# kanster/moped

Measured on AMD Instinct MI355X. Metric: detections/sec (frames/s) 640x480 ~3k SIFT vs N models, higher is better.
Workload: dtype f32

## Files before the change

### include/moped_hip.h

```cpp
#ifndef MOPED_HIP_H
#define MOPED_HIP_H

#include <stddef.h>
#include <stdint.h>

#ifdef __cplusplus
extern "C" {
#endif

#define MH_DESC_DIM 128
#define MH_MAX_BATCH 32
#define MH_MAX_IMAGES 8
#define MH_MAX_MODELS 8192
#define MH_OK 0
#define MH_ERR_ARG (-1)
#define MH_ERR_HIP (-2)
#define MH_ERR_CAPACITY (-3)
#define MH_ERR_NODEVICE (-4)

typedef struct mh_ctx mh_ctx;


int mh_create(int device, mh_ctx** out);
void mh_destroy(mh_ctx* ctx);
const char* mh_last_error(const mh_ctx* ctx);
int mh_set_stream(mh_ctx* ctx, void* hip_stream);
int mh_synchronize(mh_ctx* ctx);
int mh_reserve(mh_ctx* ctx, int max_queries, int max_clusters, int max_objects);
int mh_reserve_batch(mh_ctx* ctx, int queries_per_frame, int frames, int max_clusters, int max_objects);


int mh_db_upload(mh_ctx* ctx, const float* desc_host, const int32_t* model_of_host,
                 const float* xyz_host, int N, int n_models, int32_t index_base);
int mh_db_upload_blocks(mh_ctx* ctx, const float* desc_host, const int32_t* model_of_host, const float* xyz_host, int N,
                        int n_models, const int32_t* block_global_row, const int32_t* block_rows, int n_blocks,
                        int normalize);
int mh_db_size(const mh_ctx* ctx, int* N, int* n_models);
int mh_db_share(mh_ctx* dst, mh_ctx* src);

enum { MH_DB_INSERT = 0, MH_DB_REPLACE = 1, MH_DB_REMOVE = 2 };
int mh_db_model_rows(const mh_ctx* ctx, int model, int32_t* row_begin, int32_t* n_rows);
int mh_db_splice(mh_ctx* ctx, int op, int model, const float* desc, const float* xyz, int n_rows, int normalize,
                 int on_device);
int mh_db_reserve(mh_ctx* ctx, int64_t max_rows, int max_models);
int mh_db_adopt(mh_ctx* dst, mh_ctx* src);
int mh_db_generation(const mh_ctx* ctx, uint64_t* generation);
int mh_db_debug_fetch(mh_ctx* ctx, int which, void* out_host, size_t bytes);
int mh_db_debug_screen(mh_ctx* ctx, uint32_t out[8]);
int mh_db_debug_route(mh_ctx* ctx, int route);
int mh_db_edit_ms(mh_ctx* ctx, float* ms);


int mh_normalize(mh_ctx* ctx, float* desc_host, int n);

int mh_match(mh_ctx* ctx, const float* q_host, int Q, float ratio,
             int32_t* nn_idx, int32_t* nn_raw, float* d1, float* d2);
int mh_normalize_match(mh_ctx* ctx, float* q_host, int Q, float ratio, int32_t* nn_idx, int32_t* nn_raw, float* d1,
                       float* d2);

int mh_match_stats(mh_ctx* ctx, int Q, uint32_t stats[4], int reset);
int mh_match_set_mode(mh_ctx* ctx, int mode);
int mh_pose_set_split(mh_ctx* ctx, int on);
int mh_match_launches(mh_ctx* ctx, uint32_t out[3]);
float mh_screen_margin(float qq, float dmax);
int mh_screen_values(mh_ctx* ctx, const float* q_host, int Q, int n_rows, float* out_host, float* dmax, float* spread,
                     int shape );
uint16_t mh_screen_record_value(float top, float thr);
void mh_screen_record_bounds(uint16_t value_bits, uint32_t row0, float tau, float spread, int N, float dmax, float* lo,
                             float* hi);
float mh_screen_pack_value(float v, uint32_t id, int bits);
float mh_screen_pack_pert(float qq, float dmax, int bits);
void mh_screen_sample_bounds(uint16_t value_bits, float tau, float pert, float dmax, float* lo, float* hi);
void mh_screen_launch_plan(int Q, int q_expected, int N, int32_t out[8]);
int mh_screen_park_places(void);
int mh_match_incomplete(mh_ctx* ctx, uint32_t* count, int reset);
int mh_screen_sample_values(mh_ctx* ctx, const float* q_host, int Q, const int32_t* row0_host, float* out_host);
int mh_match_query_candidates(mh_ctx* ctx, int Q, uint32_t* out);

int mh_match_local_dev(mh_ctx* ctx, const float* qn_dev, const float* qnorm_dev, int Q,
                       int32_t* idx1_dev, float* d1_dev, float* d2_dev);
int mh_match_local_counted_dev(mh_ctx* ctx, const float* qn_dev, const float* qnorm_dev, int Q,
                               const int32_t* q_count_dev, int q_expected, int32_t* idx1_dev, float* d1_dev,
                               float* d2_dev);
int mh_match_merge_dev(mh_ctx* ctx, const int32_t* idx1_s_dev, const float* d1_s_dev,
                       const float* d2_s_dev, int n_shards, int Q,
                       int32_t* idx1_dev, float* d1_dev, float* d2_dev);
int mh_normalize_dev(mh_ctx* ctx, float* q_dev, float* qnorm_dev, int Q);


int mh_meanshift(mh_ctx* ctx, const float* pts_host, int n, int dim, float radius,
                 float merge, int min_pts, int max_iter, int32_t* label,
                 int32_t* order, int32_t* n_clusters);
int mh_meanshift_batch(mh_ctx* ctx, const float* pts_host, const int32_t* off, int n_problems,
                       int dim, float radius, float merge, int min_pts, int max_iter,
                       int32_t* label, int32_t* order, int32_t* n_clusters);


typedef struct {
  float u, v;
  float x, y, z;
} mh_corr;

typedef struct {
  float K[4];
  float cam[7];
} mh_cam;

typedef struct {
  int n_hypotheses;
  int max_objects_per_cluster;
  int n_pts_align;
  int min_n_pts_object;
  float error_threshold;
  int lm_iters_l2;
  int lm_iters_l4;
} mh_pose_params;

typedef struct {
  float pose[7];
  int32_t cluster;
  int32_t n_inliers;
  float err;
} mh_pose_out;

int mh_pose_ransac(mh_ctx* ctx, const mh_corr* corr_host, const int32_t* cluster_off,
                   int n_clusters, const mh_cam* cam, const mh_pose_params* prm,
                   uint64_t seed, mh_pose_out* out_host, int32_t* n_out);
int mh_pose_ransac_images(mh_ctx* ctx, const mh_corr* corr_host, const int32_t* image_of_host,
                          const int32_t* cluster_off, int n_clusters, const mh_cam* cams, int n_images,
                          const mh_pose_params* prm, uint64_t seed, mh_pose_out* out_host, int32_t* n_out);

typedef struct {
  float wx, wy, wz;
  float w;
} mh_depth;

#define MH_DEPTH_NONE 0
#define MH_DEPTH_BACKPROJECTION 1
#define MH_DEPTH_REPROJECTION 2

int mh_pose_ransac_depth(mh_ctx* ctx, const mh_corr* corr_host, const mh_depth* depth_host,
                         const int32_t* cluster_off, int n_clusters, const mh_cam* cam,
                         const mh_pose_params* prm, int kind, float alpha, uint64_t seed,
                         mh_pose_out* out_host, int32_t* n_out);

int mh_project_test(mh_ctx* ctx, const float pose[7], const mh_corr* corr_host, int n,
                    const mh_cam* cam, float thr, uint8_t* inlier_host, float* err2_host,
                    int32_t* n_inliers);


int mh_filter_images(mh_ctx* ctx, const mh_corr* corr_host, const int32_t* image_of_host, const int32_t* model_off,
                     int n_models, const int32_t* obj_model, const float* obj_pose, int n_obj, const mh_cam* cams,
                     int n_images, int min_points, float feature_distance, float min_score, float* score,
                     uint8_t* keep, int32_t* out_order, int32_t* cl_members, int32_t* cl_off, int32_t* n_kept);
int mh_filter(mh_ctx* ctx, const mh_corr* corr_host, const int32_t* model_off, int n_models,
              const int32_t* obj_model, const float* obj_pose, int n_obj, const mh_cam* cam,
              int min_points, float feature_distance, float min_score,
              float* score, uint8_t* keep, int32_t* out_order, int32_t* cl_members,
// ... 403 lines not shown
```

### moped_amd/capi.py

```python
from __future__ import annotations

import ctypes as C
import os

import numpy as np

_HERE = os.path.dirname(os.path.abspath(__file__))
LIB_PATH = os.environ.get("MH_LIB_PATH") or os.path.join(_HERE, "libmoped_hip.so")

MH_OK = 0
MH_ERR_ARG = -1
MH_ERR_CAPACITY = -3


class MhError(RuntimeError):
    pass


class mh_corr(C.Structure):
    _fields_ = [("u", C.c_float), ("v", C.c_float), ("x", C.c_float), ("y", C.c_float), ("z", C.c_float)]


class mh_cam(C.Structure):
    _fields_ = [("K", C.c_float * 4), ("cam", C.c_float * 7)]
# ... 117 lines not shown
    sp.merge_dist = float(merge_dist)
    return sp


def make_view(depth_ptr, fill_ptr=None, pose=None, K=None) -> mh_view:
    v = mh_view()
    v.depth_xyzn_dev = depth_ptr
    v.fill_distance_dev = fill_ptr
    v.pose[:] = [float(x) for x in (pose if pose is not None else POSE_IDENTITY)]
    v.K[:] = [float(x) for x in (K if K is not None else (1.0, 1.0, 0.0, 0.0))]
    return v


RAW_DEPTH_F32_M, RAW_DEPTH_U16_MM = 0, 1


class mh_raw_depth(C.Structure):
    _fields_ = [("format", C.c_int32), ("width", C.c_int32), ("height", C.c_int32), ("elem_stride", C.c_int32),
                ("row_stride", C.c_int32), ("offset", C.c_int32)]


def make_raw_depth(fmt, width, height, elem_stride=None, row_stride=None, offset=0) -> mh_raw_depth:
    es = 4 if fmt == RAW_DEPTH_F32_M else 2
    elem_stride = es if elem_stride is None else elem_stride
    row_stride = width * elem_stride if row_stride is None else row_stride
    return mh_raw_depth(int(fmt), int(width), int(height), int(elem_stride), int(row_stride), int(offset))


def make_filter_depth_params(p):
    if p is None or isinstance(p, mh_filter_depth_params):
        return p
    a, b, c = p
    return mh_filter_depth_params(float(a), float(b), float(c))


EXPORTS = [
    "mh_create", "mh_destroy", "mh_last_error", "mh_set_stream", "mh_synchronize", "mh_reserve",
    "mh_db_upload", "mh_db_size", "mh_normalize", "mh_match", "mh_normalize_match", "mh_match_local_dev", "mh_match_local_counted_dev",
    "mh_match_merge_dev", "mh_normalize_dev", "mh_meanshift", "mh_meanshift_batch", "mh_pose_ransac", "mh_pose_ransac_depth",
    "mh_frame_set_depth", "mh_project_test",
    "mh_filter", "mh_frame_default_params", "mh_frame_enqueue", "mh_frame_set_depth_image", "mh_frame_enqueue_match_local",
    "mh_frame_enqueue_rest", "mh_frame_fetch", "mh_frame_result_dev", "mh_enable_timing", "mh_timing",
    "mh_frame_set_cluster_linkage", "mh_cluster_linkage", "mh_frame_set_depth_image_host",
    "mh_depth_fill", "mh_depth_fill_status", "mh_depth_fill_host", "mh_depth_fill_batch", "mh_depth_fill_set_mode", "mh_depth_fill_get_mode", "mh_depth_fill_stats",
    "mh_frame_enqueue_rest_batch", "mh_frame_enqueue_rest_frames", "mh_frame_fetch_slot", "mh_frame_result_copy_slots_dev",
    "mh_frame_set_depth_rules", "mh_frame_fetch_matches", "mh_frame_enqueue_rest_strided", "mh_frame_result_copy_dev",
    "mh_sift_extract", "mh_sift_extract_dev", "mh_frame_enqueue_image", "mh_frame_enqueue_image_batch", "mh_frame_features_dev", "mh_frame_keypoints",
    "mh_models_create", "mh_models_destroy", "mh_models_last_error", "mh_models_add_xml",
    "mh_models_add_xml_buffer", "mh_models_count", "mh_models_rows", "mh_models_name", "mh_models_range",
    "mh_models_desc", "mh_models_xyz", "mh_models_save", "mh_models_load", "mh_db_upload_models",
    "mh_db_splice", "mh_db_reserve", "mh_db_adopt", "mh_db_generation", "mh_db_model_rows", "mh_db_splice_models",
    "mh_db_debug_fetch", "mh_depth_rules_debug_fetch", "mh_db_debug_screen", "mh_db_debug_route", "mh_db_edit_ms",
    "mh_db_upload_raw", "mh_db_share", "mh_match_stats", "mh_match_set_mode", "mh_match_launches", "mh_pose_set_split", "mh_frame_fetch_match_points", "mh_screen_margin", "mh_frame_counters", "mh_match_timing", "mh_frame_set_images", "mh_filter_images",
    "mh_pose_ransac_images",
    "mh_comm_unique_id", "mh_comm_create", "mh_comm_create_all", "mh_comm_create_host", "mh_comm_destroy", "mh_comm_info",
    "mh_frame_enqueue_sharded", "mh_frame_enqueue_sharded_batch", "mh_frame_enqueue_sharded_all",
    "mh_frame_previous_objects", "mh_frame_gather_objects", "mh_frame_enqueue_batch", "mh_frame_set_depth_image_batch",
    "mh_pose_kernel_info", "mh_db_upload_blocks", "mh_frame_fetch_matches_slot", "mh_frame_fetch_match_reps_slot",
    "mh_screen_values", "mh_screen_record_value", "mh_screen_record_bounds", "mh_reserve_batch", "mh_frame_run_host",
    "mh_frame_block_stride", "mh_frame_fetch_batch_async", "mh_frame_fetch_previous_async", "mh_frame_fetch_wait",
    "mh_frame_fetch_query", "mh_host_alloc", "mh_host_free", "mh_frame_run_host_begin", "mh_frame_wait_descriptors",
    "mh_step_match", "mh_step_match_fetch", "mh_step_cluster", "mh_step_pose", "mh_step_filter",
    "mh_set_linkage_scratch_limit",
    "mh_undistort_map", "mh_undistort", "mh_undistort_dev", "mh_frame_set_undistort",
    "mh_sift_extract_batch_dev", "mh_sift_debug_plan", "mh_sift_debug_level", "mh_sift_debug_candidates",
    "mh_sift_debug_keys", "mh_sift_debug_blur",
    "mh_screen_pack_value", "mh_screen_pack_pert", "mh_screen_sample_bounds", "mh_screen_launch_plan", "mh_match_incomplete",
    "mh_screen_sample_values", "mh_match_query_candidates", "mh_screen_park_places",
    "mh_frame_enqueue_images", "mh_frame_enqueue_images_batch", "mh_frame_set_undistort_images", "mh_frame_image_counts",
    "mh_frame_features_image_dev",
    "mh_filter_depth_set_points", "mh_filter_depth", "mh_frame_set_filter_depth",
    "mh_frame_route", "mh_filter_depth_debug_form",
    "mh_depth_filter", "mh_depth_prop", "mh_frame_run_kinect_host",
    "mh_linkage_debug_matrix", "mh_linkage_debug_agglomerate", "mh_linkage_set_mode", "mh_linkage_get_mode", "mh_linkage_stats", "mh_frame_debug_fetch_clusters_slot",
    "mh_planar_rows_dev", "mh_planar_rows_batch_dev", "mh_db_splice_image", "mh_db_splice_images",
    "mh_models_add_rows", "mh_models_write_xml",
    "mh_view_rows_dev", "mh_view_rows_batch_dev", "mh_db_append", "mh_db_splice_view", "mh_db_append_view", "mh_db_splice_views",
    "mh_depth_map_from_raw_dev", "mh_depth_map_from_raw_batch_dev", "mh_depth_map_from_raw_host",
    "mh_frame_run_kinect_raw_host",
    "mh_frame_debug_fetch_cluster_table_slot",
    "mh_object_hulls", "mh_hull_debug_form",
    "mh_frame_set_hulls", "mh_frame_fetch_hulls_slot", "mh_frame_fetch_hulls", "mh_frame_hull_block_stride",
    "mh_frame_fetch_batch_hulls_async",
]
COMM_ID_BYTES = 128
EX2_OBJECTS = 62
ALLGATHER_FN = C.CFUNCTYPE(C.c_int, C.c_void_p, C.c_void_p, C.c_void_p, C.c_size_t)

DIM = 128
HULL_LDS_POINTS = 8192
DB_INSERT, DB_REPLACE, DB_REMOVE = 0, 1, 2
_lib = None


def load():
    global _lib
    if _lib is not None:
        return _lib
    try:
        import torch
    except Exception:
        pass
    if not os.path.exists(LIB_PATH):
        raise MhError(f"{LIB_PATH} not built: run `python -c 'import __graft_entry__ as g; g.build()'`")
    L = C.CDLL(LIB_PATH)
    vp, i32, f32 = C.c_void_p, C.c_int, C.c_float
    L.mh_create.argtypes = [i32, C.POINTER(vp)]
    L.mh_destroy.argtypes = [vp]
    L.mh_destroy.restype = None
    L.mh_last_error.argtypes = [vp]
    L.mh_last_error.restype = C.c_char_p
    L.mh_set_stream.argtypes = [vp, vp]
    L.mh_synchronize.argtypes = [vp]
    L.mh_reserve.argtypes = [vp, i32, i32, i32]
    L.mh_reserve_batch.argtypes = [vp, i32, i32, i32, i32]
    if hasattr(L, "mh_lane_create"):
        L.mh_lane_create.argtypes = [i32, i32, i32, i32, C.POINTER(vp)]
        L.mh_lane_destroy.argtypes = [vp]
        L.mh_set_lane.argtypes = [vp, vp]
    L.mh_db_upload.argtypes = [vp, vp, vp, vp, i32, i32, C.c_int32]
    L.mh_db_size.argtypes = [vp, C.POINTER(i32), C.POINTER(i32)]
    L.mh_normalize.argtypes = [vp, vp, i32]
    L.mh_match.argtypes = [vp, vp, i32, f32, vp, vp, vp, vp]
    L.mh_normalize_match.argtypes = [vp, vp, i32, f32, vp, vp, vp, vp]
    L.mh_match_local_dev.argtypes = [vp, vp, vp, i32, vp, vp, vp]
    if hasattr(L, "mh_match_local_counted_dev"):
        L.mh_match_local_counted_dev.argtypes = [vp, vp, vp, i32, vp, i32, vp, vp, vp]
    L.mh_match_merge_dev.argtypes = [vp, vp, vp, vp, i32, i32, vp, vp, vp]
    L.mh_normalize_dev.argtypes = [vp, vp, vp, i32]
    L.mh_meanshift.argtypes = [vp, vp, i32, i32, f32, f32, i32, i32, vp, vp, C.POINTER(C.c_int32)]
    L.mh_meanshift_batch.argtypes = [vp, vp, vp, i32, i32, f32, f32, i32, i32, vp, vp, vp]
    L.mh_pose_ransac.argtypes = [vp, vp, vp, i32, C.POINTER(mh_cam), C.POINTER(mh_pose_params),
                                 C.c_uint64, vp, C.POINTER(C.c_int32)]
    L.mh_pose_ransac_depth.argtypes = [vp, vp, vp, vp, i32, C.POINTER(mh_cam), C.POINTER(mh_pose_params), i32, f32,
                                       C.c_uint64, vp, C.POINTER(C.c_int32)]
    L.mh_frame_set_depth.argtypes = [vp, vp, i32, f32]
    L.mh_project_test.argtypes = [vp, vp, vp, i32, C.POINTER(mh_cam), f32, vp, vp, C.POINTER(C.c_int32)]
    L.mh_filter.argtypes = [vp, vp, vp, i32, vp, vp, i32, C.POINTER(mh_cam), i32, f32, f32,
                            vp, vp, vp, vp, vp, C.POINTER(C.c_int32)]
    L.mh_frame_default_params.argtypes = [C.POINTER(mh_frame_params)]
    L.mh_frame_default_params.restype = None
    L.mh_frame_enqueue.argtypes = [vp, vp, vp, i32, C.POINTER(mh_cam), C.POINTER(mh_frame_params), C.c_uint64]
    L.mh_frame_run_host.argtypes = [vp, vp, vp, vp, i32, C.POINTER(mh_cam), i32, C.POINTER(mh_frame_params), C.c_uint64, i32,
                                    vp, i32, C.POINTER(C.c_int32), vp]
    L.mh_frame_run_host_begin.argtypes = [vp, vp, vp, vp, i32, C.POINTER(mh_cam), i32, C.POINTER(mh_frame_params), C.c_uint64, i32]
    L.mh_sift_extract.argtypes = [vp, vp, i32, i32, i32, vp, vp, vp, i32, C.POINTER(C.c_int32)]
    L.mh_sift_extract_dev.argtypes = [vp, vp, i32, i32, i32, vp, vp, vp, i32, vp]
    L.mh_sift_extract_batch_dev.argtypes = [vp, vp, i32, i32, i32, i32, vp, vp, i32, vp]
    L.mh_sift_debug_plan.argtypes = [vp, vp, vp, vp, vp]
    L.mh_sift_debug_level.argtypes = [vp, i32, i32, i32, i32, vp]
    L.mh_sift_debug_candidates.argtypes = [vp, i32, vp, vp, i32, C.POINTER(C.c_int32)]
    L.mh_sift_debug_keys.argtypes = [vp, i32, vp, i32, C.POINTER(C.c_int32)]
    L.mh_sift_debug_blur.argtypes = [vp, i32, vp, i32, i32, f32, i32, vp, vp, vp]
    L.mh_frame_enqueue_image.argtypes = [vp, vp, i32, i32, i32, i32, C.POINTER(mh_cam), C.POINTER(mh_frame_params),
                                         C.c_uint64]
    L.mh_frame_enqueue_image_batch.argtypes = [vp, vp, i32, i32, i32, i32, i32, C.POINTER(mh_cam), C.POINTER(mh_frame_params), vp]
    L.mh_frame_set_depth_image_host.argtypes = [vp, vp, vp, i32, i32, i32, f32, f32]
    L.mh_depth_fill.argtypes = [vp, vp, i32, i32, i32, i32, vp, vp, vp]
    L.mh_depth_fill_status.argtypes = [vp]
    L.mh_depth_fill_set_mode.argtypes = [vp, i32]
    L.mh_depth_fill_get_mode.argtypes = [vp, vp]
    L.mh_depth_fill_stats.argtypes = [vp, i32, vp]
    if hasattr(L, "mh_depth_fill_batch"):
        L.mh_depth_fill_batch.argtypes = [vp, C.POINTER(vp), C.POINTER(vp), i32, i32, i32, i32, i32, vp]
    L.mh_depth_fill_host.argtypes = [vp, vp, i32, i32, i32, i32, vp, vp, vp]
    L.mh_frame_set_cluster_linkage.argtypes = [vp, C.POINTER(mh_linkage_params)]
# ... 42 lines not shown
    L.mh_db_upload_raw.argtypes = [vp, vp, vp, vp, i32, i32, i32, i32]
    L.mh_frame_set_depth_image.argtypes = [vp, vp, vp, i32, i32, i32, f32, f32]
    L.mh_frame_enqueue_match_local.argtypes = [vp, vp, i32, vp]
    L.mh_frame_enqueue_rest.argtypes = [vp, vp, i32, vp, i32, C.POINTER(mh_cam),
                                        C.POINTER(mh_frame_params), C.c_uint64]
    L.mh_frame_fetch.argtypes = [vp, vp, i32, C.POINTER(C.c_int32), vp]
    L.mh_frame_result_dev.argtypes = [vp, C.POINTER(vp), C.POINTER(C.c_int64)]
    L.mh_db_share.argtypes = [vp, vp]
    L.mh_db_splice.argtypes = [vp, i32, i32, vp, vp, i32, i32, i32]
    L.mh_db_reserve.argtypes = [vp, C.c_int64, i32]
    L.mh_db_adopt.argtypes = [vp, vp]
    L.mh_db_generation.argtypes = [vp, C.POINTER(C.c_uint64)]
    L.mh_db_model_rows.argtypes = [vp, i32, C.POINTER(C.c_int32), C.POINTER(C.c_int32)]
    L.mh_db_splice_models.argtypes = [vp, i32, i32, vp, i32]
    L.mh_db_debug_fetch.argtypes = [vp, i32, vp, C.c_size_t]
    L.mh_depth_rules_debug_fetch.argtypes = [vp, i32, i32, vp, C.c_size_t]
    L.mh_depth_filter.argtypes = [vp, vp, i32, i32, vp, i32, f32, vp, vp, i32, vp]
    L.mh_depth_prop.argtypes = [vp, vp, vp, i32, i32, vp, i32, vp]
    L.mh_frame_run_kinect_host.argtypes = [vp, vp, vp, vp, i32, i32, i32, i32, C.POINTER(mh_cam), C.POINTER(mh_frame_params),
                                           i32, i32, i32, f32, f32, C.c_uint64, vp, i32, C.POINTER(C.c_int32), vp]
    if hasattr(L, "mh_depth_map_from_raw_dev"):
        rd = C.POINTER(mh_raw_depth)
        L.mh_depth_map_from_raw_dev.argtypes = [vp, vp, rd, vp, vp, i32, i32]
        L.mh_depth_map_from_raw_batch_dev.argtypes = [vp, C.POINTER(vp), rd, vp, C.POINTER(vp), i32, i32, i32]
        L.mh_depth_map_from_raw_host.argtypes = [vp, vp, rd, vp, vp, i32, i32]
        L.mh_frame_run_kinect_raw_host.argtypes = [vp, vp, vp, rd, vp, vp, i32, i32, i32, i32, C.POINTER(mh_cam),
                                                   C.POINTER(mh_frame_params), i32, i32, i32, f32, f32, C.c_uint64, vp, i32,
                                                   C.POINTER(C.c_int32), vp]
    L.mh_db_debug_screen.argtypes = [vp, vp]
    L.mh_db_debug_route.argtypes = [vp, i32]
    L.mh_db_edit_ms.argtypes = [vp, C.POINTER(f32)]
    L.mh_match_stats.argtypes = [vp, i32, vp, i32]
    L.mh_match_set_mode.argtypes = [vp, i32]
    L.mh_match_launches.argtypes = [vp, vp]
    L.mh_pose_set_split.argtypes = [vp, i32]
    L.mh_frame_counters.argtypes = [vp, vp]
    L.mh_frame_set_images.argtypes = [vp, vp, vp, i32]
    L.mh_filter_images.argtypes = [vp, vp, vp, vp, i32, vp, vp, i32, vp, i32, i32, f32, f32,
                                   vp, vp, vp, vp, vp, C.POINTER(C.c_int32)]
    L.mh_pose_ransac_images.argtypes = [vp, vp, vp, vp, i32, vp, i32, C.POINTER(mh_pose_params),
                                        C.c_uint64, vp, C.POINTER(C.c_int32)]
    L.mh_match_timing.argtypes = [vp, vp]
    L.mh_screen_margin.argtypes = [f32, f32]
    L.mh_screen_margin.restype = f32
    L.mh_enable_timing.argtypes = [vp, i32]
    L.mh_timing.argtypes = [vp, C.POINTER(mh_times)]
    L.mh_comm_unique_id.argtypes = [vp]
    L.mh_comm_create.argtypes = [vp, vp, i32, i32, C.POINTER(vp)]
    L.mh_comm_create_all.argtypes = [C.POINTER(vp), i32, C.POINTER(vp)]
    L.mh_comm_create_host.argtypes = [vp, i32, i32, ALLGATHER_FN, vp, C.POINTER(vp)]
    L.mh_comm_destroy.argtypes = [vp]
    L.mh_comm_info.argtypes = [vp, C.POINTER(i32), C.POINTER(i32), C.POINTER(i32)]
    L.mh_frame_enqueue_sharded.argtypes = [vp, vp, vp, vp, i32, C.POINTER(mh_cam), C.POINTER(mh_frame_params), C.c_uint64]
    L.mh_frame_enqueue_sharded_batch.argtypes = [vp, vp, vp, vp, i32, i32, C.POINTER(mh_cam),
                                                 C.POINTER(mh_frame_params), C.POINTER(C.c_uint64)]
    L.mh_frame_enqueue_sharded_all.argtypes = [C.POINTER(vp), C.POINTER(vp), i32, C.POINTER(vp), C.POINTER(vp), i32, i32,
                                               C.POINTER(mh_cam), C.POINTER(mh_frame_params), C.POINTER(C.c_uint64)]
    L.mh_frame_enqueue_batch.argtypes = [vp, vp, vp, i32, i32, C.POINTER(mh_cam), C.POINTER(mh_frame_params),
                                         C.POINTER(C.c_uint64)]
    L.mh_frame_set_depth_image_batch.argtypes = [vp, C.POINTER(vp), C.POINTER(vp), i32, i32, i32, i32, f32, f32]
    L.mh_frame_previous_objects.argtypes = [vp, i32, vp, i32, C.POINTER(C.c_int32)]
    L.mh_frame_gather_objects.argtypes = [vp, vp, i32, vp, i32, C.POINTER(C.c_int32)]
    L.mh_pose_kernel_info.argtypes = [vp, i32, vp]
    L.mh_frame_fetch_matches_slot.argtypes = [vp, i32, vp, vp, i32, C.POINTER(C.c_int32)]
    L.mh_frame_fetch_match_reps_slot.argtypes = [vp, i32, vp, i32, C.POINTER(C.c_int32)]
    L.mh_frame_fetch_match_points.argtypes = [vp, vp, i32, C.POINTER(C.c_int32)]
    L.mh_frame_enqueue_rest_frames.argtypes = [vp, vp, i32, vp, i32, i32, i32, i32, C.POINTER(mh_cam),
                                               C.POINTER(mh_frame_params), C.POINTER(C.c_uint64)]
    L.mh_screen_values.argtypes = [vp, vp, i32, i32, vp, C.POINTER(f32), C.POINTER(f32), i32]
    L.mh_screen_record_value.argtypes = [f32, f32]
    L.mh_screen_record_value.restype = C.c_uint16
    L.mh_screen_record_bounds.argtypes = [C.c_uint16, C.c_uint32, f32, f32, i32, f32, C.POINTER(f32), C.POINTER(f32)]
    L.mh_screen_record_bounds.restype = None
    if hasattr(L, "mh_screen_pack_value"):
        L.mh_screen_pack_value.argtypes = [f32, C.c_uint32, i32]
        L.mh_screen_pack_value.restype = f32
        L.mh_screen_pack_pert.argtypes = [f32, f32, i32]
        L.mh_screen_pack_pert.restype = f32
        L.mh_screen_sample_bounds.argtypes = [C.c_uint16, f32, f32, f32, C.POINTER(f32), C.POINTER(f32)]
        L.mh_screen_sample_bounds.restype = None
        L.mh_screen_launch_plan.argtypes = [i32, i32, i32, vp]
        L.mh_screen_launch_plan.restype = None
        L.mh_match_incomplete.argtypes = [vp, C.POINTER(C.c_uint32), i32]
    if hasattr(L, "mh_screen_sample_values"):
        L.mh_screen_sample_values.argtypes = [vp, vp, i32, vp, vp]
        L.mh_match_query_candidates.argtypes = [vp, i32, vp]
    L.mh_db_upload_blocks.argtypes = [vp, vp, vp, vp, i32, i32, vp, vp, i32, i32]
    L.mh_frame_block_stride.argtypes = [i32]
    L.mh_frame_block_stride.restype = C.c_size_t
    L.mh_frame_fetch_batch_async.argtypes = [vp, i32, i32, vp, C.c_uint32]
    L.mh_frame_fetch_previous_async.argtypes = [vp, i32, vp, C.c_uint32]
    L.mh_frame_fetch_wait.argtypes = [vp, C.POINTER(C.c_int32)]
    L.mh_host_alloc.argtypes = [vp, C.c_size_t, C.POINTER(vp)]
    L.mh_host_free.argtypes = [vp, vp]
    L.mh_frame_wait_descriptors.argtypes = [vp]
    if hasattr(L, "mh_step_match"):
        L.mh_set_linkage_scratch_limit.argtypes = [vp, C.c_size_t]
        L.mh_step_match.argtypes = [vp, vp, vp, i32, C.POINTER(mh_cam), f32, i32]
        L.mh_step_match_fetch.argtypes = [vp, vp, vp, vp, i32, C.POINTER(C.c_int32)]
        L.mh_step_cluster.argtypes = [vp, f32, f32, i32, i32, vp, vp, vp, i32, i32, C.POINTER(C.c_int32)]
        L.mh_step_pose.argtypes = [vp, i32, C.POINTER(mh_pose_params), C.c_uint64, vp, i32, C.POINTER(C.c_int32)]
        L.mh_step_filter.argtypes = [vp, i32, i32, f32, f32, i32, vp, vp, vp, vp, vp, i32, C.POINTER(C.c_int32)]
    L.mh_frame_fetch_query.argtypes = [vp]
    if hasattr(L, "mh_undistort"):
        L.mh_undistort_map.argtypes = [vp, i32, i32, vp, vp, vp, vp]
        L.mh_undistort.argtypes = [vp, vp, vp, i32, i32, vp, vp]
        L.mh_undistort_dev.argtypes = [vp, vp, vp, i32, i32, vp, vp]
        L.mh_frame_set_undistort.argtypes = [vp, vp]
    if hasattr(L, "mh_frame_enqueue_images"):
        L.mh_frame_enqueue_images.argtypes = [vp, vp, i32, i32, i32, i32, i32, vp, C.POINTER(mh_frame_params), C.c_uint64]
        L.mh_frame_enqueue_images_batch.argtypes = [vp, vp, i32, i32, i32, i32, i32, i32, vp, C.POINTER(mh_frame_params), vp]
        L.mh_frame_set_undistort_images.argtypes = [vp, vp, i32]
        L.mh_frame_image_counts.argtypes = [vp, vp, i32, C.POINTER(C.c_int32)]
        L.mh_frame_features_image_dev.argtypes = [vp, C.POINTER(vp)]
    if hasattr(L, "mh_filter_depth"):
        L.mh_filter_depth_set_points.argtypes = [vp, vp, vp, i32]
        L.mh_filter_depth.argtypes = [vp, vp, vp, i32, vp, vp, i32, C.POINTER(mh_cam), i32, f32, f32, C.POINTER(mh_cam),
                                      C.POINTER(mh_filter_depth_params), vp, vp, vp, vp, vp, C.POINTER(C.c_int32), vp, vp, vp]
        L.mh_frame_set_filter_depth.argtypes = [vp, C.POINTER(mh_filter_depth_params), C.POINTER(mh_filter_depth_params),
                                                C.POINTER(mh_cam)]
    if hasattr(L, "mh_frame_route"):
        L.mh_frame_route.argtypes = [vp, vp]
        L.mh_filter_depth_debug_form.argtypes = [vp, i32]
    if hasattr(L, "mh_planar_rows_dev"):
        L.mh_planar_rows_dev.argtypes = [vp, vp, vp, vp, i32, C.POINTER(mh_planar_spec), vp, vp, i32, vp, vp]
        L.mh_planar_rows_batch_dev.argtypes = [vp, vp, vp, vp, i32, i32, C.POINTER(mh_planar_spec), vp, vp, i32, vp, vp]
        L.mh_db_splice_image.argtypes = [vp, i32, i32, vp, i32, i32, i32, i32, C.POINTER(mh_planar_spec),
                                         C.POINTER(C.c_int32), vp, vp, vp, i32]
        L.mh_db_splice_images.argtypes = [vp, i32, vp, i32, i32, i32, i32, i32, C.POINTER(mh_planar_spec), vp, vp, vp, vp, i32]
        L.mh_models_add_rows.argtypes = [vp, C.c_char_p, vp, vp, C.c_int64]
        L.mh_models_write_xml.argtypes = [vp, i32, C.c_char_p]
    if hasattr(L, "mh_view_rows_dev"):
        pv, ps, pd = C.POINTER(mh_view), C.POINTER(mh_view_spec), C.POINTER(mh_view_dup)
        L.mh_view_rows_dev.argtypes = [vp, vp, vp, vp, i32, pv, i32, i32, ps, pd, vp, vp, i32, vp, vp, vp]
        L.mh_view_rows_batch_dev.argtypes = [vp, vp, vp, vp, i32, i32, pv, i32, i32, ps, pd, vp, vp, i32, vp, vp, vp]
        L.mh_db_append.argtypes = [vp, i32, vp, vp, i32, i32, i32]
        L.mh_db_splice_view.argtypes = [vp, i32, i32, vp, pv, i32, i32, i32, i32, ps, C.POINTER(C.c_int32), vp, vp, vp, vp, i32]
        L.mh_db_append_view.argtypes = [vp, i32, vp, pv, i32, i32, i32, i32, ps, C.POINTER(C.c_int32), vp, vp, vp, vp, i32]
        L.mh_db_splice_views.argtypes = [vp, i32, vp, pv, i32, i32, i32, i32, i32, ps, vp, vp, vp, vp, vp, i32]
    if hasattr(L, "mh_object_hulls"):
        L.mh_object_hulls.argtypes = [vp, vp, vp, i32, C.POINTER(mh_cam), i32, vp, vp, vp, vp]
        L.mh_hull_debug_form.argtypes = [vp, i32]
        L.mh_frame_set_hulls.argtypes = [vp, i32, i32]
        L.mh_frame_fetch_hulls_slot.argtypes = [vp, i32, i32, i32, vp, vp, vp, vp, C.POINTER(C.c_int32)]
        L.mh_frame_fetch_hulls.argtypes = [vp, i32, i32, vp, vp, vp, vp, C.POINTER(C.c_int32)]
        L.mh_frame_hull_block_stride.argtypes = [i32, i32]
        L.mh_frame_hull_block_stride.restype = C.c_size_t
        L.mh_frame_fetch_batch_hulls_async.argtypes = [vp, i32, i32, vp]
    _lib = L
    return L


def _calib(v):
    a = np.ascontiguousarray(v, np.float32).reshape(-1)
    if a.size != 4:
        raise ValueError("a calibration has 4 values")
    return a


def make_cam(K, cam) -> mh_cam:
    c = mh_cam()
    c.K[:] = [float(x) for x in K]
    c.cam[:] = [float(x) for x in cam]
    return c


# ... 400 lines not shown
        return dict(zip(names, (int(v) for v in o)))

    def db_debug_fetch(self, which: str) -> np.ndarray:
        sc = self.db_debug_screen()
        N, img = sc["N"], sc["has_image"]
        n_pad = (N + 127) // 128 * 128
        k, dt, n = {"desc": (0, np.float32, n_pad * DIM), "norm": (1, np.float32, n_pad), "xyz": (2, np.float32, N * 3),
                    "model": (3, np.int32, N), "desc_h": (4, np.uint16, n_pad * DIM if img else 0),
                    "neg_h": (5, np.float32, n_pad // 128 * 192 if img else 0)}[which]
        out = np.zeros(n, dt)
        self._ck(self.L.mh_db_debug_fetch(self.h, k, _ptr(out), out.nbytes), "mh_db_debug_fetch")
        return out

    def db_debug_route(self, route: int):
        self._ck(self.L.mh_db_debug_route(self.h, int(route)), "mh_db_debug_route")

    def db_edit_ms(self) -> float:
        ms = C.c_float(0)
        self._ck(self.L.mh_db_edit_ms(self.h, C.byref(ms)), "mh_db_edit_ms")
        return float(ms.value)

    def frame_counters(self) -> dict:
        c = np.zeros(8, np.int32)
        self._ck(self.L.mh_frame_counters(self.h, _ptr(c)), "mh_frame_counters")
        names = ("matches", "clusters", "r2", "r3", "r4", "pose_tasks", "error", "hypotheses")
        return dict(zip(names, (int(v) for v in c)))

    def pose_kernel_info(self, kind=0):
        o = np.zeros(8, np.int32)
        self._ck(self.L.mh_pose_kernel_info(self.h, int(kind), _ptr(o)), "mh_pose_kernel_info")
        waves = int(o[5])
        return {"vgprs": int(o[0]), "lds_bytes": int(o[1]), "threads": int(o[2]), "workgroups_per_cu": int(o[3]),
                "scratch_bytes": int(o[4]), "waves_per_workgroup": waves,
                "waves_per_simd": int(o[3]) * waves / 4.0}

    def match_timing(self) -> dict:
        t = np.zeros(5, np.float32)
        self._ck(self.L.mh_match_timing(self.h, _ptr(t)), "mh_match_timing")
        return dict(zip(("prepare_ms", "pass_a_ms", "thresholds_ms", "pass_b_ms", "pass_c_ms"), (float(v) for v in t)))

    def screen_values(self, qn, n_rows, shape=0):
        qn = np.ascontiguousarray(qn, np.float32)
        out = np.zeros((qn.shape[0], n_rows), np.float32)
        dmax, spread = C.c_float(0), C.c_float(0)
        self._ck(self.L.mh_screen_values(self.h, _ptr(qn), qn.shape[0], n_rows, _ptr(out), C.byref(dmax), C.byref(spread),
                                         int(shape)), "mh_screen_values")
        return out, dmax.value, spread.value

    def screen_sample_values(self, qn, row0):
        qn = np.ascontiguousarray(qn, np.float32)
        row0 = np.ascontiguousarray(row0, np.int32)
        assert row0.shape == (qn.shape[0], 2)
        out = np.zeros((qn.shape[0], 2, 8), np.float32)
        self._ck(self.L.mh_screen_sample_values(self.h, _ptr(qn), qn.shape[0], _ptr(row0), _ptr(out)), "mh_screen_sample_values")
        return out

    def match_set_mode(self, mode: int):
        self._ck(self.L.mh_match_set_mode(self.h, int(mode)), "mh_match_set_mode")

    def pose_set_split(self, on: bool):
        self._ck(self.L.mh_pose_set_split(self.h, int(bool(on))), "mh_pose_set_split")

    def match_kernel_launches(self) -> dict:
        o = np.zeros(3, np.uint32)
        self._ck(self.L.mh_match_launches(self.h, _ptr(o)), "mh_match_launches")
        return {"valu": int(o[0]), "mfma": int(o[1]), "screen": int(o[2])}

    def match_stats(self, Q=0, reset=False) -> dict:
        st = np.zeros(4, np.uint32)
        self._ck(self.L.mh_match_stats(self.h, int(Q), _ptr(st), int(reset)), "mh_match_stats")
        return {"candidates": int(st[0]), "brute_force_queries": int(st[1]), "queries": int(st[2]),
                "two_stage": bool(st[3])}

    def match_query_candidates(self, Q):
        out = np.zeros(int(Q), np.uint32)
        self._ck(self.L.mh_match_query_candidates(self.h, int(Q), _ptr(out)), "mh_match_query_candidates")
        return out

    def match_incomplete(self, reset=False) -> int:
        n = C.c_uint32(0)
        self._ck(self.L.mh_match_incomplete(self.h, C.byref(n), int(reset)), "mh_match_incomplete")
        return int(n.value)

    def normalize(self, desc):
        d = np.ascontiguousarray(desc, np.float32).copy()
        self._ck(self.L.mh_normalize(self.h, _ptr(d), d.shape[0]), "mh_normalize")
        return d

    def match(self, q, ratio=0.8):
        q = np.ascontiguousarray(q, np.float32)
        Q = q.shape[0]
        acc = np.full(Q, -1, np.int32)
        raw = np.full(Q, -1, np.int32)
        d1 = np.zeros(Q, np.float32)
        d2 = np.zeros(Q, np.float32)
        self._ck(self.L.mh_match(self.h, _ptr(q), Q, ratio, _ptr(acc), _ptr(raw), _ptr(d1), _ptr(d2)), "mh_match")
        return acc, raw, d1, d2

    def normalize_match(self, q, ratio=0.8):
        q = np.ascontiguousarray(q, np.float32).copy()
        Q = q.shape[0]
        acc = np.full(Q, -1, np.int32)
        raw = np.full(Q, -1, np.int32)
        d1 = np.zeros(Q, np.float32)
        d2 = np.zeros(Q, np.float32)
        self._ck(self.L.mh_normalize_match(self.h, _ptr(q), Q, ratio, _ptr(acc), _ptr(raw), _ptr(d1), _ptr(d2)),
                 "mh_normalize_match")
        return q, acc, raw, d1, d2

    def meanshift(self, pts, radius=200.0, merge=20.0, min_pts=7, max_iter=100):
        pts = np.ascontiguousarray(pts, np.float32)
        n = pts.shape[0]
        dim = pts.shape[1] if pts.ndim == 2 else 2
        label = np.full(max(n, 1), -1, np.int32)
        order = np.full(max(n, 1), -1, np.int32)
        ncl = C.c_int32(0)
        self._ck(self.L.mh_meanshift(self.h, _ptr(pts), n, dim, radius, merge, min_pts, max_iter,
                                     _ptr(label), _ptr(order), C.byref(ncl)), "mh_meanshift")
        label = label[:n]
        clusters, pos = [], 0
        for c in range(ncl.value):
            sz = int((label == c).sum())
            clusters.append(order[pos:pos + sz].copy())
            pos += sz
        return clusters, label

    def meanshift_batch(self, problems, radius=200.0, merge=20.0, min_pts=7, max_iter=100):
        dim = 2
        for p in problems:
            if np.asarray(p).ndim == 2 and np.asarray(p).shape[0]:
                dim = np.asarray(p).shape[1]
        sizes = [int(np.asarray(p).shape[0]) for p in problems]
        off = np.zeros(len(problems) + 1, np.int32)
        off[1:] = np.cumsum(sizes)
        total = int(off[-1])
        pts = (np.concatenate([np.asarray(p, np.float32).reshape(-1, dim) for p in problems])
               if total else np.zeros((0, dim), np.float32))
        pts = np.ascontiguousarray(pts, np.float32)
        label = np.full(max(total, 1), -1, np.int32)
        order = np.full(max(total, 1), -1, np.int32)
        ncl = np.zeros(max(len(problems), 1), np.int32)
        self._ck(self.L.mh_meanshift_batch(self.h, _ptr(pts), _ptr(off), len(problems), dim, radius, merge,
                                           min_pts, max_iter, _ptr(label), _ptr(order), _ptr(ncl)),
                 "mh_meanshift_batch")
        out = []
        for i in range(len(problems)):
            b, e = int(off[i]), int(off[i + 1])
            lab, ordr = label[b:e], order[b:e]
            clusters, pos = [], 0
            for c in range(int(ncl[i])):
                sz = int((lab == c).sum())
                clusters.append(ordr[pos:pos + sz].copy())
                pos += sz
            out.append((clusters, lab.copy()))
        return out

    def pose_ransac(self, corr, cluster_off, K, cam, params: mh_pose_params, seed=1):
        corr = np.ascontiguousarray(corr, CORR_DTYPE)
        cluster_off = np.ascontiguousarray(cluster_off, np.int32)
        ncl = len(cluster_off) - 1
        R = max(params.max_objects_per_cluster, 1)
        out = np.zeros(max(ncl * R, 1), POSE_OUT_DTYPE)
        n_out = C.c_int32(0)
        c = make_cam(K, cam)
        self._ck(self.L.mh_pose_ransac(self.h, _ptr(corr), _ptr(cluster_off), ncl, C.byref(c),
                                       C.byref(params), seed, _ptr(out), C.byref(n_out)), "mh_pose_ransac")
# ... 971 lines not shown
```

### moped_amd/csrc/api.hip

```cpp
#include <algorithm>
#include <cmath>
#include <cstring>
#include <new>
#include <vector>

#include "context.h"
#include "steps.h"

using namespace mh;

namespace mh {

int use_stream(mh_ctx* ctx) {
  if (!ctx->held.empty()) db_poll_held(ctx, false);
  if (ctx->stream) return MH_OK;
  if (!ctx->own_stream) MH_HIP(ctx, hipStreamCreateWithFlags(&ctx->own_stream, hipStreamNonBlocking));
  ctx->stream = ctx->own_stream;
  return MH_OK;
}

int ensure_scratch(mh_ctx* ctx, size_t bytes) {
  if (bytes > ctx->scratch.cap) MH_HIP(ctx, ctx->scratch.ensure(bytes + bytes / 4 + 4096, ctx->stream));
  return MH_OK;
}

int ensure_pinned(mh_ctx* ctx, size_t bytes) {
  if (bytes > ctx->pinned.cap) MH_HIP(ctx, ctx->pinned.ensure(bytes + bytes / 4 + 4096, ctx->stream));
  return MH_OK;
}

int ensure_own_depth(mh_ctx* ctx, size_t px) {
  MH_HIP(ctx, ctx->own_depth.ensure(px * 4, ctx->stream));
  MH_HIP(ctx, ctx->own_fill.ensure(px, ctx->stream));
  return MH_OK;
}

void bind_store(mh_ctx* ctx) {
  const DbStore* st = ctx->store.get();
  ctx->N = st ? st->N : 0;
  ctx->n_models = st ? st->n_models : 0;
  ctx->index_base = st ? st->index_base : 0;
  ctx->rmap = RowMap();
  if (st) {
    ctx->rmap.base = st->index_base;
    ctx->rmap.nb = st->n_blocks;
    ctx->rmap.glo = st->blk_glo;
    ctx->rmap.llo = st->blk_llo;
  }
  ctx->db_desc = st ? st->desc : nullptr;
  ctx->db_norm = st ? st->norm : nullptr;
  ctx->db_xyz = st ? st->xyz : nullptr;
  ctx->db_model = st ? st->model : nullptr;
  ctx->sdb = st ? st->screen : ScreenDb();
}

int ensure_match_scratch(mh_ctx* ctx, int Q) {
  hipStream_t s = ctx->stream;
  MH_HIP(ctx, ctx->match_pack.ensure(match_pack_floats(Q), s));
  MH_HIP(ctx, ctx->match_scratch.ensure(match_scratch_elems(Q, ctx->N > 0 ? ctx->N : 1), s));
  const int q_pad = screen_q_pad(Q);
  if (ctx->sdb.usable && q_pad > ctx->sbuf.q_pad) {
    ScreenBufs& b = ctx->sbuf;
    mh_ctx::ScreenOwn& o = ctx->screen_own;
    b = ScreenBufs();
    const size_t qp = (size_t)q_pad, slots = qp * screen_rec_slots();
    MH_HIP(ctx, o.qh.ensure(qp * DIM, s));
    MH_HIP(ctx, o.qbad.ensure(qp, s));
    MH_HIP(ctx, o.part.ensure(screen_part_bytes(q_pad), s));
    MH_HIP(ctx, o.tau.ensure(qp, s));
    MH_HIP(ctx, o.recs.ensure(slots, s));
    MH_HIP(ctx, o.ovf_cnt.ensure(qp, s));
    MH_HIP(ctx, o.ovf.ensure(qp * SCREEN_OVF_CAP, s));
    MH_HIP(ctx, o.stats.ensure(qp * 3, s));
    MH_HIP(ctx, o.inc.ensure(qp + 1, s));
    MH_HIP(ctx, hipMemsetAsync(o.inc, 0, (qp + 1) * sizeof(unsigned int), s));
    MH_HIP(ctx, hipMemsetAsync(o.recs, 0, slots * sizeof(uint2), s));
    MH_HIP(ctx, hipMemsetAsync(o.ovf_cnt, 0, qp * sizeof(int32_t), s));
    MH_HIP(ctx, hipMemsetAsync(o.stats, 0, qp * 3 * sizeof(unsigned int), s));
    b.qh = o.qh;
    b.qbad = o.qbad;
    b.part = reinterpret_cast<float2*>(o.part.p);
    b.tau = o.tau;
    b.recs = o.recs;
    b.ovf_cnt = o.ovf_cnt;
    b.ovf = o.ovf;
    b.stats = o.stats;
    b.inc = o.inc;
    b.ovf_cap = SCREEN_OVF_CAP;
    b.q_pad = q_pad;
  }
  return MH_OK;
}

int ctx_match(mh_ctx* ctx, const float* qn, const float* qnorm, int Q, int32_t* idx1, float* d1, float* d2,
              const int32_t* q_count, int q_expected) {
  if (Q <= 0) return MH_OK;
  int rc = ensure_match_scratch(ctx, Q);
  if (rc) return rc;
  const int qe = (q_expected > 0 && q_expected < Q) ? q_expected : Q;
  const int screen_mode = ctx->match_mode >= 2 ? 0 : ctx->match_mode;
  const int kernel_pin = ctx->match_mode >= 2 ? ctx->match_mode - 2 : -1;
  if (ctx->sdb.usable && ctx->sbuf.q_pad >= screen_q_pad(Q) && screen_wanted(qe, ctx->N, screen_mode)) {
    ctx->sbuf.ev = nullptr;
    if (ctx->timing && ctx->ev_made) {
      ctx->sbuf.ev = ctx->mev[ctx->mev_next];
      ctx->mev_next = (ctx->mev_next + 1) % mh_ctx::MEV_SETS;
      ++ctx->mev_used;
    }
    ctx->sbuf.big = ctx->lane_stream;
    ctx->sbuf.n_cus = ctx->n_cus;
    ctx->sbuf.ev_in = ctx->lane_in;
    ctx->sbuf.ev_out = ctx->lane_out;
    launch_match_screen(qn, qnorm, Q, ctx->db_desc, ctx->db_norm, ctx->N, ctx->rmap, ctx->sdb, ctx->sbuf, idx1, d1,
                        d2, ctx->stream, q_count, q_expected);
    ++ctx->match_launches[2];
  } else {
    const int k = launch_match(qn, qnorm, Q, ctx->db_desc, ctx->db_norm, ctx->N, ctx->rmap, ctx->match_scratch,
                               ctx->match_pack, idx1, d1, d2, ctx->stream, q_count, q_expected, kernel_pin);
    if (k >= 0) ++ctx->match_launches[k];
  }
  return MH_OK;
}

int ensure_frame_buffers(mh_ctx* ctx, int Q) {
  if (Q <= ctx->max_q) return MH_OK;
  int cap = ctx->max_q > 0 ? ctx->max_q : 4096;
  while (cap < Q) cap *= 2;
  const size_t n = (size_t)cap;
  hipStream_t s = ctx->stream;
  MH_HIP(ctx, ctx->q_desc.ensure(n * DIM, s));
  MH_HIP(ctx, ctx->q_norm.ensure(n, s));
  MH_HIP(ctx, ctx->q_uv.ensure(n * 2, s));
  MH_HIP(ctx, ctx->nn_idx.ensure(n, s));
  MH_HIP(ctx, ctx->nn_d1.ensure(n, s));
  MH_HIP(ctx, ctx->nn_d2.ensure(n, s));
  ctx->max_q = cap;
  return MH_OK;
}

}

extern "C" {

int mh_create(int device, mh_ctx** out) {
  if (!out) return MH_ERR_ARG;
  *out = nullptr;
  int count = 0;
  if (hipGetDeviceCount(&count) != hipSuccess || count <= 0 || device < 0 || device >= count)
    return MH_ERR_NODEVICE;
  hipDeviceProp_t prop;
  if (hipGetDeviceProperties(&prop, device) != hipSuccess) return MH_ERR_NODEVICE;
  if (std::strncmp(prop.gcnArchName, "gfx950", 6) != 0) return MH_ERR_NODEVICE;
  if (hipSetDevice(device) != hipSuccess) return MH_ERR_HIP;
  mh_ctx* ctx = new (std::nothrow) mh_ctx;
  if (!ctx) return MH_ERR_HIP;
  ctx->device = device;
  ctx->n_cus = prop.multiProcessorCount;
  ctx->stream = nullptr;
  *out = ctx;
  return MH_OK;
}

void mh_free_frame_state(mh_ctx* ctx);
void mh_free_sift_state(mh_ctx* ctx);
void mh_free_undistort_state(mh_ctx* ctx);

void mh_destroy(mh_ctx* ctx) {
  if (!ctx) return;
  hipSetDevice(ctx->device);
  if (ctx->stream) hipStreamSynchronize(ctx->stream);
  mh_free_frame_state(ctx);
  mh_free_sift_state(ctx);
  mh_free_undistort_state(ctx);
  db_poll_held(ctx, true);
  for (hipEvent_t e : ctx->held_events) hipEventDestroy(e);
  for (hipEvent_t e : ctx->db_ev)
    if (e) hipEventDestroy(e);
  if (ctx->wb_ev) hipEventDestroy(ctx->wb_ev);
  if (ctx->wb_stream) hipStreamDestroy(ctx->wb_stream);
  if (ctx->ev_made)
    for (auto& e : ctx->ev) hipEventDestroy(e);
  for (auto& set : ctx->mev)
    for (auto& e : set)
      if (e) hipEventDestroy(e);
  if (ctx->dlv.done) hipEventDestroy(ctx->dlv.done);
  if (ctx->hulls.done) hipEventDestroy(ctx->hulls.done);
  if (ctx->lane_in) hipEventDestroy(ctx->lane_in);
  if (ctx->lane_out) hipEventDestroy(ctx->lane_out);
  if (ctx->own_stream) hipStreamDestroy(ctx->own_stream);
  delete ctx;
}

#ifdef MH_EXPERIMENTS
extern "C" int mh_lane_create(int device, int n_streams, int reserve_cus_per_xcd, int low_priority, mh_lane** out) {
  if (low_priority) return MH_ERR_ARG;
// ... 231 lines not shown
}

int mh_normalize(mh_ctx* ctx, float* desc_host, int n) {
  if (!ctx || n < 0 || (n > 0 && !desc_host)) return MH_ERR_ARG;
  if (n == 0) return MH_OK;
  MH_HIP(ctx, hipSetDevice(ctx->device));
  if (int rc_stream = mh::use_stream(ctx)) return rc_stream;
  int rc = ensure_frame_buffers(ctx, n);
  if (rc) return rc;
  const size_t bytes = (size_t)n * DIM * sizeof(float);
  MH_HIP(ctx, hipMemcpyAsync(ctx->q_desc, desc_host, bytes, hipMemcpyHostToDevice, ctx->stream));
  launch_normalize(ctx->q_desc, ctx->q_norm, n, ctx->stream);
  MH_HIP(ctx, hipGetLastError());
  MH_HIP(ctx, hipMemcpyAsync(desc_host, ctx->q_desc, bytes, hipMemcpyDeviceToHost, ctx->stream));
  MH_HIP(ctx, hipStreamSynchronize(ctx->stream));
  return MH_OK;
}

int mh_normalize_dev(mh_ctx* ctx, float* q_dev, float* qnorm_dev, int Q) {
  if (!ctx || Q < 0 || (Q > 0 && (!q_dev || !qnorm_dev))) return MH_ERR_ARG;
  MH_HIP(ctx, hipSetDevice(ctx->device));
  if (int rc_stream = mh::use_stream(ctx)) return rc_stream;
  launch_normalize(q_dev, qnorm_dev, Q, ctx->stream);
  MH_HIP(ctx, hipGetLastError());
  return MH_OK;
}

int mh_match_local_dev(mh_ctx* ctx, const float* qn_dev, const float* qnorm_dev, int Q,
                       int32_t* idx1_dev, float* d1_dev, float* d2_dev) {
  if (!ctx || Q < 0 || (Q > 0 && (!qn_dev || !qnorm_dev || !idx1_dev || !d1_dev || !d2_dev)))
    return MH_ERR_ARG;
  if (Q == 0) return MH_OK;
  MH_HIP(ctx, hipSetDevice(ctx->device));
  if (int rc_stream = mh::use_stream(ctx)) return rc_stream;
  int rc = ctx_match(ctx, qn_dev, qnorm_dev, Q, idx1_dev, d1_dev, d2_dev);
  if (rc) return rc;
  MH_HIP(ctx, hipGetLastError());
  return MH_OK;
}

int mh_match_local_counted_dev(mh_ctx* ctx, const float* qn_dev, const float* qnorm_dev, int Q, const int32_t* q_count_dev,
                               int q_expected, int32_t* idx1_dev, float* d1_dev, float* d2_dev) {
  if (!ctx || Q < 0 || q_expected < 0 || !q_count_dev || (Q > 0 && (!qn_dev || !qnorm_dev || !idx1_dev || !d1_dev || !d2_dev)))
    return MH_ERR_ARG;
  if (Q == 0) return MH_OK;
  MH_HIP(ctx, hipSetDevice(ctx->device));
  if (int rc_stream = mh::use_stream(ctx)) return rc_stream;
  int rc = ctx_match(ctx, qn_dev, qnorm_dev, Q, idx1_dev, d1_dev, d2_dev, q_count_dev, q_expected);
  if (rc) return rc;
  MH_HIP(ctx, hipGetLastError());
  return MH_OK;
}

int mh_match_merge_dev(mh_ctx* ctx, const int32_t* idx1_s_dev, const float* d1_s_dev,
                       const float* d2_s_dev, int n_shards, int Q, int32_t* idx1_dev,
                       float* d1_dev, float* d2_dev) {
  if (!ctx || Q < 0 || n_shards < 0) return MH_ERR_ARG;
  if (Q == 0) return MH_OK;
  MH_HIP(ctx, hipSetDevice(ctx->device));
  if (int rc_stream = mh::use_stream(ctx)) return rc_stream;
  launch_match_merge(idx1_s_dev, d1_s_dev, d2_s_dev, n_shards, Q, (size_t)Q, idx1_dev, d1_dev, d2_dev,
                     ctx->stream);
  MH_HIP(ctx, hipGetLastError());
  return MH_OK;
}

static int match_host(mh_ctx* ctx, const float* q_host, float* normalized_out, int Q, float ratio, int32_t* nn_idx,
                      int32_t* nn_raw, float* d1, float* d2) {
  if (!ctx || Q < 0 || (Q > 0 && (!q_host || !nn_idx))) return MH_ERR_ARG;
  if (Q == 0) return MH_OK;
  MH_HIP(ctx, hipSetDevice(ctx->device));
  if (int rc_stream = mh::use_stream(ctx)) return rc_stream;
  int rc = ensure_frame_buffers(ctx, Q);
  if (rc) return rc;
  if ((rc = ensure_match_scratch(ctx, Q))) return rc;
  if ((rc = ensure_pinned(ctx, (size_t)Q * 16))) return rc;
  if ((rc = ensure_scratch(ctx, (size_t)Q * 4))) return rc;
  const size_t bytes = (size_t)Q * DIM * sizeof(float);
  MH_HIP(ctx, hipMemcpyAsync(ctx->q_desc, q_host, bytes, hipMemcpyHostToDevice, ctx->stream));
  if (normalized_out)
    launch_normalize(ctx->q_desc, ctx->q_norm, Q, ctx->stream);
  else
    launch_row_norms(ctx->q_desc, ctx->q_norm, Q, ctx->stream);
  if ((rc = ctx_match(ctx, ctx->q_desc, ctx->q_norm, Q, ctx->nn_idx, ctx->nn_d1, ctx->nn_d2))) return rc;
  int32_t* d_acc = (int32_t*)ctx->scratch.p;
  launch_accept(ctx->nn_idx, ctx->nn_d1, ctx->nn_d2, Q, ratio, d_acc, ctx->stream);
  MH_HIP(ctx, hipGetLastError());
  int32_t* h_acc = (int32_t*)ctx->pinned.p;
  int32_t* h_raw = h_acc + Q;
  float* h_d1 = (float*)(h_raw + Q);
  float* h_d2 = h_d1 + Q;
  MH_HIP(ctx, hipMemcpyAsync(h_acc, d_acc, (size_t)Q * 4, hipMemcpyDeviceToHost, ctx->stream));
  MH_HIP(ctx, hipMemcpyAsync(h_raw, ctx->nn_idx, (size_t)Q * 4, hipMemcpyDeviceToHost, ctx->stream));
  MH_HIP(ctx, hipMemcpyAsync(h_d1, ctx->nn_d1, (size_t)Q * 4, hipMemcpyDeviceToHost, ctx->stream));
  MH_HIP(ctx, hipMemcpyAsync(h_d2, ctx->nn_d2, (size_t)Q * 4, hipMemcpyDeviceToHost, ctx->stream));
  if (normalized_out) MH_HIP(ctx, hipMemcpyAsync(normalized_out, ctx->q_desc, bytes, hipMemcpyDeviceToHost, ctx->stream));
  MH_HIP(ctx, hipStreamSynchronize(ctx->stream));
  std::memcpy(nn_idx, h_acc, (size_t)Q * 4);
  if (nn_raw) std::memcpy(nn_raw, h_raw, (size_t)Q * 4);
  if (d1) std::memcpy(d1, h_d1, (size_t)Q * 4);
  if (d2) std::memcpy(d2, h_d2, (size_t)Q * 4);
  return MH_OK;
}

int mh_match(mh_ctx* ctx, const float* q_host, int Q, float ratio, int32_t* nn_idx,
             int32_t* nn_raw, float* d1, float* d2) {
  return match_host(ctx, q_host, nullptr, Q, ratio, nn_idx, nn_raw, d1, d2);
}

int mh_normalize_match(mh_ctx* ctx, float* q_host, int Q, float ratio, int32_t* nn_idx, int32_t* nn_raw, float* d1,
                       float* d2) {
  return match_host(ctx, q_host, q_host, Q, ratio, nn_idx, nn_raw, d1, d2);
}

#ifdef MH_TRACE
static unsigned long long* g_trace_dev = nullptr;
int mh_trace_enable(int on) {
  if (on && !g_trace_dev) {
    if (hipMalloc(&g_trace_dev, (8 + 4 * TRACE_CAP) * sizeof(unsigned long long)) != hipSuccess) return MH_ERR_HIP;
    hipMemset(g_trace_dev, 0, 64);
  }
  unsigned long long* p = on ? g_trace_dev : nullptr;
  const int n = std::min(trace_n_binds().load(), 32);
  for (int i = 0; i < n; ++i) trace_binds()[i](p);
  hipDeviceSynchronize();
  return MH_OK;
}
long long mh_trace_fetch(unsigned long long* out, long long cap) {
  if (!g_trace_dev) return -1;
  hipDeviceSynchronize();
  unsigned long long n = 0;
  hipMemcpy(&n, g_trace_dev, sizeof n, hipMemcpyDeviceToHost);
  const unsigned long long have = std::min<unsigned long long>(n, TRACE_CAP);
  const unsigned long long take = std::min<unsigned long long>(have, (unsigned long long)std::max(cap, 0ll));
  if (take && out) hipMemcpy(out, g_trace_dev + 8, take * 32, hipMemcpyDeviceToHost);
  hipMemset(g_trace_dev, 0, 8);
  return (long long)n;
}
#endif

float mh_screen_margin(float qq, float dmax) { return screen_margin_host(qq, dmax); }

uint16_t mh_screen_record_value(float top, float thr) { return screen_record_value(top, thr); }

void mh_screen_record_bounds(uint16_t value_bits, uint32_t row0, float tau, float spread, int N, float dmax, float* lo,
                             float* hi) {
  float l, h;
  screen_record_bounds(value_bits, row0, tau, spread, N, dmax, l, h);
  if (lo) *lo = l;
  if (hi) *hi = h;
}

float mh_screen_pack_value(float v, uint32_t id, int bits) { return screen_pack_value(v, id, bits); }

float mh_screen_pack_pert(float qq, float dmax, int bits) { return screen_pack_pert(qq, dmax, bits); }

void mh_screen_sample_bounds(uint16_t value_bits, float tau, float pert, float dmax, float* lo, float* hi) {
  float l, h;
  screen_sample_bounds(value_bits, tau, pert, dmax, l, h);
  if (lo) *lo = l;
  if (hi) *hi = h;
}

void mh_screen_launch_plan(int Q, int q_expected, int N, int32_t out[8]) {
  int v[8];
  screen_launch_plan(Q, q_expected, N, v);
  for (int k = 0; k < 8; ++k) out[k] = v[k];
}

int mh_screen_park_places(void) { return screen_park_places(); }

int mh_match_incomplete(mh_ctx* ctx, uint32_t* count, int reset) {
  if (!ctx || !count) return MH_ERR_ARG;
  MH_HIP(ctx, hipSetDevice(ctx->device));
  if (int rc_stream = mh::use_stream(ctx)) return rc_stream;
  MH_HIP(ctx, hipStreamSynchronize(ctx->stream));
  *count = 0;
  if (ctx->sbuf.inc) {
    unsigned int* c = ctx->sbuf.inc + ctx->sbuf.q_pad;
    MH_HIP(ctx, hipMemcpy(count, c, sizeof(unsigned int), hipMemcpyDeviceToHost));
    if (reset) MH_HIP(ctx, hipMemset(c, 0, sizeof(unsigned int)));
  }
  return MH_OK;
}

int mh_screen_values(mh_ctx* ctx, const float* q_host, int Q, int n_rows, float* out_host, float* dmax, float* spread,
                     int shape) {
  if (!ctx || !q_host || !out_host || Q <= 0 || n_rows <= 0 || (Q & 31) || (n_rows & 31)) {
    if (ctx) ctx->err = "mh_screen_values: Q and n_rows must be positive multiples of 32";
    return MH_ERR_ARG;
  }
  if (!ctx->sdb.dbh || n_rows > (ctx->N + 127) / 128 * 128) {
    ctx->err = "mh_screen_values: the database has no f16 image (fewer than 4096 rows?) or fewer rows than asked for";
    return MH_ERR_ARG;
  }
  MH_HIP(ctx, hipSetDevice(ctx->device));
  if (int rc_stream = mh::use_stream(ctx)) return rc_stream;
  const int q_pad = screen_q_pad(Q);
  hipStream_t s = ctx->stream;
  DevBuf<float> qd, qn, out;
  DevBuf<_Float16> qh;
  DevBuf<uint8_t> qbad;
  int rc = MH_OK;
  if (qd.ensure((size_t)Q * DIM, s) != hipSuccess || qn.ensure(Q, s) != hipSuccess ||
      out.ensure((size_t)Q * n_rows, s) != hipSuccess || qh.ensure((size_t)q_pad * DIM, s) != hipSuccess ||
      qbad.ensure(q_pad, s) != hipSuccess) {
    ctx->err = "mh_screen_values: out of device memory";
    return MH_ERR_HIP;
  }
  hipMemcpyAsync(qd, q_host, (size_t)Q * DIM * 4, hipMemcpyHostToDevice, ctx->stream);
  launch_row_norms(qd, qn, Q, ctx->stream);
  launch_screen_prepare(qd, qn, Q, q_pad, qh, qbad, ctx->stream);
  launch_screen_values(qh, Q, ctx->sdb, n_rows, out, ctx->stream, shape);
  if (hipMemcpyAsync(out_host, out, (size_t)Q * n_rows * 4, hipMemcpyDeviceToHost, ctx->stream) != hipSuccess ||
      hipStreamSynchronize(ctx->stream) != hipSuccess || hipGetLastError() != hipSuccess) {
    ctx->err = "mh_screen_values: device error";
    rc = MH_ERR_HIP;
  }
  if (dmax) *dmax = ctx->sdb.dmax;
  if (spread) *spread = ctx->sdb.spread;
  return rc;
}

int mh_screen_sample_values(mh_ctx* ctx, const float* q_host, int Q, const int32_t* row0_host, float* out_host) {
  if (!ctx || !q_host || !row0_host || !out_host || Q <= 0) return MH_ERR_ARG;
  if (!ctx->sdb.dbh) {
    ctx->err = "mh_screen_sample_values: the database has no f16 image (fewer than 4096 rows?)";
    return MH_ERR_ARG;
  }
  const int n_pad = (ctx->N + 127) / 128 * 128;
  for (int i = 0; i < 2 * Q; ++i) {
    const int r = row0_host[i];
    if (r < 0 || (r & 3) || (r & 31) >= 16 || r + 19 >= n_pad) {
      ctx->err = "mh_screen_sample_values: row0 is not the first row of a lane's block (32 b + 4 quarter) inside the padded DB";
      return MH_ERR_ARG;
    }
  }
  MH_HIP(ctx, hipSetDevice(ctx->device));
  if (int rc_stream = mh::use_stream(ctx)) return rc_stream;
  hipStream_t s = ctx->stream;
  DevBuf<float> qd, out;
  DevBuf<int32_t> rd;
  int rc = MH_OK;
  if (qd.ensure((size_t)Q * DIM, s) != hipSuccess || out.ensure((size_t)Q * 16, s) != hipSuccess ||
      rd.ensure((size_t)Q * 2, s) != hipSuccess) {
    ctx->err = "mh_screen_sample_values: out of device memory";
    return MH_ERR_HIP;
  }
  hipMemcpyAsync(qd, q_host, (size_t)Q * DIM * 4, hipMemcpyHostToDevice, ctx->stream);
  hipMemcpyAsync(rd, row0_host, (size_t)Q * 2 * 4, hipMemcpyHostToDevice, ctx->stream);
  launch_screen_sample_values(qd, Q, ctx->sdb, rd, out, ctx->stream);
  if (hipMemcpyAsync(out_host, out, (size_t)Q * 16 * 4, hipMemcpyDeviceToHost, ctx->stream) != hipSuccess ||
      hipStreamSynchronize(ctx->stream) != hipSuccess || hipGetLastError() != hipSuccess) {
    ctx->err = "mh_screen_sample_values: device error";
    rc = MH_ERR_HIP;
  }
  return rc;
}

int mh_match_set_mode(mh_ctx* ctx, int mode) {
  if (!ctx || mode < -1 || mode > 3) return MH_ERR_ARG;
  ctx->match_mode = mode;
  return MH_OK;
}

int mh_pose_set_split(mh_ctx* ctx, int on) {
  if (!ctx) return MH_ERR_ARG;
  ctx->pose_split = on ? 1 : 0;
  return MH_OK;
}

int mh_match_launches(mh_ctx* ctx, uint32_t out[3]) {
  if (!ctx || !out) return MH_ERR_ARG;
  for (int k = 0; k < 3; ++k) out[k] = ctx->match_launches[k];
  return MH_OK;
}

int mh_match_stats(mh_ctx* ctx, int Q, uint32_t stats[4], int reset) {
  if (!ctx || !stats) return MH_ERR_ARG;
  MH_HIP(ctx, hipSetDevice(ctx->device));
  if (int rc_stream = mh::use_stream(ctx)) return rc_stream;
  stats[0] = stats[1] = stats[2] = stats[3] = 0;
  if (Q > 0) {
    int rc = ensure_match_scratch(ctx, Q);
    if (rc) return rc;
    stats[3] = (ctx->sdb.usable && ctx->sbuf.q_pad >= screen_q_pad(Q) && screen_wanted(Q, ctx->N, ctx->match_mode >= 2 ? 0 : ctx->match_mode)) ? 1u : 0u;
  }
  MH_HIP(ctx, hipStreamSynchronize(ctx->stream));
  if (ctx->sbuf.stats) {
    std::vector<unsigned int> h((size_t)ctx->sbuf.q_pad * 3);
    MH_HIP(ctx, hipMemcpy(h.data(), ctx->sbuf.stats, h.size() * sizeof(unsigned int), hipMemcpyDeviceToHost));
    unsigned long long sum[3] = {0, 0, 0};
    for (size_t i = 0; i < h.size(); ++i) sum[i % 3] += h[i];
    for (int k = 0; k < 3; ++k) stats[k] = (uint32_t)std::min<unsigned long long>(sum[k], 0xFFFFFFFFull);
    if (reset) MH_HIP(ctx, hipMemset(ctx->sbuf.stats, 0, h.size() * sizeof(unsigned int)));
  }
  return MH_OK;
}

int mh_match_query_candidates(mh_ctx* ctx, int Q, uint32_t* out) {
  if (!ctx || !out || Q <= 0) return MH_ERR_ARG;
  MH_HIP(ctx, hipSetDevice(ctx->device));
  if (int rc_stream = mh::use_stream(ctx)) return rc_stream;
  MH_HIP(ctx, hipStreamSynchronize(ctx->stream));
  if (!ctx->sbuf.stats || Q > ctx->sbuf.q_pad) {
    ctx->err = "mh_match_query_candidates: no two-stage scratch for that many queries";
    return MH_ERR_ARG;
  }
  std::vector<unsigned int> h((size_t)Q * 3);
  MH_HIP(ctx, hipMemcpy(h.data(), ctx->sbuf.stats, h.size() * sizeof(unsigned int), hipMemcpyDeviceToHost));
  for (int q = 0; q < Q; ++q) out[q] = h[3 * (size_t)q];
  return MH_OK;
}

int mh_enable_timing(mh_ctx* ctx, int on) {
  if (!ctx) return MH_ERR_ARG;
  MH_HIP(ctx, hipSetDevice(ctx->device));
  if (int rc_stream = mh::use_stream(ctx)) return rc_stream;
  if (on && !ctx->ev_made) {
    for (auto& e : ctx->ev) MH_HIP(ctx, hipEventCreate(&e));
    for (auto& set : ctx->mev)
      for (auto& e : set) MH_HIP(ctx, hipEventCreate(&e));
    ctx->ev_made = true;
  }
  ctx->timing = on != 0;
  ctx->mev_next = ctx->mev_used = 0;
  return MH_OK;
}

int mh_match_timing(mh_ctx* ctx, float ms[5]) {
  if (!ctx || !ms || !ctx->timing || !ctx->ev_made || ctx->mev_used == 0) return MH_ERR_ARG;
  MH_HIP(ctx, hipSetDevice(ctx->device));
  MH_HIP(ctx, hipStreamSynchronize(ctx->stream));
  const int n = std::min(ctx->mev_used, (int)mh_ctx::MEV_SETS);
  double sum[5] = {0, 0, 0, 0, 0};
  for (int k = 0; k < n; ++k) {
    const int set = ((ctx->mev_next - 1 - k) % mh_ctx::MEV_SETS + mh_ctx::MEV_SETS) % mh_ctx::MEV_SETS;
    for (int i = 0; i < 5; ++i) {
      float t = 0.f;
      if (hipEventElapsedTime(&t, ctx->mev[set][i], ctx->mev[set][i + 1]) != hipSuccess) return MH_ERR_HIP;
      sum[i] += t;
    }
// ... 8 lines not shown
```

### moped_amd/csrc/api_frame.hip

```cpp
#include <climits>
#include <cstring>

#include "frame.h"
#include "hull.h"

using namespace mh;

namespace {

static_assert(1 + MH_MAX_IMAGES <= MH_MAX_BATCH, "a frame's total and counts fit one row of the words");
inline int32_t* images_single_total(const mh_ctx* ctx) { return ctx->imf.words ? ctx->imf.words + 2 * MH_MAX_BATCH : nullptr; }

__global__ void image_batch_tail_kernel(float* __restrict__ desc, float* __restrict__ norm, const int32_t* __restrict__ counts,
                                        int Q, int B) {
  const int i = blockIdx.x * blockDim.x + threadIdx.x;
  if (i >= B * Q * (DIM / 4)) return;
  const int row = i / (DIM / 4), f = row / Q, q = row - f * Q;
  if (q < min(counts[f], Q)) return;
  reinterpret_cast<float4*>(desc)[i] = make_float4(0.f, 0.f, 0.f, 0.f);
  if (i % (DIM / 4) == 0) norm[row] = -1.f;
}
__global__ void image_batch_mask_kernel(int32_t* __restrict__ idx, float* __restrict__ d1, float* __restrict__ d2,
                                        const int32_t* __restrict__ counts, int Q, int B) {
  const int row = blockIdx.x * blockDim.x + threadIdx.x;
// ... 39 lines not shown

int read_out(mh_ctx* ctx, const int32_t* head, const int32_t* snap, int32_t flags, const mh_object* first, int n_first,
             const unsigned char* result_dev, mh_object* objects_host, int max_objects, int32_t* n_objects, int32_t* counts) {
  FrameState* fs = ctx->fs;
  const int n = head[0];
  *n_objects = n;
  if (counts) std::memcpy(counts, snap, 4 * sizeof(int32_t));
  const int tasks = 4 * std::max(snap[1], snap[3]);
  fs->task_grid = std::min(96, std::max(16, (tasks + tasks / 2 + 7) / 8 * 8));
  fs->ms_grid = std::min(32, std::max(4, snap[1] + 2));
  const int take = n < max_objects ? n : max_objects;
  if (take > 0 && objects_host) {
    const int have = std::min(take, n_first);
    std::memcpy(objects_host, first, sizeof(mh_object) * (size_t)have);
    if (take > have)
      MH_HIP(ctx, hipMemcpy(objects_host + have, result_dev + 16 + sizeof(mh_object) * (size_t)have,
                            sizeof(mh_object) * (size_t)(take - have), hipMemcpyDeviceToHost));
  }
  return frame_flags(ctx, flags);
}

int match_lists(mh_ctx* ctx, const char* who, int slot, int cap, int32_t* n_matches, size_t* arena, int* take) {
  if (int rc_enter = mh::enter(ctx)) return rc_enter;
  FrameState* fs = ctx->fs;
  if (slot < 0) slot = fs->list_first + fs->list_n - 1;
  if (slot < fs->list_first || slot >= fs->list_first + fs->list_n) {
    ctx->err = std::string(who) + ": the lists of that frame are gone (frames that went through the steps one "
               "after the other share one set of working arrays: only the last one's remain)";
    return MH_ERR_ARG;
  }
  *arena = (size_t)(slot - fs->list_first) * fs->arena_bytes;
  int32_t snap[4] = {0, 0, 0, 0};
  MH_HIP(ctx, hipMemcpyAsync(snap, fs->snap + 4 * slot, sizeof snap, hipMemcpyDeviceToHost, ctx->stream));
  MH_HIP(ctx, hipStreamSynchronize(ctx->stream));
  *n_matches = snap[0];
  *take = std::min(snap[0], cap);
  return MH_OK;
}

int result_copy_bytes(mh_ctx* ctx, int max_objects, size_t* bytes) {
  if (int rc_enter = mh::enter(ctx)) return rc_enter;
  if (!ctx->fs)
    if (int rc = prepare_frame(ctx, ctx->max_q > 0 ? ctx->max_q : 1)) return rc;
  *bytes = std::min(ctx->fs->result_bytes, 16 + sizeof(mh_object) * (size_t)max_objects);
  return MH_OK;
}

int rest_of_batch(mh_ctx* ctx, FrameCall c, int B, const uint64_t* seeds, bool merge, bool own_maps = false) {
  if (merge) {
    if (int rc = ensure_batch_arenas(ctx, B)) return rc;
    c.seed = seeds[0];
    c.seeds = seeds;
    c.batch_n = B;
    if (c.gathered) stamp(ctx, 1);
    return frame_rest(ctx, c);
  }
  const float* const q_uv = c.q_uv;
  const int32_t* const gathered = c.gathered;
  const int32_t* const q_count = c.q_count;
  own_maps = own_maps && B > 1 && ctx->batch_imgs == B && ctx->depth_img.img;
  int rc = MH_OK;
  for (int f = 0; f < B && rc == MH_OK; ++f) {
    c.q_uv = q_uv + 2 * (size_t)f * c.Q;
    c.gathered = gathered ? gathered + (size_t)f * c.Q : nullptr;
    c.q0 = gathered ? 0 : f * c.Q;
    c.slot = c.frame = f;
    c.seed = seeds[f];
    c.q_count = q_count ? q_count + f : nullptr;
    if (own_maps) {
      c.img = ctx->batch_img[f];
      c.fill = ctx->batch_fill[f];
    }
    if (gathered) stamp(ctx, 1);
    rc = frame_rest(ctx, c);
  }
  if (rc == MH_OK) ctx->frame_route[0] = B;
  return rc;
}

int image_frame_rest(mh_ctx* ctx, int Q, int32_t* n_dev, const mh_cam* cam, const mh_frame_params* prm, uint64_t seed) {
  ctx->feat_count_dev = n_dev;
  stamp(ctx, 0);
  launch_normalize(ctx->q_desc, ctx->q_norm, Q, ctx->stream, n_dev);
  if (int rc = ctx_match(ctx, ctx->q_desc, ctx->q_norm, Q, ctx->nn_idx, ctx->nn_d1, ctx->nn_d2, n_dev, ctx->feat_expected)) return rc;
  stamp(ctx, 1);
  FrameCall c{ctx->q_uv, Q, cam, prm, seed};
  c.q_count = n_dev;
  return frame_rest(ctx, c);
}

int image_batch_rest(mh_ctx* ctx, int Q, int B, const int32_t* counts, const mh_cam* cam, const mh_frame_params* prm,
                     const uint64_t* seeds, bool merge, bool own_maps = false) {
  hipStream_t s = ctx->stream;
  launch_normalize_batch(ctx->q_desc, ctx->q_norm, Q, B, s, counts);
  MH_HIP(ctx, hipGetLastError());
  ctx->feat_count_dev = nullptr;
  stamp(ctx, 0);
  hipLaunchKernelGGL(image_batch_tail_kernel, dim3((B * Q * (DIM / 4) + 255) / 256), dim3(256), 0, s, ctx->q_desc, ctx->q_norm,
                     counts, Q, B);
  if (int rc = ctx_match(ctx, ctx->q_desc, ctx->q_norm, B * Q, ctx->nn_idx, ctx->nn_d1, ctx->nn_d2)) return rc;
  hipLaunchKernelGGL(image_batch_mask_kernel, dim3((B * Q + 255) / 256), dim3(256), 0, s, ctx->nn_idx, ctx->nn_d1, ctx->nn_d2,
                     counts, Q, B);
  stamp(ctx, 1);
  FrameCall c{ctx->q_uv, Q, cam, prm, 0};
  c.q_count = counts;
  return rest_of_batch(ctx, c, B, seeds, merge, own_maps);
}

int enqueue_rest(mh_ctx* ctx, const float* q_uv_dev, int Q, const int32_t* gathered_dev, int n_shards, int shard_stride,
                 int plane_stride, int slot, const mh_cam* cam, const mh_frame_params* prm, uint64_t seed) {
  if (!ctx || Q <= 0 || !q_uv_dev || !gathered_dev || n_shards <= 0 || !cam || !prm) return MH_ERR_ARG;
  if (int rc = filter_depth_frame_ok(ctx, "mh_frame_enqueue_rest", prm, 1, true)) return rc;
  if (int rc_enter = mh::enter(ctx)) return rc_enter;
  if (int rc = prepare_frame(ctx, Q)) return rc;
  stamp(ctx, 1);
  FrameCall c{q_uv_dev, Q, cam, prm, seed};
  c.gathered = gathered_dev;
  c.n_shards = n_shards;
  c.shard_stride = shard_stride;
  c.plane_stride = plane_stride;
  c.slot = slot;
  return frame_rest(ctx, c);
}

}

namespace mh {

int upload_cams(mh_ctx* ctx, const mh_cam* cams, int n_images) {
  MH_HIP(ctx, ctx->cams_dev.ensure(MH_MAX_IMAGES, ctx->stream));
  ctx->cams_view = ctx->cams_dev;
  DevCam h[MH_MAX_IMAGES];
  for (int i = 0; i < n_images; ++i) h[i] = make_devcam(cams[i]);
  MH_HIP(ctx, hipStreamSynchronize(ctx->stream));
  MH_HIP(ctx, hipMemcpy(ctx->cams_dev, h, sizeof(DevCam) * n_images, hipMemcpyHostToDevice));
  return MH_OK;
}

int enqueue_features(mh_ctx* ctx, float* q_desc_dev, const float* q_uv_dev, int Q, const mh_cam* cam,
                     const mh_frame_params* prm, uint64_t seed, const FeatureOptions& opt) {
  if (opt.stage_lo == 0 && opt.stage_hi == 5)
    if (int rc = filter_depth_frame_ok(ctx, "frame", prm)) return rc;
  if (int rc_enter = enter(ctx)) return rc_enter;
  if (int rc = prepare_frame(ctx, Q)) return rc;
  ctx->feat_count_dev = nullptr;
  stamp(ctx, 0);
  launch_normalize(q_desc_dev, ctx->q_norm, Q, ctx->stream);
  if (opt.write_back && ctx->wb_ev) hipEventRecord(ctx->wb_ev, ctx->stream);
  if (int rc_m = ctx_match(ctx, q_desc_dev, ctx->q_norm, Q, ctx->nn_idx, ctx->nn_d1, ctx->nn_d2)) return rc_m;
  stamp(ctx, 1);
  ctx->step.done = -1;
  FrameCall c{q_uv_dev, Q, cam, prm, seed};
  c.stage_lo = opt.stage_lo;
  c.stage_hi = opt.stage_hi;
  return frame_rest(ctx, c);
}

int host_frame_begin(mh_ctx* ctx, float* q_desc_host, const float* q_uv_host, const int32_t* q_image_host, int Q,
                     const mh_cam* cams, int n_images, const mh_frame_params* prm, uint64_t seed, const FeatureOptions& opt) {
  if (!ctx || Q <= 0 || !q_desc_host || !q_uv_host || !cams || n_images < 1 || n_images > MH_MAX_IMAGES || !prm ||
      (n_images > 1 && !q_image_host)) {
    if (ctx) ctx->err = "mh_frame_run_host: bad argument";
    return MH_ERR_ARG;
  }
  if (int rc_enter = mh::enter(ctx)) return rc_enter;
  if (ctx->wb_stream) {
    MH_HIP(ctx, hipStreamSynchronize(ctx->wb_stream));
    ctx->wb_pending = false;
  }
  int rc = ensure_frame_buffers(ctx, Q);
  if (rc) return rc;
  MH_HIP(ctx, hipMemcpyAsync(ctx->q_desc, q_desc_host, (size_t)Q * DIM * sizeof(float), hipMemcpyHostToDevice, ctx->stream));
  MH_HIP(ctx, hipMemcpyAsync(ctx->q_uv, q_uv_host, (size_t)Q * 2 * sizeof(float), hipMemcpyHostToDevice, ctx->stream));
  if (n_images > 1) {
    if (ctx->hf_img.cap < (size_t)Q) MH_HIP(ctx, ctx->hf_img.ensure((size_t)ctx->max_q, ctx->stream));
    MH_HIP(ctx, hipMemcpyAsync(ctx->hf_img, q_image_host, (size_t)Q * sizeof(int32_t), hipMemcpyHostToDevice, ctx->stream));
    if ((rc = mh_frame_set_images(ctx, ctx->hf_img, cams, n_images))) return rc;
  } else if (ctx->q_img) {
    if ((rc = mh_frame_set_images(ctx, nullptr, nullptr, 0))) return rc;
  }
  if (opt.write_back && !ctx->wb_stream) {
    MH_HIP(ctx, hipStreamCreateWithFlags(&ctx->wb_stream, hipStreamNonBlocking));
    MH_HIP(ctx, hipEventCreateWithFlags(&ctx->wb_ev, hipEventDisableTiming));
  }
  if ((rc = enqueue_features(ctx, ctx->q_desc, ctx->q_uv, Q, &cams[0], prm, seed, opt))) return rc;
  if (opt.write_back) {
    MH_HIP(ctx, hipStreamWaitEvent(ctx->wb_stream, ctx->wb_ev, 0));
    ctx->wb_pending = true;
    MH_HIP(ctx, hipMemcpyAsync(q_desc_host, ctx->q_desc, (size_t)Q * DIM * sizeof(float), hipMemcpyDeviceToHost, ctx->wb_stream));
  }
  return MH_OK;
}

int delivery_begin(mh_ctx* ctx, void* host_block, size_t bytes, unsigned char** dst_dev) {
  auto& d = ctx->dlv;
  if (d.pending) {
    ctx->err = "delivery: the context's previous delivery has not been waited for (mh_frame_fetch_wait)";
    return MH_ERR_ARG;
  }
  if (!d.done) MH_HIP(ctx, hipEventCreateWithFlags(&d.done, hipEventDisableTiming));
  void* dev = nullptr;
  if (hipHostGetDevicePointer(&dev, host_block, 0) == hipSuccess && dev) {
    *dst_dev = static_cast<unsigned char*>(dev);
    return MH_OK;
  }
  (void)hipGetLastError();
  MH_HIP(ctx, d.stage.ensure(bytes, ctx->stream));
  *dst_dev = d.stage;
  return MH_OK;
}

int delivery_end(mh_ctx* ctx, void* host_block, size_t bytes, unsigned char* dst_dev, int B, int max_objects, uint32_t tag) {
  auto& d = ctx->dlv;
  MH_HIP(ctx, hipGetLastError());
  if (dst_dev == d.stage)
    MH_HIP(ctx, hipMemcpyAsync(host_block, d.stage, bytes, hipMemcpyDeviceToHost, ctx->stream));
  MH_HIP(ctx, hipEventRecord(d.done, ctx->stream));
  d.pending = true;
  d.host_block = static_cast<unsigned char*>(host_block);
  d.B = B;
  d.max_objects = max_objects;
  d.tag = tag;
  return MH_OK;
}

}

extern "C" {

size_t mh_frame_block_stride(int max_objects) {
  return sizeof(mh_frame_head) + sizeof(mh_object) * (size_t)(max_objects > 0 ? max_objects : 0);
}
// ... 531 lines not shown
  }
  if ((rc = sift_into_batch(ctx, gray_dev, F * n, width, height, double_size, cap, m.desc, m.xy, m.words))) return rc;
  ImagesPackArgs pa;
  pa.sdesc = m.desc;
  pa.sxy = m.xy;
  pa.scount = m.words;
  pa.desc = ctx->q_desc;
  pa.uv = ctx->q_uv;
  pa.q_img = m.q_img;
  pa.totals = batched ? m.words + MH_MAX_BATCH : images_single_total(ctx);
  pa.counts = batched ? m.words + 2 * MH_MAX_BATCH : images_single_total(ctx) + 1;
  pa.cams_dev = m.cams;
  pa.cap = cap;
  pa.n_images = n;
  for (int i = 0; i < MH_MAX_IMAGES; ++i) pa.cams[i] = make_devcam(cams[i < n ? i : 0]);
  launch_images_pack(pa, F, s);
  MH_HIP(ctx, hipGetLastError());
  if (!batched) {
    m.n_live = n;
    return image_frame_rest(ctx, Q, pa.totals, &cams[0], prm, seeds[0]);
  }
  m.n_live = 0;
  return image_batch_rest(ctx, Q, F, pa.totals, &cams[0], prm, seeds, merge);
}

int mh_frame_enqueue_images(mh_ctx* ctx, const uint8_t* const* gray_dev, int n_images, int width, int height, int double_size,
                            int max_keypoints_per_image, const mh_cam* cams, const mh_frame_params* prm, uint64_t seed) {
  return enqueue_images(ctx, "mh_frame_enqueue_images", gray_dev, 1, n_images, width, height, double_size,
                        max_keypoints_per_image, cams, prm, &seed, false);
}

int mh_frame_enqueue_images_batch(mh_ctx* ctx, const uint8_t* const* gray_dev, int n_frames, int n_images, int width,
                                  int height, int double_size, int max_keypoints_per_image, const mh_cam* cams,
                                  const mh_frame_params* prm, const uint64_t* seeds) {
  return enqueue_images(ctx, "mh_frame_enqueue_images_batch", gray_dev, n_frames, n_images, width, height, double_size,
                        max_keypoints_per_image, cams, prm, seeds, true);
}

int mh_frame_image_counts(mh_ctx* ctx, int32_t* counts, int cap, int32_t* n_images) {
  if (!ctx || !n_images || cap < 0 || (cap > 0 && !counts) || ctx->imf.last_n <= 0) return MH_ERR_ARG;
  *n_images = ctx->imf.last_n;
  for (int i = 0; i < ctx->imf.last_n && i < cap; ++i) counts[i] = ctx->imf.last[i];
  return MH_OK;
}

int mh_frame_features_image_dev(mh_ctx* ctx, int32_t** q_image_dev) {
  if (!ctx || !q_image_dev || !ctx->feat_count_dev || ctx->feat_count_dev != images_single_total(ctx) || !ctx->imf.n_live)
    return MH_ERR_ARG;
  *q_image_dev = ctx->imf.q_img;
  return MH_OK;
}

int mh_frame_features_dev(mh_ctx* ctx, float** desc_dev, float** uv_dev, int32_t** n_dev) {
  if (!ctx || !ctx->feat_count_dev) return MH_ERR_ARG;
  if (desc_dev) *desc_dev = ctx->q_desc;
  if (uv_dev) *uv_dev = ctx->q_uv;
  if (n_dev) *n_dev = ctx->feat_count_dev;
  return MH_OK;
}

int mh_frame_keypoints(mh_ctx* ctx, int32_t* n_keypoints) {
  if (!ctx || !n_keypoints || ctx->feat_last < 0) return MH_ERR_ARG;
  *n_keypoints = ctx->feat_last;
  return MH_OK;
}

int mh_frame_enqueue_batch(mh_ctx* ctx, float* q_desc_dev, const float* q_uv_dev, int Q, int B, const mh_cam* cam,
                           const mh_frame_params* prm, const uint64_t* seeds) {
  if (!ctx || Q <= 0 || B < 1 || B > MH_MAX_BATCH || !q_desc_dev || !q_uv_dev || !cam || !prm || !seeds)
    return MH_ERR_ARG;
  if (B > 1 && (ctx->depth_img.img || ctx->rules.on) && ctx->batch_imgs != B) {
    ctx->err = "mh_frame_enqueue_batch: a depth map belongs to ONE frame (mh_frame_set_depth_image_batch hands in one per "
               "frame of the batch)";
    return MH_ERR_ARG;
  }
  if (int rc_fd = filter_depth_frame_ok(ctx, "mh_frame_enqueue_batch", prm)) return rc_fd;
  if (int rc_enter = mh::enter(ctx)) return rc_enter;
  const bool merge = B > 1 && merged_batch_ok(ctx, prm, true, B);
  int rc = prepare_frame(ctx, B * Q, Q, merge ? B : 1);
  if (rc) return rc;
  ctx->feat_count_dev = nullptr;
  stamp(ctx, 0);
  launch_normalize(q_desc_dev, ctx->q_norm, B * Q, ctx->stream);
  if ((rc = ctx_match(ctx, q_desc_dev, ctx->q_norm, B * Q, ctx->nn_idx, ctx->nn_d1, ctx->nn_d2))) return rc;
  stamp(ctx, 1);
  return rest_of_batch(ctx, FrameCall{q_uv_dev, Q, cam, prm, 0}, B, seeds, merge, true);
}

int mh_frame_enqueue_match_local(mh_ctx* ctx, float* q_desc_dev, int Q, int32_t* top2_dev) {
  if (!ctx || Q <= 0 || !q_desc_dev || !top2_dev) return MH_ERR_ARG;
  if (int rc_enter = mh::enter(ctx)) return rc_enter;
  int rc = ensure_frame_buffers(ctx, Q);
  if (rc) return rc;
  if ((rc = ensure_match_scratch(ctx, Q))) return rc;
  if (!ctx->fs && (rc = prepare_frame(ctx, Q))) return rc;
  float* d1 = reinterpret_cast<float*>(top2_dev + Q);
  ctx->feat_count_dev = nullptr;
  stamp(ctx, 0);
  launch_normalize(q_desc_dev, ctx->q_norm, Q, ctx->stream);
  if (int rc_m = ctx_match(ctx, q_desc_dev, ctx->q_norm, Q, top2_dev, d1, d1 + Q)) return rc_m;
  MH_HIP(ctx, hipGetLastError());
  return MH_OK;
}

int mh_frame_enqueue_rest(mh_ctx* ctx, const float* q_uv_dev, int Q, const int32_t* gathered_dev,
                          int n_shards, const mh_cam* cam, const mh_frame_params* prm, uint64_t seed) {
  return enqueue_rest(ctx, q_uv_dev, Q, gathered_dev, n_shards, 0, 0, 0, cam, prm, seed);
}

int mh_frame_fetch(mh_ctx* ctx, mh_object* objects_host, int max_objects, int32_t* n_objects,
                   int32_t* counts) {
  if (!ctx || !n_objects || !ctx->fs) return MH_ERR_ARG;
  if (int rc_enter = mh::enter(ctx)) return rc_enter;
  FrameState* fs = ctx->fs;
  FrameState::FetchPin& pin = *fs->fetch_pin;
  if (fs->host_armed && !ctx->feat_count_dev) {
    MH_HIP(ctx, hipStreamSynchronize(ctx->stream));
    const FrameHostBlock& h = *fs->host_block;
    const uint32_t seq = h.seq;
    if (seq != fs->host_seq_expect) fs->host_seq_expect = seq;
    else
      return read_out(ctx, h.head, h.snap, h.error, h.objects, FRAME_HOST_OBJECTS, fs->result, objects_host, max_objects,
                      n_objects, counts);
  }
  const size_t first = std::min(fs->result_bytes, sizeof pin.head + sizeof pin.objects);
  MH_HIP(ctx, hipMemcpyAsync(pin.head, fs->result, first, hipMemcpyDeviceToHost, ctx->stream));
  MH_HIP(ctx, hipMemcpyAsync(pin.snap, fs->snap, sizeof pin.snap, hipMemcpyDeviceToHost, ctx->stream));
  MH_HIP(ctx, hipMemcpyAsync(&pin.fc, fs->counts, sizeof pin.fc, hipMemcpyDeviceToHost, ctx->stream));
  pin.n_feat = -1;
  const int rig = ctx->feat_count_dev && ctx->feat_count_dev == images_single_total(ctx) ? ctx->imf.n_live : 0;
  if (ctx->feat_count_dev)
    MH_HIP(ctx, hipMemcpyAsync(&pin.n_feat, ctx->feat_count_dev, sizeof(int32_t) * (1 + rig), hipMemcpyDeviceToHost, ctx->stream));
  MH_HIP(ctx, hipStreamSynchronize(ctx->stream));
  const int32_t n_feat = pin.n_feat;
  if (n_feat >= 0) {
    ctx->feat_expected = ctx->feat_last = n_feat;
    ctx->imf.last_n = rig ? rig : 1;
    ctx->imf.last[0] = n_feat;
    for (int i = 0; i < rig; ++i) ctx->imf.last[i] = pin.img_n[i];
  }
  return read_out(ctx, pin.head, pin.snap, pin.fc.error, pin.objects, FETCH_PIN_OBJECTS, fs->result, objects_host, max_objects,
                  n_objects, counts);
}

int mh_frame_enqueue_rest_strided(mh_ctx* ctx, const float* q_uv_dev, int Q, const int32_t* gathered_dev, int n_shards,
                                  int shard_stride_words, const mh_cam* cam, const mh_frame_params* prm, uint64_t seed) {
  if (!ctx || shard_stride_words < 3 * Q) return MH_ERR_ARG;
  return enqueue_rest(ctx, q_uv_dev, Q, gathered_dev, n_shards, shard_stride_words, 0, 0, cam, prm, seed);
}

int mh_frame_enqueue_rest_batch(mh_ctx* ctx, const float* q_uv_dev, int Q, const int32_t* gathered_dev, int n_shards,
                                int shard_stride_words, int plane_stride_words, int slot, const mh_cam* cam,
                                const mh_frame_params* prm, uint64_t seed) {
  if (!ctx || slot < 0 || slot >= MH_MAX_BATCH || plane_stride_words < Q || shard_stride_words < 3 * plane_stride_words)
    return MH_ERR_ARG;
  return enqueue_rest(ctx, q_uv_dev, Q, gathered_dev, n_shards, shard_stride_words, plane_stride_words, slot, cam, prm, seed);
}

int mh_frame_enqueue_rest_frames(mh_ctx* ctx, const float* q_uv_dev, int Q, const int32_t* gathered_dev, int n_shards,
                                 int shard_stride_words, int plane_stride_words, int B, const mh_cam* cam,
                                 const mh_frame_params* prm, const uint64_t* seeds) {
  if (!ctx || Q <= 0 || !q_uv_dev || !gathered_dev || n_shards <= 0 || !cam || !prm || !seeds || B < 1 || B > MH_MAX_BATCH ||
      plane_stride_words < Q || shard_stride_words < 3 * plane_stride_words)
    return MH_ERR_ARG;
  if (int rc_fd = filter_depth_frame_ok(ctx, "mh_frame_enqueue_rest_frames", prm, 1, true)) return rc_fd;
  if (int rc_enter = mh::enter(ctx)) return rc_enter;
  const bool merge = B > 1 && merged_batch_ok(ctx, prm);
// ... 248 lines not shown
```

### moped_amd/csrc/context.h

```cpp
#pragma once
#include <cmath>
#include <cstring>
#include <memory>
#include <mutex>
#include <string>
#include <vector>

#include "common.h"
#include "devbuf.h"
#include "screen.h"
#include "steps.h"

struct DbStore;

struct DbPool {
  std::mutex mu;
  size_t cap_rows = 0;
  int max_models = 0;
  DbStore* spare = nullptr;
  ~DbPool();
};

struct DbStore {
  int device = 0;
// ... 17 lines not shown
  mh::DevBuf<int32_t> model_begin_dev;
  uint64_t generation = 0;
  hipEvent_t ready = nullptr;
  std::shared_ptr<DbPool> pool;
  ~DbStore() {
    if (!ready) return;
    int cur = 0;
    const bool have = hipGetDevice(&cur) == hipSuccess;
    hipSetDevice(device);
    hipEventDestroy(ready);
    if (have) hipSetDevice(cur);
  }
};

inline DbPool::~DbPool() { delete spare; }

inline void retire_store(DbStore* st) {
  if (!st) return;
  std::shared_ptr<DbPool> pool = std::move(st->pool);
  st->pool.reset();
  if (pool) {
    std::lock_guard<std::mutex> lock(pool->mu);
    if (!pool->spare && st->n_blocks <= 1 && st->cap >= pool->cap_rows) {
      pool->spare = st;
      return;
    }
  }
  delete st;
}
inline std::shared_ptr<DbStore> make_store(int device) {
  std::shared_ptr<DbStore> st(new DbStore, retire_store);
  st->device = device;
  return st;
}

inline void screen_from_stats(DbStore* st, const unsigned int h[8]) {
  float dd_max, x_max;
  std::memcpy(&dd_max, &h[0], 4);
  std::memcpy(&x_max, &h[1], 4);
  st->screen.dbh = st->desc_h;
  st->screen.dneg = st->neg_h;
  st->screen.dmax = std::sqrt(dd_max);
  std::memcpy(&st->screen.spread, &h[3], 4);
  st->screen.zero_idx = (int32_t)h[4];
  std::memcpy(&st->screen.zero_d1, &h[5], 4);
  std::memcpy(&st->screen.zero_d2, &h[6], 4);
  st->screen.usable = h[2] == 0 && x_max < 60000.f;
}

struct mh_lane {
  int device = 0;
  std::vector<hipStream_t> streams;
  unsigned next = 0;
  int reserve = 0, low_priority = 0;
};

struct mh_ctx {
  int device = 0;
  int n_cus = 0;
  hipStream_t own_stream = nullptr;
  hipStream_t stream = nullptr;
  std::string err;

  std::shared_ptr<DbStore> store;
  int N = 0, n_models = 0;
  int32_t index_base = 0;
  mh::RowMap rmap;
  float* db_desc = nullptr;
  float* db_norm = nullptr;
  float* db_xyz = nullptr;
  int32_t* db_model = nullptr;
  mh::ScreenDb sdb;
  mh::ScreenBufs sbuf;
  struct ScreenOwn {
    mh::DevBuf<_Float16> qh;
    mh::DevBuf<uint8_t> qbad;
    mh::DevBuf<unsigned char> part;
    mh::DevBuf<float> tau;
    mh::DevBuf<uint2> recs, ovf;
    mh::DevBuf<int32_t> ovf_cnt;
    mh::DevBuf<unsigned int> stats, inc;
  } screen_own;
  int match_mode = -1;
  int pose_split = 1;
  std::shared_ptr<DbPool> pool;
  int db_models_reserved = 0;
  struct HeldStore {
    std::shared_ptr<DbStore> store;
    hipEvent_t done = nullptr;
  };
  std::vector<HeldStore> held;
  std::vector<hipEvent_t> held_events;
  mh::DevBuf<float> db_stage;
  struct Planar {
    mh::DevBuf<float> desc, xy;
    mh::DevBuf<float> rows_desc, rows_xyz;
    mh::DevBuf<int32_t> words;
    mh::DevBuf<float> box;
    mh::DevBuf<int32_t> stats;
    mh::DevBuf<float> qn, qnorm, m_d1, m_d2;
    mh::DevBuf<int32_t> m_idx;
  } planar;
  int db_edit_route = 0;
  hipEvent_t db_ev[2] = {nullptr, nullptr};
  bool db_ev_valid = false;
  uint32_t match_launches[3] = {0, 0, 0};
  struct mh_lane* lane = nullptr;
  hipStream_t lane_stream = nullptr;
  hipEvent_t lane_in = nullptr, lane_out = nullptr;

  int max_q = 0, max_clusters = 0, max_objects = 0;
  mh::DevBuf<float> q_desc;
  mh::DevBuf<float> q_norm;
  mh::DevBuf<float> q_uv;
  mh::DevBuf<int32_t> nn_idx;
  mh::DevBuf<float> nn_d1;
  mh::DevBuf<float> nn_d2;
  mh::DevBuf<mh::Top2> match_scratch;
  mh::DevBuf<float> match_pack;

  mh::DevBuf<unsigned char> scratch;
  mh::PinBuf<unsigned char> pinned;
  hipStream_t wb_stream = nullptr;
  hipEvent_t wb_ev = nullptr;
  bool wb_pending = false;

  struct StepState {
    int done = -1;
    int Q = 0, M = 0;
    int n_clusters = 0;
    int n_slots = 0;
    mh_cam cam;
    std::vector<int32_t> model_off;
    std::vector<int32_t> valid;
    std::vector<int32_t> valid_model;
  } step;

  struct FrameState* fs = nullptr;
  struct SiftState* sift = nullptr;
  struct UndistortState* und = nullptr;
  bool und_on = false;
  float und_dist[4] = {0, 0, 0, 0};
  int32_t* feat_count_dev = nullptr;
  mh::DevBuf<int32_t> img_counts;
  int feat_expected = 0;
  int feat_last = -1;
  const float4* batch_img[MH_MAX_BATCH] = {};
  const float* batch_fill[MH_MAX_BATCH] = {};
  int batch_imgs = 0;
  const int32_t* exchange_tags = nullptr;

  struct Exchange {
    mh::DevBuf<int32_t> local;
    mh::DevBuf<int32_t> gathered;
    size_t stride = 0;
    int world = 0, batch = 0, bq = 0;
    mh::DevBuf<unsigned char> flush;
    std::vector<int32_t> host;
  } ex;

  const int32_t* q_img = nullptr;
  mh::DevBuf<int32_t> hf_img;
  mh::DevBuf<mh::DevCam> cams_dev;
  const mh::DevCam* cams_view = nullptr;
  int n_images = 1;

// ... 35 lines not shown
  bool linkage_on = false;
  mh::LinkageParams linkage;
  mh::DevBuf<float> own_depth;
  mh::DevBuf<float> own_fill;
  mh::DevBuf<uint8_t> own_gray;
  mh::DevBuf<unsigned char> own_raw;
  mh::DevBuf<float> lk_scratch;
  mh::DevBuf<unsigned char> df_buf;
  int df_mode = 0;
  int df_lv_frames = 0;
  size_t lk_scratch_limit = (size_t)4 << 30;
  int lk_mode = 0;
  mh::DevBuf<unsigned long long> lk_stats;

  struct FilterDepthState {
    mh::DevBuf<float> pts;
    mh::DevBuf<int32_t> off;
    int n_models = 0;
    int db_models = 0;
    uint64_t db_generation = 0;
    bool on[2] = {false, false};
    mh_filter_depth_params prm[2] = {};
    mh_cam cam = {};
    int debug_form = 0;
  } fdepth;
  int hull_debug_form = 0;
  struct HullState {
    int max_vertices = 0;
    int image = 0;
    mh::DevBuf<unsigned char> block;
    size_t slot_bytes = 0;
    int block_vertices = 0;
    mh::DevBuf<float2> scratch;
    const DbStore* scratch_store = nullptr;
    uint64_t scratch_generation = 0;
    int slot_vertices[MH_MAX_BATCH] = {};
    hipEvent_t done = nullptr;
    bool pending = false;
  } hulls;
  int32_t frame_route[4] = {0, 0, 0, 0};

  struct Delivery {
    hipEvent_t done = nullptr;
    bool pending = false;
    mh::DevBuf<unsigned char> stage;
    unsigned char* host_block = nullptr;
    int B = 0, max_objects = 0;
    uint32_t tag = 0;
  } dlv;

  bool timing = false;
  hipEvent_t ev[10] = {};
  static constexpr int MEV_SETS = 32;
  hipEvent_t mev[MEV_SETS][6] = {};
  int mev_next = 0, mev_used = 0;
  bool ev_made = false;
};

namespace mh {

#define MH_HIP(ctx, call)                                                         \
  do {                                                                            \
    hipError_t e_ = (call);                                                       \
    if (e_ != hipSuccess) {                                                       \
      (ctx)->err = std::string(#call) + ": " + hipGetErrorString(e_);             \
      return MH_ERR_HIP;                                                          \
    }                                                                             \
  } while (0)

int use_stream(mh_ctx* ctx);
void bind_store(mh_ctx* ctx);
void db_poll_held(mh_ctx* ctx, bool wait);
int filter_depth_points_ok(mh_ctx* ctx, const char* who, int n_models);
int filter_depth_frame_ok(mh_ctx* ctx, const char* who, const mh_frame_params* prm, int n_cameras = 1, bool sharded = false);
int hulls_frame_ok(mh_ctx* ctx, const char* who, int n_cameras, bool sharded);
int ensure_frame_buffers(mh_ctx* ctx, int Q);
int ensure_scratch(mh_ctx* ctx, size_t bytes);
int ensure_pinned(mh_ctx* ctx, size_t bytes);
int ensure_own_depth(mh_ctx* ctx, size_t px);
int ensure_match_scratch(mh_ctx* ctx, int Q);
int depth_map_from_raw_own(mh_ctx* ctx, const char* who, const void* raw_host, const mh_raw_depth* raw, const float K[4],
                           int width, int height);
int ctx_match(mh_ctx* ctx, const float* qn, const float* qnorm, int Q, int32_t* idx1, float* d1, float* d2,
              const int32_t* q_count = nullptr, int q_expected = 0);
int delivery_begin(mh_ctx* ctx, void* host_block, size_t bytes, unsigned char** dst_dev);
int delivery_end(mh_ctx* ctx, void* host_block, size_t bytes, unsigned char* dst_dev, int B, int max_objects, uint32_t tag);
int sift_into(mh_ctx* ctx, const uint8_t* gray_dev, int width, int height, int double_size, int cap,
              float* desc_dev, float* xy_dev, int32_t** n_dev_out, int32_t* count_word = nullptr);
int undistort_frame(mh_ctx* ctx, const uint8_t* const* gray_dev, int n, int width, int height, const float K[4],
                    const uint8_t** staged);
int sift_into_batch(mh_ctx* ctx, const uint8_t* const* gray_dev, int n, int width, int height, int double_size, int cap,
                    float* desc_dev, float* xy_dev, int32_t* count_words);
int undistort_frame_images(mh_ctx* ctx, const uint8_t* const* gray_dev, int n, int n_cams, int width, int height,
                           const mh_cam* cams, const float (*dist)[4], const uint8_t** staged);

struct ImagesPackArgs {
  const float* sdesc;
  const float* sxy;
  const int32_t* scount;
  float* desc;
  float* uv;
  int32_t* q_img;
  int32_t* totals;
  int32_t* counts;
  DevCam* cams_dev;
  int cap, n_images;
  DevCam cams[MH_MAX_IMAGES];
};
void launch_images_pack(const ImagesPackArgs& a, int n_frames, hipStream_t s);

struct PlanarArgs {
  const float* desc;
  const float* xy;
  const int32_t* n;
  int cap;
  mh_planar_spec spec;
  int all;
  float* desc_out;
  float* desc_copy;
  float* xyz_out;
  size_t out_pitch;
  int out_cap;
  int32_t* n_out;
  float* bbox;
};
void launch_planar_rows(const PlanarArgs& a, int n_images, hipStream_t s);
int planar_spec_check(mh_ctx* ctx, const char* who, const mh_planar_spec* spec, int* all);
struct ViewArgs {
  const float* desc;
  const float* xy;
  const int32_t* n;
  int cap;
  int w, h;
  mh_view_spec spec;
  int roi_all, box_all, dup_on;
  mh_view_dup dup;
  float* desc_out;
  float* desc_copy;
  float* xyz_out;
  size_t out_pitch;
  int out_cap;
  int32_t* n_out;
  float* bbox;
  int32_t* stats;
  struct View {
    const float4* map;
    const float* fill;
    float pose[7];
  } v[MH_MAX_BATCH];
};
void launch_view_rows(const ViewArgs& a, int n_views, hipStream_t s);
int view_args_check(mh_ctx* ctx, const char* who, const mh_view* views, int n_views, int width, int height,
                    const mh_view_spec* spec, ViewArgs* a);
const int32_t* sift_counters_dev(mh_ctx* ctx, int slot);

}
```

### moped_amd/csrc/match_screen.hip

```cpp
#include <type_traits>
#include <hip/hip_fp16.h>

#include <algorithm>
#include <cstdlib>

#include "common.h"
#include "screen.h"

MH_TRACE_TU()

namespace mh {

namespace {

typedef _Float16 half8 __attribute__((ext_vector_type(8)));
typedef float v16f __attribute__((ext_vector_type(16)));
#define MH_AS1 __attribute__((address_space(1)))
#define MH_AS3 __attribute__((address_space(3)))

constexpr int SC_QPAD = 3 * 1024;
constexpr int SC_TILE = 128;
constexpr int SC_TILE_BYTES = SC_TILE * DIM * 2;
constexpr bool SC_SHAPE16_LARGE = true;
constexpr int SC_NW_LARGE = 8;
__host__ __device__ constexpr int sc_recbuf(int nw) { return nw >= 8 ? 112 : 40; }
constexpr int SC_GROUP = 1;
constexpr int SC_NBUF = 2 * SC_GROUP;
constexpr int SC_DD = 192;
constexpr int SC_LDS_TILES = SC_NBUF * SC_TILE_BYTES + SC_NBUF * SC_DD * 4;
constexpr int SC_REC_BYTES = 80;
__host__ __device__ constexpr int sc_lds_bytes(int nw) { return SC_LDS_TILES + nw * sc_recbuf(nw) * SC_REC_BYTES; }
static_assert(SC_TILE == 128 && DIM == 128, "tile image and chunk swizzle assume 128 x 128");

__host__ __device__ inline float screen_margin(float qq, float dmax) {
  const float nq = sqrtf(fmaxf(qq, 0.f));
  const float E = 0.000978f * nq * dmax + 4e-7f * (nq + dmax) + 3e-5f * (nq * dmax + 0.5f * dmax * dmax);
  return 2.f * E + 2e-6f * (qq + dmax * dmax);
}

__global__ __launch_bounds__(256) void db_to_half_kernel(const float* __restrict__ db, const float* __restrict__ dnorm, int N,
                                                         size_t n_chunks, _Float16* __restrict__ dbh, float* __restrict__ dneg,
                                                         unsigned int* __restrict__ stats) {
  __shared__ unsigned int red[3];
  if (threadIdx.x < 3) red[threadIdx.x] = 0;
  __syncthreads();
  float x_max = 0.f, dd_max = 0.f;
  unsigned int bad = 0;
  for (size_t i = (size_t)blockIdx.x * blockDim.x + threadIdx.x; i < n_chunks; i += (size_t)gridDim.x * blockDim.x) {
    const float4 a = reinterpret_cast<const float4*>(db)[2 * i], b = reinterpret_cast<const float4*>(db)[2 * i + 1];
    half8 h;
    h[0] = (_Float16)a.x; h[1] = (_Float16)a.y; h[2] = (_Float16)a.z; h[3] = (_Float16)a.w;
    h[4] = (_Float16)b.x; h[5] = (_Float16)b.y; h[6] = (_Float16)b.z; h[7] = (_Float16)b.w;
    reinterpret_cast<half8*>(dbh)[i] = h;
    const int row = (int)(i >> 4);
    if ((i & 15) == 0) dneg[(size_t)(row >> 7) * SC_DD + (row & 127)] = -0.5f * dnorm[row];
    if (row < N) {
      x_max = fmaxf(x_max, fmaxf(fmaxf(fmaxf(fabsf(a.x), fabsf(a.y)), fmaxf(fabsf(a.z), fabsf(a.w))),
                                 fmaxf(fmaxf(fabsf(b.x), fabsf(b.y)), fmaxf(fabsf(b.z), fabsf(b.w)))));
      if ((i & 15) == 0) {
        const float dd = dnorm[row];
        if (!(dd >= 0.f) || dd == __builtin_inff()) bad = 1;
        else dd_max = fmaxf(dd_max, dd);
      }
    }
  }
  atomicMax(&red[0], __float_as_uint(dd_max));
  atomicMax(&red[1], __float_as_uint(x_max));
  if (bad) atomicOr(&red[2], 1u);
  __syncthreads();
  if (threadIdx.x == 0) {
    atomicMax(&stats[0], red[0]);
    atomicMax(&stats[1], red[1]);
    if (red[2]) atomicOr(&stats[2], 1u);
  }
}

__global__ void db_block_bounds_kernel(const float* __restrict__ dnorm, int N, int n_tiles, float* __restrict__ dneg,
                                       unsigned int* __restrict__ stats) {
  const int b = blockIdx.x * blockDim.x + threadIdx.x;
  if (b >= n_tiles * 4) return;
  float hi = -__builtin_inff(), lo = __builtin_inff();
  for (int r = 0; r < 32; ++r) {
    const int row = b * 32 + r;
    const float v = row < N ? -0.5f * dnorm[row] : -__builtin_inff();
    if (row < N) hi = fmaxf(hi, v);
    lo = fminf(lo, v);
  }
  float* t = dneg + (size_t)(b >> 2) * SC_DD;
  t[128 + (b & 3)] = hi;
  t[132 + (b & 3)] = lo;
  if (b * 32 + 32 <= N && hi - lo >= 0.f) atomicMax(&stats[3], __float_as_uint(hi - lo));
  if ((b & 3) == 0)
    for (int i = 136; i < SC_DD; ++i) t[i] = 0.f;
}

__global__ __launch_bounds__(1024) void db_zero_query_kernel(const float* __restrict__ dnorm, int N, unsigned int* __restrict__ stats) {
  __shared__ float s1[1024], s2[1024];
  __shared__ int si[1024];
  float b1 = __builtin_inff(), b2 = __builtin_inff();
  int i1 = -1;
  for (int r = threadIdx.x; r < N; r += 1024) {
    const float d = fmaxf(dnorm[r], 0.f);
    if (d < b1 || i1 < 0) {
      if (i1 >= 0) b2 = fminf(b2, b1);
      b1 = d;
      i1 = r;
    } else {
      b2 = fminf(b2, d);
    }
  }
  s1[threadIdx.x] = b1;
  s2[threadIdx.x] = b2;
  si[threadIdx.x] = i1;
  __syncthreads();
  for (int st = 512; st > 0; st >>= 1) {
    if ((int)threadIdx.x < st) {
      const float o1 = s1[threadIdx.x + st], o2 = s2[threadIdx.x + st];
      const int oi = si[threadIdx.x + st];
      float a1 = s1[threadIdx.x], a2 = s2[threadIdx.x];
      int ai = si[threadIdx.x];
// ... 825 lines not shown
          const int pnb = (nb + NQB - 1) % NQB;
          v4f acc[2][2] = {{zero4, zero4}, {zero4, zero4}};
          float m0 = -__builtin_inff(), m1 = -__builtin_inff();
          const float t0 = tau_lds[pnb * 32 + l16], t1 = tau_lds[pnb * 32 + 16 + l16];
#pragma unroll
          for (int s = 0; s < 4; ++s) {
#pragma unroll
            for (int ti = 0; ti < 2; ++ti)
#pragma unroll
              for (int tj = 0; tj < 2; ++tj)
                acc[ti][tj] = __builtin_amdgcn_mfma_f32_16x16x32_f16(a[ti][s], bq[nb][tj][s], acc[ti][tj], 0, 0, 0);
            if (s == 2) m0 = max8(pend[0][0], pend[1][0]);
            if (s == 3) m1 = max8(pend[0][1], pend[1][1]);
          }
          __builtin_amdgcn_sched_group_barrier(0x008, 8, 0);
#pragma unroll
          for (int g = 0; g < 8; ++g) {
            __builtin_amdgcn_sched_group_barrier(0x008, 1, 0);
            __builtin_amdgcn_sched_group_barrier(0x002, 2, 0);
          }
          __builtin_amdgcn_sched_barrier(0);
          {
            const float thr0 = t0 - pend_hi, thr1 = t1 - pend_hi;
            emit_block(m0 > thr0, m1 > thr1, pend, pnb, pend_row0, m0, m1, thr0, thr1);
          }
          __builtin_amdgcn_sched_barrier(0);
#pragma unroll
          for (int ti = 0; ti < 2; ++ti)
#pragma unroll
            for (int tj = 0; tj < 2; ++tj) pend[ti][tj] = acc[ti][tj];
          pend_row0 = row0;
          pend_hi = hi[rb];
        }
      }
    }
    if (more) asm volatile("s_waitcnt vmcnt(0)" ::: "memory");
    __syncthreads();
    side ^= 1;
  }
  }
  if (MODE == 1) {
    {
      const float m0 = max8(pend[0][0], pend[1][0]), m1 = max8(pend[0][1], pend[1][1]);
      const float thr0 = tau_lds[(NQB - 1) * 32 + l16] - pend_hi, thr1 = tau_lds[(NQB - 1) * 32 + 16 + l16] - pend_hi;
      emit_block(m0 > thr0, m1 > thr1, pend, NQB - 1, pend_row0, m0, m1, thr0, thr1);
    }
    flush_parked();
  }
  if (MODE == 0) {
#pragma unroll
    for (int nb = 0; nb < NQB; ++nb)
#pragma unroll
      for (int tj = 0; tj < 2; ++tj) {
        const int q = q0 + nb * 32 + 16 * tj + l16;
        if (q < A.q_pad) {
#pragma unroll
          for (int k = 0; k < SC_PART5; ++k) A.part5[((size_t)(split * 4 + quarter) * SC_PART5 + k) * A.q_pad + q] = pk[nb][tj][k];
        }
      }
  }
}

struct Best {
  float b1, b2;
  int i1;
};
__device__ __forceinline__ void take(Best& a, float d, int row) {
  const bool better = d < a.b1 || (d == a.b1 && a.i1 >= 0 && row < a.i1);
  const float lose = better ? a.b1 : d;
  a.b2 = fminf(a.b2, lose);
  a.b1 = better ? d : a.b1;
  a.i1 = better ? row : a.i1;
}
__device__ __forceinline__ void merge(Best& a, float ob1, float ob2, int oi1) {
  const bool take_o = (ob1 < a.b1) || (ob1 == a.b1 && (unsigned)oi1 < (unsigned)a.i1);
  const float lose1 = take_o ? a.b1 : ob1;
  const float s2 = fminf(a.b2, ob2);
  a.b2 = fminf(lose1, s2);
  a.b1 = take_o ? ob1 : a.b1;
  a.i1 = take_o ? oi1 : a.i1;
}

constexpr int RS_WAVES = 4;
#ifdef MH_EXPERIMENTS
constexpr int RS_WAVES_FAT = 16;
constexpr int RS_FAT_K = 2;
#endif
constexpr int RS_MAXC = 1024;
constexpr int RS_STAGE = 8;
static_assert(RS_STAGE * DIM * 4 <= RS_MAXC * 4 && RS_STAGE % 2 == 0 && RS_STAGE <= 32, "staged rows live in the candidate list's LDS");

__device__ __forceinline__ float exact_dist(const float* __restrict__ q_lds, const float* __restrict__ row, float nq, float dn) {
  float s = 0.f;
  const float4* r4 = reinterpret_cast<const float4*>(row);
#pragma unroll 2
  for (int c = 0; c < DIM / 16; ++c) {
    const float4 x0 = r4[4 * c], x1 = r4[4 * c + 1], x2 = r4[4 * c + 2], x3 = r4[4 * c + 3];
    const float4 y0 = *reinterpret_cast<const float4*>(q_lds + 16 * c), y1 = *reinterpret_cast<const float4*>(q_lds + 16 * c + 4);
    const float4 y2 = *reinterpret_cast<const float4*>(q_lds + 16 * c + 8), y3 = *reinterpret_cast<const float4*>(q_lds + 16 * c + 12);
    s = fmaf(y0.x, x0.x, s); s = fmaf(y0.y, x0.y, s); s = fmaf(y0.z, x0.z, s); s = fmaf(y0.w, x0.w, s);
    s = fmaf(y1.x, x1.x, s); s = fmaf(y1.y, x1.y, s); s = fmaf(y1.z, x1.z, s); s = fmaf(y1.w, x1.w, s);
    s = fmaf(y2.x, x2.x, s); s = fmaf(y2.y, x2.y, s); s = fmaf(y2.z, x2.z, s); s = fmaf(y2.w, x2.w, s);
    s = fmaf(y3.x, x3.x, s); s = fmaf(y3.y, x3.y, s); s = fmaf(y3.z, x3.z, s); s = fmaf(y3.w, x3.w, s);
  }
  return fmaxf(fmaf(-2.f, s, nq + dn), 0.f);
}

__device__ __forceinline__ void wave_lds_sync() {
  __builtin_amdgcn_fence(__ATOMIC_RELEASE, "wavefront");
  __builtin_amdgcn_wave_barrier();
  __builtin_amdgcn_fence(__ATOMIC_ACQUIRE, "wavefront");
}

__device__ __forceinline__ v4f sample_pair_values(const float* __restrict__ q_lds, const _Float16* __restrict__ dbh,
                                                  const float* __restrict__ dneg, int row0x, int row0y, int lane) {
  const int g = lane >> 4, i = lane & 15;
  const int arow = (i < 8 ? row0x : row0y) + (i & 3) + 16 * ((i >> 2) & 1);
  const half8* ap = reinterpret_cast<const half8*>(dbh + (size_t)arow * DIM + 8 * g);
  half8 a[4];
#pragma unroll
  for (int s = 0; s < 4; ++s) a[s] = ap[4 * s];
  const int crow = (g < 2 ? row0x : row0y) + 16 * (g & 1);
  const float4 c = *reinterpret_cast<const float4*>(dneg + (size_t)(crow >> 7) * SC_DD + (crow & 127));
  v4f acc = {c.x, c.y, c.z, c.w};
#pragma unroll
  for (int s = 0; s < 4; ++s) {
    const float4 y0 = *reinterpret_cast<const float4*>(q_lds + 32 * s + 8 * g), y1 = *reinterpret_cast<const float4*>(q_lds + 32 * s + 8 * g + 4);
    half8 b;
    b[0] = (_Float16)y0.x; b[1] = (_Float16)y0.y; b[2] = (_Float16)y0.z; b[3] = (_Float16)y0.w;
    b[4] = (_Float16)y1.x; b[5] = (_Float16)y1.y; b[6] = (_Float16)y1.z; b[7] = (_Float16)y1.w;
    acc = __builtin_amdgcn_mfma_f32_16x16x32_f16(a[s], b, acc, 0, 0, 0);
  }
  return acc;
}

constexpr int RS_ITERS = (SC_SLOT_PITCH + SCREEN_OVF_CAP + 63) / 64;
struct RsScalars {
  int bad;
  float nq, tau_q;
  int n_ovf;
  unsigned incw;
  float2 qv;
};
constexpr size_t rs_lds_bytes(int waves) { return (size_t)waves * (DIM * 4 + RS_MAXC * 4 + SC_SA_SLOTS * 4 + 8); }

struct RsArgs {
  const float* qn;
  const float* qnorm;
  const uint8_t* qbad;
  int Q;
  const int32_t* q_count;
  const float* db;
  const float* dnorm;
  int N;
  RowMap rmap;
  uint2* recs;
  int n_slots;
  int32_t* ovf_cnt;
  uint2* ovf;
  int ovf_cap;
  float dmax;
  const float* tau;
  float spread;
  int32_t* idx1;
  float* d1;
  float* d2;
  unsigned int* stats;
  int32_t zero_idx;
  float zero_d1, zero_d2;
  SampleGeom g;
  const unsigned int* inc;
  unsigned int* inc_count;
  const _Float16* dbh;
  const float* dneg;
};
typedef const __attribute__((address_space(4))) RsArgs* RsArgsPtr;
__device__ __forceinline__ RsArgsPtr rs_args() {
  RsArgsPtr p = (RsArgsPtr)__builtin_amdgcn_kernarg_segment_ptr();
  asm volatile("" : "+s"(p));
  return p;
}

constexpr int RS_ITERS_C = (SC_SLOT_PITCH + 63) / 64;
template <int COMPACT>
__device__ __forceinline__ void rs_load_slots(const uint2* recs, int n_slots, int sa_slots, int q, int lane, uint2 (&rv)[RS_ITERS]) {
  const uint2* theirs = recs + (size_t)q * SC_SLOT_PITCH;
  if (COMPACT) {
    rv[0] = theirs[lane];
#pragma unroll
    for (int it = 1; it < RS_ITERS; ++it) rv[it] = make_uint2(0u, 0u);
    return;
  }
  const int n_own = n_slots + sa_slots;
#pragma unroll
  for (int it = 0; it < RS_ITERS; ++it) {
    const int j = it * 64 + lane;
    rv[it] = j < n_own ? theirs[j < n_slots ? j : SC_SLOTS_MAX + (j - n_slots)] : make_uint2(0u, 0u);
  }
}
#define RS_CONST(T, p) ((const __attribute__((address_space(4))) T*)(p))
__device__ __forceinline__ RsScalars rs_load_scalars(const uint8_t* qbad, const float* qnorm, const float* tau, const int32_t* ovf_cnt,
                                                     const unsigned int* inc, const float* qn, int q, int lane) {
  RsScalars v;
  v.qv = reinterpret_cast<const float2*>(qn + (size_t)q * DIM)[lane];
  v.n_ovf = RS_CONST(int32_t, ovf_cnt)[q];
  const unsigned w = RS_CONST(unsigned int, inc ? inc : reinterpret_cast<const unsigned int*>(tau))[q];
  v.bad = (RS_CONST(unsigned int, qbad)[q >> 2] >> (8 * (q & 3))) & 0xFFu;
  v.nq = RS_CONST(float, qnorm)[q];
  v.tau_q = RS_CONST(float, tau)[q];
  v.incw = inc ? w : 0u;
  return v;
}

static_assert(RS_ITERS_C <= RS_ITERS, "a counted list's slots fit the registers the scan has");
template <int COMPACT>
__device__ __forceinline__ void rescore_query(
    int q, int lane, float* q_sw, int* cand_sw, int* samp_sw, int* ncand_sw, int* nsamp_sw, uint2 (&recv)[RS_ITERS], const RsScalars sc, int Qe,
    const float* __restrict__ db, const float* __restrict__ dnorm, int N,
    RowMap rmap, uint2* __restrict__ recs, int n_slots, int32_t* __restrict__ ovf_cnt, uint2* __restrict__ ovf,
    int ovf_cap, float dmax, float spread, int32_t* __restrict__ idx1, float* __restrict__ d1, float* __restrict__ d2,
    unsigned int* __restrict__ stats, int32_t zero_idx, float zero_d1, float zero_d2, SampleGeom g,
    unsigned int* __restrict__ inc_count, const _Float16* __restrict__ dbh, const float* __restrict__ dneg) {
  uint2* mine = recs + (size_t)q * SC_SLOT_PITCH;
  const int n_own = COMPACT ? min(sc.n_ovf, SC_SLOT_PITCH) : n_slots + g.sa_slots;
  auto slot_at = [&](int j) -> uint2& { return mine[COMPACT || j < n_slots ? j : SC_SLOTS_MAX + (j - n_slots)]; };
  const int bad = sc.bad;
  const float nq = sc.nq;
  const float tau_q = sc.tau_q;
  const int n_ovf = sc.n_ovf;
  const unsigned incw = sc.incw;
  const float2 qv = sc.qv;
  asm volatile("" ::"v"(bad), "v"(nq), "v"(tau_q), "v"(n_ovf), "v"(incw), "v"(qv.x), "v"(qv.y), "s"(Qe));
  if (q >= Qe) {
    if (lane == 0) {
      idx1[q] = -1;
      d1[q] = __builtin_inff();
      d2[q] = __builtin_inff();
    }
    return;
  }
  if (bad == 2) {
    if (lane == 0) {
      idx1[q] = -1;
      d1[q] = __builtin_inff();
      d2[q] = __builtin_inff();
    }
    return;
  }
  if (bad == 3) {
    if (lane == 0) {
      idx1[q] = zero_idx >= 0 ? row_to_global(rmap, zero_idx) : -1;
      d1[q] = zero_d1;
      d2[q] = zero_d2;
      if (stats) stats[3 * q + 2] += 1u;
    }
    return;
  }
  wave_lds_sync();
  if (lane == 0) {
    *ncand_sw = 0;
    *nsamp_sw = 0;
  }
  q_sw[2 * lane] = qv.x;
  q_sw[2 * lane + 1] = qv.y;
  bool brute = n_ovf > (COMPACT ? SC_SLOT_PITCH : ovf_cap) || bad == 1;
  int n_cand = 0;
  if (!brute) {
    float l1 = -__builtin_inff(), l2 = -__builtin_inff();
    const float pert = screen_pack_pert(nq, dmax, g.pack_bits);
    auto bounds = [tau_q, spread, N, dmax, pert](uint2 rec, float& lo, float& hi) {
      if (rec.x & SC_REC_SAMPLE) screen_sample_bounds((unsigned short)(rec.y >> 16), tau_q, pert, dmax, lo, hi);
      else screen_record_bounds((unsigned short)(rec.y >> 16), rec.x & 0x3FFFFFFFu, tau_q, spread, N, dmax, lo, hi);
    };
    const bool more = COMPACT && n_own > 64;
    if (more) {
#pragma unroll
      for (int it = 1; it < RS_ITERS_C; ++it) {
        const int j = it * 64 + lane;
        recv[it] = j < n_own ? mine[j] : make_uint2(0u, 0u);
      }
    }
    auto scan = [&](int it) {
      const int j = it * 64 + lane;
      uint2 rec = recv[it];
      if (COMPACT) {
        if (j < n_own) mine[j] = make_uint2(0u, 0u);
        else rec = make_uint2(0u, 0u);
      } else if (j < n_own) {
        if (rec.y) slot_at(j) = make_uint2(0u, 0u);
      } else if (j < n_own + n_ovf) {
        rec = ovf[(size_t)q * ovf_cap + (j - n_own)];
      }
      recv[it] = rec;
      if (rec.y & 0xFFFFu) {
        float lo, hi;
        bounds(rec, lo, hi);
        l2 = fmaxf(l2, fminf(l1, lo));
        l1 = fmaxf(l1, lo);
      }
    };
    if (COMPACT) {
      scan(0);
      if (more) {
#pragma unroll
        for (int it = 1; it < RS_ITERS_C; ++it) scan(it);
      }
    } else {
#pragma unroll
      for (int it = 0; it < RS_ITERS; ++it) scan(it);
    }
#pragma unroll
    for (int d = 1; d < 64; d <<= 1) {
      const float o1 = __shfl_xor(l1, d), o2 = __shfl_xor(l2, d);
      l2 = fmaxf(fmaxf(l2, o2), fminf(l1, o1));
      l1 = fmaxf(l1, o1);
    }
    const float keep_from = l2 - screen_margin(nq, dmax);
    auto keep = [&](int it) {
      const uint2 rec = recv[it];
      unsigned bits = rec.y & 0xFFFFu;
      if (bits) {
        float lo, hi;
        bounds(rec, lo, hi);
        if (hi < keep_from) bits = 0;
      }
      const int hi_stride = (rec.x & 0x80000000u) ? 16 : 8;
      const int row0 = (int)(rec.x & 0x3FFFFFFFu);
      if (bits && (rec.x & SC_REC_SAMPLE)) {
        const int w = atomicAdd(nsamp_sw, 1);
        if (w < SC_SA_SLOTS) samp_sw[w] = row0;
        bits = 0;
      }
      while (bits) {
        const int r = __builtin_ctz(bits);
        bits &= bits - 1;
        const int w = atomicAdd(ncand_sw, 1);
        if (w < RS_MAXC) cand_sw[w] = row0 + (r & 3) + hi_stride * (r >> 2);
      }
    };
    if (COMPACT) {
      keep(0);
      if (more) {
#pragma unroll
        for (int it = 1; it < RS_ITERS_C; ++it) keep(it);
      }
    } else {
#pragma unroll
      for (int it = 0; it < RS_ITERS; ++it) keep(it);
    }
    wave_lds_sync();
    const int n_samp = min(*nsamp_sw, SC_SA_SLOTS), n_pad_rows = (N + SC_TILE - 1) / SC_TILE * SC_TILE;
    for (int p = 0; p < n_samp; p += 2) {
      const bool pair = p + 1 < n_samp;
      const int rx = samp_sw[p], ry = samp_sw[pair ? p + 1 : p];
      if (rx + 19 >= n_pad_rows || ry + 19 >= n_pad_rows) continue;
      const v4f w = sample_pair_values(q_sw, dbh, dneg, rx, ry, lane);
      const int grp = lane >> 4;
      if ((lane & 15) == 0 && (grp < 2 || pair)) {
        const int base = (grp < 2 ? rx : ry) + 16 * (grp & 1);
#pragma unroll
        for (int r = 0; r < 4; ++r)
          if (w[r] > tau_q) {
            const int at = atomicAdd(ncand_sw, 1);
            if (at < RS_MAXC) cand_sw[at] = base + r;
          }
      }
    }
    if (n_samp) wave_lds_sync();
    n_cand = *ncand_sw;
    if (n_cand > RS_MAXC) brute = true;
  } else if (COMPACT ? n_ovf > 0 : n_ovf > ovf_cap) {
    for (int j = lane; j < n_own; j += 64) slot_at(j) = make_uint2(0u, 0u);
  }
  if (n_ovf && lane == 0) ovf_cnt[q] = 0;
  wave_lds_sync();

  Best best = {__builtin_inff(), __builtin_inff(), -1};
  const int n_rows = brute ? N : n_cand;
  if (!brute && n_cand <= 64) {
    const int my_row = lane < n_cand ? cand_sw[lane] : -1;
    const bool my_ok = my_row >= 0 && my_row < N;
    const float my_dn = my_ok ? dnorm[my_row] : 0.f;
    wave_lds_sync();
    float4* stage = reinterpret_cast<float4*>(cand_sw);
    const int n_st = min(n_cand, RS_STAGE);
    const int half = lane >> 5, c = lane & 31;
    float4 v[RS_STAGE / 2];
#pragma unroll
    for (int i = 0; i < RS_STAGE / 2; ++i) {
      const int r = 2 * i + half;
      const int row_r = __shfl(my_row, r);
      v[i] = make_float4(0.f, 0.f, 0.f, 0.f);
      if (r < n_st && row_r >= 0 && row_r < N) v[i] = reinterpret_cast<const float4*>(db + (size_t)row_r * DIM)[c];
    }
#pragma unroll
    for (int i = 0; i < RS_STAGE / 2; ++i) {
      const int r = 2 * i + half;
      if (r < n_st) stage[r * 32 + (c ^ r)] = v[i];
    }
    wave_lds_sync();
    if (lane < n_st) {
      if (my_ok) {
        float sdot = 0.f;
        const float4* qs4 = reinterpret_cast<const float4*>(q_sw);
#pragma unroll 8
        for (int k = 0; k < 32; ++k) {
          const float4 x = stage[lane * 32 + (k ^ lane)], y = qs4[k];
          sdot = fmaf(y.x, x.x, sdot); sdot = fmaf(y.y, x.y, sdot); sdot = fmaf(y.z, x.z, sdot); sdot = fmaf(y.w, x.w, sdot);
        }
        take(best, fmaxf(fmaf(-2.f, sdot, nq + my_dn), 0.f), my_row);
      }
    } else if (my_ok) {
      take(best, exact_dist(q_sw, db + (size_t)my_row * DIM, nq, my_dn), my_row);
    }
  } else {
    for (int k = lane; k < n_rows; k += 64) {
      const int row = brute ? k : cand_sw[k];
      if (row >= 0 && row < N) take(best, exact_dist(q_sw, db + (size_t)row * DIM, nq, dnorm[row]), row);
    }
  }
  if (incw && !brute) {
    for (unsigned sm = incw & 0x0FFFFFFFu; sm; sm &= sm - 1) {
      const int split = __builtin_ctz(sm);
      const int sel0 = split * g.tiles_base + min(split, g.tiles_rem);
      const int sel1 = min(sel0 + g.tiles_base + (split < g.tiles_rem ? 1 : 0), g.n_sel);
      for (int k = sel0 * SC_TILE + lane; k < sel1 * SC_TILE; k += 64) {
        const int row = (g.tile_first + (k >> 7) * g.tile_stride) * SC_TILE + (k & 127);
        if (((incw >> (28 + ((k & 15) >> 2))) & 1u) && row < N)
          take(best, exact_dist(q_sw, db + (size_t)row * DIM, nq, dnorm[row]), row);
      }
    }
    if (lane == 0 && inc_count) atomicAdd(inc_count, 1u);
  }
#pragma unroll
  for (int d = 1; d < 64; d <<= 1) {
    const float ob1 = __shfl_xor(best.b1, d), ob2 = __shfl_xor(best.b2, d);
    const int oi1 = __shfl_xor(best.i1, d);
    if (oi1 >= 0) merge(best, ob1, ob2, oi1);
  }
  if (lane == 0) {
    idx1[q] = best.i1 >= 0 ? row_to_global(rmap, best.i1) : -1;
    d1[q] = best.b1;
    d2[q] = best.b2;
    if (stats) {
      stats[3 * q] += (unsigned)n_cand;
      stats[3 * q + 1] += brute ? 1u : 0u;
      stats[3 * q + 2] += 1u;
    }
  }
}

template <int WAVES, int PF, int COMPACT>
__global__ __launch_bounds__(64 * WAVES) __attribute__((amdgpu_waves_per_eu(WAVES == 12 ? 6 : 8, WAVES == 12 ? 6 : 8))) void rescore_kernel(const RsArgs args) {
  MH_TRACE_SCOPE(mh::TK_PASS_C);
  extern __shared__ __attribute__((aligned(16))) unsigned char rs_lds[];
  const int lane0 = threadIdx.x & 63;
  const int wave0 = __builtin_amdgcn_readfirstlane(threadIdx.x >> 6);
  const int q_first = blockIdx.x * WAVES + wave0, q_stride = (int)gridDim.x * WAVES;
  if (q_first >= args.Q) return;
  const int Qe = args.q_count ? min(args.Q, *RS_CONST(int32_t, args.q_count)) : args.Q;
  uint2 recv_next[RS_ITERS];
  RsScalars sc_next = {};
  if (PF >= 1) rs_load_slots<COMPACT>(args.recs, args.n_slots, args.g.sa_slots, q_first, lane0, recv_next);
  if (PF >= 2) sc_next = rs_load_scalars(args.qbad, args.qnorm, args.tau, args.ovf_cnt, args.inc, args.qn, q_first, lane0);
  for (int q = q_first;; q += q_stride) {
    int lane = lane0, wave = wave0;
    asm volatile("" : "+v"(lane), "+s"(wave));
    float* const q_sw = reinterpret_cast<float*>(rs_lds) + wave * DIM;
    int* const cand_sw = reinterpret_cast<int*>(rs_lds + (size_t)WAVES * DIM * 4) + wave * RS_MAXC;
    int* const samp_sw = reinterpret_cast<int*>(rs_lds + (size_t)WAVES * (DIM + RS_MAXC) * 4) + wave * SC_SA_SLOTS;
    int* const ncand_sw = reinterpret_cast<int*>(rs_lds + (size_t)WAVES * (DIM + RS_MAXC + SC_SA_SLOTS) * 4) + wave;
    int* const nsamp_sw = ncand_sw + WAVES;
    const RsArgsPtr A = rs_args();
    const int Q = A->Q;
    if (q >= Q) break;
    uint2 recv[RS_ITERS];
    if (PF >= 1) {
#pragma unroll
      for (int it = 0; it < RS_ITERS; ++it) recv[it] = recv_next[it];
    } else {
      rs_load_slots<COMPACT>(A->recs, A->n_slots, A->g.sa_slots, q, lane, recv);
    }
    const RsScalars sc = PF >= 2 ? sc_next : rs_load_scalars(A->qbad, A->qnorm, A->tau, A->ovf_cnt, A->inc, A->qn, q, lane);
    if (PF >= 1 && q + q_stride < Q) {
      rs_load_slots<COMPACT>(A->recs, A->n_slots, A->g.sa_slots, q + q_stride, lane, recv_next);
      if (PF >= 2) sc_next = rs_load_scalars(A->qbad, A->qnorm, A->tau, A->ovf_cnt, A->inc, A->qn, q + q_stride, lane);
    }
    RowMap rmap;
    rmap.glo = A->rmap.glo;
    rmap.llo = A->rmap.llo;
    rmap.nb = A->rmap.nb;
    rmap.base = A->rmap.base;
    const SampleGeom g = {A->g.sa_slots, A->g.pack_bits, A->g.tile_first, A->g.tile_stride, A->g.tiles_base, A->g.tiles_rem, A->g.n_sel};
    rescore_query<COMPACT>(q, lane, q_sw, cand_sw, samp_sw, ncand_sw, nsamp_sw, recv, sc, Qe, A->db, A->dnorm, A->N, rmap, A->recs,
                  A->n_slots, A->ovf_cnt, A->ovf, A->ovf_cap, A->dmax, A->spread, A->idx1, A->d1, A->d2, A->stats, A->zero_idx,
                  A->zero_d1, A->zero_d2, g, A->inc_count, A->dbh, A->dneg);
  }
}
static_assert(std::is_same<decltype(&rescore_kernel<RS_WAVES, 0, 0>), void (*)(RsArgs)>::value,
              "rs_args() reads RsArgs from offset 0 of the kernel argument segment: it must stay the only parameter");

__global__ __launch_bounds__(64) void screen_values_kernel(const _Float16* __restrict__ qh, const _Float16* __restrict__ dbh,
                                                           const float* __restrict__ dneg, int n_rows, float* __restrict__ out,
                                                           int shape16) {
  const int lane = threadIdx.x, half = lane >> 5, l32 = lane & 31;
  const int q0 = blockIdx.x * 32, r0 = blockIdx.y * 32;
  if (shape16) {
    const int quarter = lane >> 4, l16 = lane & 15;
#pragma unroll
    for (int ti = 0; ti < 2; ++ti)
#pragma unroll
      for (int tj = 0; tj < 2; ++tj) {
        v4f acc;
#pragma unroll
        for (int r = 0; r < 4; ++r) {
          const int row = r0 + 16 * ti + 4 * quarter + r;
          acc[r] = dneg[(size_t)(row >> 7) * SC_DD + (row & 127)];
        }
#pragma unroll
        for (int s = 0; s < 4; ++s) {
          const half8 a = *reinterpret_cast<const half8*>(dbh + (size_t)(r0 + 16 * ti + l16) * DIM + 32 * s + 8 * quarter);
          const half8 b = *reinterpret_cast<const half8*>(qh + (size_t)(q0 + 16 * tj + l16) * DIM + 32 * s + 8 * quarter);
          acc = __builtin_amdgcn_mfma_f32_16x16x32_f16(a, b, acc, 0, 0, 0);
        }
#pragma unroll
        for (int r = 0; r < 4; ++r) out[(size_t)(q0 + 16 * tj + l16) * n_rows + r0 + 16 * ti + 4 * quarter + r] = acc[r];
      }
    return;
  }
  half8 a[8], b[8];
  const _Float16* arow = dbh + (size_t)(r0 + l32) * DIM + 8 * half;
  const _Float16* brow = qh + (size_t)(q0 + l32) * DIM + 8 * half;
#pragma unroll
  for (int s = 0; s < 8; ++s) {
    a[s] = *reinterpret_cast<const half8*>(arow + 16 * s);
    b[s] = *reinterpret_cast<const half8*>(brow + 16 * s);
  }
  v16f acc;
#pragma unroll
  for (int r = 0; r < 16; ++r) {
    const int row = r0 + (r & 3) + 8 * (r >> 2) + 4 * half;
    acc[r] = dneg[(size_t)(row >> 7) * SC_DD + (row & 127)];
  }
#pragma unroll
  for (int s = 0; s < 8; ++s) acc = __builtin_amdgcn_mfma_f32_32x32x16_f16(a[s], b[s], acc, 0, 0, 0);
#pragma unroll
  for (int r = 0; r < 16; ++r) out[(size_t)(q0 + l32) * n_rows + r0 + (r & 3) + 8 * (r >> 2) + 4 * half] = acc[r];
}

__global__ __launch_bounds__(64) void screen_sample_values_kernel(const float* __restrict__ qn, const _Float16* __restrict__ dbh,
                                                                  const float* __restrict__ dneg, const int32_t* __restrict__ row0,
                                                                  float* __restrict__ out) {
  __shared__ __attribute__((aligned(16))) float q_s[DIM];
  const int lane = threadIdx.x, q = blockIdx.x;
  const float2 qv = reinterpret_cast<const float2*>(qn + (size_t)q * DIM)[lane];
  q_s[2 * lane] = qv.x;
  q_s[2 * lane + 1] = qv.y;
  __syncthreads();
  const v4f w = sample_pair_values(q_s, dbh, dneg, row0[2 * q], row0[2 * q + 1], lane);
  if ((lane & 15) == 0)
#pragma unroll
    for (int r = 0; r < 4; ++r) out[(size_t)q * 16 + 4 * (lane >> 4) + r] = w[r];
}

}

#ifdef SC_PROF
extern "C" int mh_debug_screen_trace(unsigned long long* out ) {
  return hipMemcpyFromSymbol(out, HIP_SYMBOL(g_sc_trace), 2 * 1024 * sizeof(unsigned long long)) == hipSuccess ? 0 : -1;
}
extern "C" int mh_debug_screen_prof(unsigned long long out[8], int reset, int ablate) {
  if (hipMemcpyFromSymbol(out, HIP_SYMBOL(g_sc_prof), 8 * sizeof(unsigned long long)) != hipSuccess) return -1;
  if (reset) {
    unsigned long long z[8] = {};
    if (hipMemcpyToSymbol(HIP_SYMBOL(g_sc_prof), z, sizeof z) != hipSuccess) return -1;
  }
  g_sc_ablate = ablate;
  return 0;
}
#endif
#ifdef MH_EXPERIMENTS
extern "C" long long mh_debug_screen_direct_appends(int reset) {
  unsigned long long v = 0, z = 0;
  if (hipMemcpyFromSymbol(&v, HIP_SYMBOL(g_sc_direct_appends), sizeof v) != hipSuccess) return -1;
  if (reset && hipMemcpyToSymbol(HIP_SYMBOL(g_sc_direct_appends), &z, sizeof z) != hipSuccess) return -1;
  return (long long)v;
}
#endif

float screen_margin_host(float qq, float dmax) { return screen_margin(qq, dmax); }

size_t screen_db_half_elems(int N) { return ((size_t)N + SC_TILE - 1) / SC_TILE * SC_TILE * DIM; }
size_t screen_dneg_elems(int N) { return ((size_t)N + SC_TILE - 1) / SC_TILE * SC_DD; }

void launch_db_to_half(const float* db, const float* dnorm, int N, _Float16* dbh, float* dneg, unsigned int* stats,
                       hipStream_t s) {
  const size_t n_chunks = screen_db_half_elems(N) / 8;
  if (n_chunks == 0) return;
  const unsigned blocks = (unsigned)std::min<size_t>((n_chunks + 255) / 256, 2048);
  hipLaunchKernelGGL(db_to_half_kernel, dim3(blocks), dim3(256), 0, s, db, dnorm, N, n_chunks, dbh, dneg, stats);
  launch_db_aggregates(dnorm, N, dneg, stats, s);
}

void launch_db_aggregates(const float* dnorm, int N, float* dneg, unsigned int* stats, hipStream_t s) {
  const int n_tiles = (N + SC_TILE - 1) / SC_TILE;
  if (n_tiles == 0) return;
  hipLaunchKernelGGL(db_block_bounds_kernel, dim3((n_tiles * 4 + 255) / 256), dim3(256), 0, s, dnorm, N, n_tiles, dneg, stats);
  hipLaunchKernelGGL(db_zero_query_kernel, dim3(1), dim3(1024), 0, s, dnorm, N, stats);
}

void launch_screen_values(const _Float16* qh, int Q, const ScreenDb& sdb, int n_rows, float* out, hipStream_t s, int shape) {
  if (Q <= 0 || n_rows <= 0) return;
  const int shape16 = shape == 2 || (shape == 0 && SC_SHAPE16_LARGE);
  hipLaunchKernelGGL(screen_values_kernel, dim3(Q / 32, n_rows / 32), dim3(64), 0, s, qh, sdb.dbh, sdb.dneg, n_rows, out, shape16);
}
void launch_screen_sample_values(const float* qn, int Q, const ScreenDb& sdb, const int32_t* row0, float* out, hipStream_t s) {
  if (Q <= 0) return;
  hipLaunchKernelGGL(screen_sample_values_kernel, dim3(Q), dim3(64), 0, s, qn, sdb.dbh, sdb.dneg, row0, out);
}
void launch_screen_prepare(const float* qn, const float* qnorm, int Q, int q_pad, _Float16* qh, uint8_t* qbad, hipStream_t s) {
  hipLaunchKernelGGL(screen_prepare_kernel, dim3((q_pad * 16 + 255) / 256), dim3(256), 0, s, qn, qnorm, Q, (const int32_t*)nullptr,
                     q_pad, qh, qbad);
}

size_t screen_rec_slots() { return SC_SLOT_PITCH; }
int screen_park_places() { return SC_RECBUF16; }

int screen_q_pad(int Q) { return (Q + SC_QPAD - 1) / SC_QPAD * SC_QPAD; }
int screen_max_splits_a() { return 64; }
size_t screen_part_bytes(int q_pad) {
  return (size_t)q_pad * std::max<size_t>(screen_max_splits_a() * sizeof(float2), (size_t)SC_SA_SPLITS_MAX * 4 * SC_PART5 * sizeof(float));
}

bool screen_wanted(int q_expected, int N, int mode) {
  static const int pinned = exp_int("MH_MATCH_SCREEN", -1);
  if (mode < 0) mode = pinned;
  if (mode == 0 || N < 4096) return false;
  if (mode == 1) return true;
  return (double)q_expected * (double)N >= 8e6;
}

namespace {

template <int NQB, int NW>
void launch_passes(ScreenArgs a, int Q, int qe, int n_tiles, int sample, int blocks_a, int blocks_b, int* n_slots_out,
                   hipEvent_t* ev, hipStream_t s, int cu_avail) {
  constexpr int QB = 32 * NQB * NW;
  constexpr int SC_THREADS = 64 * NW, SC_LDS_BYTES = sc_lds_bytes(NW);
  static DynLds attr0, attr1;
  attr0.ensure(screen_kernel<0, NQB, NW>, SC_LDS_BYTES);
  attr1.ensure(screen_kernel<1, NQB, NW>, SC_LDS_BYTES);
  blocks_a *= 8 / NW;
  (void)cu_avail;
  const int nqb = (Q + QB - 1) / QB;
  const int nqb_e = (qe + QB - 1) / QB;
  auto splits_for = [&](int n_sel, int target, int s_max) {
    int S = std::max(1, target / nqb_e);
    S = std::min(std::min(S, n_sel), s_max);
    if (S >= 8 && (S / 8 * 8) * 33 >= S * 32) S = S / 8 * 8;
    return std::max(S, 1);
  };
  const int every = sample == 8 && n_tiles < 256 ? 4 : sample;
  const int stride = n_tiles >= 4 * every ? every : 1;
  const int n_sel_a = (n_tiles + stride - 1) / stride;
  const int Sa = splits_for(n_sel_a, blocks_a, screen_max_splits_a());
  a.n_sel = n_sel_a;
  a.tile_first = std::min(stride / 2, n_tiles - 1 - (n_sel_a - 1) * stride);
  if (a.tile_first < 0) a.tile_first = 0;
  a.tile_stride = stride;
  a.n_splits = Sa;
  a.tiles_base = n_sel_a / Sa;
  a.tiles_rem = n_sel_a % Sa;
  a.n_splits_a = Sa;
// ... 46 lines not shown
  const int blocks_slot = 4 * ((p.n_sel_a + p.Sa - 1) / p.Sa);
  int bits = 2;
  while ((1 << bits) < blocks_slot) ++bits;
  p.onesweep = onesweep_on && p.stride > 1 && bits <= SC_PACK_BITS_MAX;
  p.pack_bits = p.onesweep ? bits : 0;
  constexpr int SB16_MAX = SC_SLOTS_MAX / 12;
  p.n_sel_b = p.onesweep ? n_tiles - p.n_sel_a : n_tiles;
  p.Sb = 1;
  if (blocks_b > 0) {
    p.Sb = std::min(splits_for(p.n_sel_b, blocks_b, SC_SLOTS_MAX / 4), SB16_MAX);
  } else {
    double best = 1e30;
    for (int c = 1; c <= std::min(SB16_MAX, std::max(1, p.n_sel_b / 8)); ++c) {
      const double cost = (double)((nqb_e * c + 255) / 256) * (double)((p.n_sel_b + c - 1) / c);
      if (cost <= best) {
        best = cost;
        p.Sb = c;
      }
    }
  }
  return p;
}

template <int NQB>
void launch_passes16(ScreenArgs a, int Q, int qe, int n_tiles, int sample, int blocks_a, int blocks_b, int* n_slots_out,
                     SampleGeom* geom_out, unsigned int* inc, hipEvent_t* ev, hipStream_t s) {
  constexpr int QB = 32 * NQB * 8;
  static DynLds attr0, attr1;
  attr0.ensure(screen16_kernel<0, NQB>, SC_LDS16_BYTES);
  attr1.ensure(screen16_kernel<1, NQB>, SC_LDS16_BYTES);
  const int nqb = (Q + QB - 1) / QB;
  const Plan16 p = plan_passes16<NQB>(qe, n_tiles, sample, blocks_a, blocks_b);
  a.n_sel = p.n_sel_a;
  a.tile_first = p.tile_first;
  a.tile_stride = p.stride;
  a.n_splits = p.Sa;
  a.tiles_base = p.n_sel_a / p.Sa;
  a.tiles_rem = p.n_sel_a % p.Sa;
  a.n_splits_a = p.Sa;
  a.pack_keep = ~((1u << p.pack_bits) - 1u);
  a.skip_first = a.skip_stride = 0;
  hipLaunchKernelGGL((screen16_kernel<0, NQB>), dim3(nqb * p.Sa), dim3(512), SC_LDS16_BYTES, s, a);
  if (ev) hipEventRecord(ev[2], s);
  SampleGeom g = {p.onesweep ? SC_SA_SLOTS : 0, p.pack_bits, a.tile_first, a.tile_stride, a.tiles_base, a.tiles_rem, a.n_sel};
  static_assert(SC_SA_SPLITS_MAX <= 2 * HO_PARTS_MAX, "a thread of screen_handover_kernel holds at most 8 lane slots");
  if (p.Sa <= HO_PARTS_MAX)
    hipLaunchKernelGGL(screen_handover_kernel<4>, dim3((a.q_pad + 63) / 64), dim3(64, p.Sa), 0, s, (const float*)a.part5, 4 * p.Sa,
                       a.q_pad, a.Q, a.q_count, a.qnorm, a.qbad, a.dmax, g, const_cast<float*>(a.tau), a.recs, a.ovf_cnt, inc);
  else
    hipLaunchKernelGGL(screen_handover_kernel<8>, dim3((a.q_pad + 63) / 64), dim3(64, (p.Sa + 1) / 2), 0, s, (const float*)a.part5,
                       4 * p.Sa, a.q_pad, a.Q, a.q_count, a.qnorm, a.qbad, a.dmax, g, const_cast<float*>(a.tau), a.recs, a.ovf_cnt, inc);
#ifdef MH_EXPERIMENTS
  if (exp_int("MH_SCREEN_NO_HITS", 0)) hipMemsetAsync(const_cast<float*>(a.tau), 0x7f, (size_t)a.q_pad * sizeof(float), s);
#endif
  if (ev) hipEventRecord(ev[3], s);
  a.n_sel = p.n_sel_b;
  a.tile_first = 0;
  a.tile_stride = 1;
  a.skip_first = p.onesweep ? p.tile_first : 0;
  a.skip_stride = p.onesweep ? p.stride : 0;
  a.n_splits = p.Sb;
  a.tiles_base = p.n_sel_b / p.Sb;
  a.tiles_rem = p.n_sel_b % p.Sb;
#ifdef MH_EXPERIMENTS
  static const int places = exp_int("MH_SCREEN_PLACES", 0);
  static DynLds attr_p1, attr_p2, attr_p3;
  if (places == 3) {
    attr_p3.ensure(screen16_kernel<1, NQB, 3>, SC_LDS16_BYTES);
    hipLaunchKernelGGL((screen16_kernel<1, NQB, 3>), dim3(nqb * p.Sb), dim3(512), SC_LDS16_BYTES, s, a);
  } else if (places == 1) {
    attr_p1.ensure(screen16_kernel<1, NQB, 1>, SC_LDS16_BYTES);
    hipLaunchKernelGGL((screen16_kernel<1, NQB, 1>), dim3(nqb * p.Sb), dim3(512), SC_LDS16_BYTES, s, a);
  } else if (places == 2) {
    attr_p2.ensure(screen16_kernel<1, NQB, 2>, SC_LDS16_BYTES);
    hipLaunchKernelGGL((screen16_kernel<1, NQB, 2>), dim3(nqb * p.Sb), dim3(512), SC_LDS16_BYTES, s, a);
  } else
#endif
  hipLaunchKernelGGL((screen16_kernel<1, NQB>), dim3(nqb * p.Sb), dim3(512), SC_LDS16_BYTES, s, a);
  if (ev) hipEventRecord(ev[4], s);
  *n_slots_out = 0;
  *geom_out = g;
}

template <int WAVES, int PF, int COMPACT>
void launch_pass_c_layout(int grid, hipStream_t s, const RsArgs& args) {
  static DynLds attr;
  attr.ensure(rescore_kernel<WAVES, PF, COMPACT>, rs_lds_bytes(WAVES));
  hipLaunchKernelGGL((rescore_kernel<WAVES, PF, COMPACT>), dim3(grid), dim3(64 * WAVES), rs_lds_bytes(WAVES), s, args);
}
template <int WAVES, int PF>
void launch_pass_c(int grid, hipStream_t s, const RsArgs& args, bool compact) {
  if (compact) launch_pass_c_layout<WAVES, PF, 1>(grid, s, args);
  else launch_pass_c_layout<WAVES, PF, 0>(grid, s, args);
}

struct ShapeChoice {
  int nqb_sel;
  bool passes16;
};
ShapeChoice choose_shape(int qe, int n_tiles) {
  static const int nqb_pin = exp_int("MH_SCREEN_NQB", 0);
  int nqb_sel = qe > 640 ? 2 : 1;
  if (qe >= 2048 && (long)n_tiles * ((qe + 1023) / 1024) >= 16L * 256) nqb_sel = 4;
  if (nqb_pin >= 1 && nqb_pin <= 4) nqb_sel = nqb_pin;
  static const int shape_pin = exp_int("MH_SCREEN_SHAPE", 0);
  const bool shape16 = shape_pin == 2 || (shape_pin == 0 && SC_SHAPE16_LARGE);
  const bool p16 = shape16 && ((nqb_sel == 4 && (shape_pin == 2 || (qe + 1023) / 1024 >= 12)) || (nqb_sel == 2 && shape_pin == 2));
  return {nqb_sel, p16};
}

int screen_sample_every() {
  static const int sample = std::max(1, exp_int("MH_SCREEN_SAMPLE", 8));
  return sample;
}

}

void screen_launch_plan(int Q, int q_expected, int N, int out[8]) {
  const int qe = (q_expected > 0 && q_expected < Q) ? std::max(q_expected, std::min(Q, 256)) : Q;
  const int n_tiles = (N + SC_TILE - 1) / SC_TILE;
  for (int k = 0; k < 8; ++k) out[k] = 0;
  const ShapeChoice shape = choose_shape(qe, n_tiles);
  if (!shape.passes16) return;
  const int blocks_b = std::max(0, exp_int("MH_SCREEN_BLOCKS", 0)), blocks_a = std::max(1, exp_int("MH_SCREEN_BLOCKS_A", 256));
  const Plan16 p = shape.nqb_sel == 4 ? plan_passes16<4>(qe, n_tiles, screen_sample_every(), blocks_a, blocks_b)
                                      : plan_passes16<2>(qe, n_tiles, screen_sample_every(), blocks_a, blocks_b);
  const int v[8] = {p.onesweep ? 1 : 0, p.tile_first, p.stride, p.n_sel_a, p.Sa, p.pack_bits, p.Sb, p.n_sel_b};
  for (int k = 0; k < 8; ++k) out[k] = v[k];
}

void launch_match_screen(const float* qn, const float* qnorm, int Q, const float* db, const float* dnorm, int N,
                         const RowMap& rmap, const ScreenDb& sdb, const ScreenBufs& sb, int32_t* idx1, float* d1,
                         float* d2, hipStream_t s, const int32_t* q_count, int q_expected) {
  const int sample = screen_sample_every();
  static const int blocks_b = std::max(0, exp_int("MH_SCREEN_BLOCKS", 0));
  static const int blocks_a = std::max(1, exp_int("MH_SCREEN_BLOCKS_A", 256));
  const int q_pad = screen_q_pad(Q);
  const int qe = (q_expected > 0 && q_expected < Q) ? std::max(q_expected, std::min(Q, 256)) : Q;
  const int n_tiles = (N + SC_TILE - 1) / SC_TILE;

  if (sb.ev) hipEventRecord(sb.ev[0], s);
  hipLaunchKernelGGL(screen_prepare_kernel, dim3((q_pad * 16 + 255) / 256), dim3(256), 0, s, qn, qnorm, Q, q_count, q_pad,
                     sb.qh, sb.qbad);
  hipStream_t sbig = s;
  if (sb.big && sb.ev_in && sb.ev_out) {
    hipEventRecord(sb.ev_in, s);
    hipStreamWaitEvent(sb.big, sb.ev_in, 0);
    sbig = sb.big;
  }
  if (sb.ev) hipEventRecord(sb.ev[1], sbig);
  ScreenArgs a;
  a.qh = sb.qh;
  a.dbh = sdb.dbh;
  a.dneg = sdb.dneg;
  a.qnorm = qnorm;
  a.qbad = sb.qbad;
  a.q_count = q_count;
  a.part = sb.part;
  a.part5 = reinterpret_cast<float*>(sb.part);
  a.pack_keep = ~0u;
  a.skip_first = a.skip_stride = 0;
  a.tau = sb.tau;
  a.recs = sb.recs;
  a.ovf_cnt = sb.ovf_cnt;
  a.ovf = sb.ovf;
  a.ovf_cap = sb.ovf_cap;
  a.sub_cap = 1;
  a.Q = Q;
  a.q_pad = q_pad;
  a.dmax = sdb.dmax;
#ifdef SC_PROF
  a.ablate = g_sc_ablate;
#else
  a.ablate = 0;
#endif
  const ShapeChoice shape = choose_shape(qe, n_tiles);
  const int nqb_sel = shape.nqb_sel;
  int n_slots = 0;
  SampleGeom geom = {0, 0, 0, 1, 0, 0, 0};
  static const int nw_pin = exp_int("MH_SCREEN_NW", 0);
  const int nw_sel = nw_pin == 4 || nw_pin == 8 ? nw_pin : (nqb_sel == 4 ? SC_NW_LARGE : 8);
  if (shape.passes16 && nqb_sel == 4) launch_passes16<4>(a, Q, qe, n_tiles, sample, blocks_a, blocks_b, &n_slots, &geom, sb.inc, sb.ev, sbig);
  else if (shape.passes16) launch_passes16<2>(a, Q, qe, n_tiles, sample, blocks_a, blocks_b, &n_slots, &geom, sb.inc, sb.ev, sbig);
  else if (nqb_sel == 4 && nw_sel == 4) launch_passes<4, 4>(a, Q, qe, n_tiles, sample, blocks_a, blocks_b, &n_slots, sb.ev, sbig, 256);
  else if (nqb_sel == 4) launch_passes<4, 8>(a, Q, qe, n_tiles, sample, blocks_a, blocks_b, &n_slots, sb.ev, sbig, 256);
  else if (nqb_sel == 3) launch_passes<3, 8>(a, Q, qe, n_tiles, sample, blocks_a, blocks_b, &n_slots, sb.ev, sbig, 256);
  else if (nqb_sel == 2 && nw_sel == 4) launch_passes<2, 4>(a, Q, qe, n_tiles, sample, blocks_a, blocks_b, &n_slots, sb.ev, sbig, 256);
  else if (nqb_sel == 2) launch_passes<2, 8>(a, Q, qe, n_tiles, sample, blocks_a, blocks_b, &n_slots, sb.ev, sbig, 256);
  else launch_passes<1, 8>(a, Q, qe, n_tiles, sample, blocks_a, blocks_b, &n_slots, sb.ev, sbig, 256);
  if (sbig != s) {
    hipEventRecord(sb.ev_out, sbig);
    hipStreamWaitEvent(s, sb.ev_out, 0);
  }
  RsArgs ca;
  ca.qn = qn; ca.qnorm = qnorm; ca.qbad = sb.qbad; ca.Q = Q; ca.q_count = q_count; ca.db = db; ca.dnorm = dnorm; ca.N = N;
  ca.rmap = rmap; ca.recs = sb.recs; ca.n_slots = n_slots; ca.ovf_cnt = sb.ovf_cnt; ca.ovf = sb.ovf; ca.ovf_cap = sb.ovf_cap;
  ca.dmax = sdb.dmax; ca.tau = sb.tau; ca.spread = sdb.spread; ca.idx1 = idx1; ca.d1 = d1; ca.d2 = d2; ca.stats = sb.stats;
  ca.zero_idx = sdb.zero_idx; ca.zero_d1 = sdb.zero_d1; ca.zero_d2 = sdb.zero_d2; ca.g = geom;
  ca.inc = geom.sa_slots > 0 ? sb.inc : nullptr; ca.inc_count = sb.inc ? sb.inc + sb.q_pad : nullptr; ca.dbh = sdb.dbh; ca.dneg = sdb.dneg;
#ifdef MH_EXPERIMENTS
  static const int pc_waves = exp_int("MH_PASSC_WAVES", RS_WAVES), pc_k = exp_int("MH_PASSC_K", RS_FAT_K);
  static const int pc_pf = exp_int("MH_PASSC_PREFETCH", 0), pc_all = exp_int("MH_PASSC_FAT_ALL", 0);
  const int n_cus = sb.n_cus > 0 ? sb.n_cus : 256;
  const int fat_waves = pc_waves == 12 ? 12 : RS_WAVES_FAT;
  if (pc_waves != RS_WAVES && (pc_all || Q > RS_FAT_K * n_cus * RS_WAVES_FAT)) {
    const int cover = (Q + fat_waves - 1) / fat_waves, grid = pc_k > 0 ? std::min(cover, pc_k * n_cus) : cover;
    if (fat_waves == 12 && pc_pf == 0) launch_pass_c<12, 0>(grid, s, ca, shape.passes16);
    else if (fat_waves == 12 && pc_pf == 1) launch_pass_c<12, 1>(grid, s, ca, shape.passes16);
    else if (fat_waves == 12) launch_pass_c<12, 2>(grid, s, ca, shape.passes16);
    else if (pc_pf == 0) launch_pass_c<RS_WAVES_FAT, 0>(grid, s, ca, shape.passes16);
    else if (pc_pf == 1) launch_pass_c<RS_WAVES_FAT, 1>(grid, s, ca, shape.passes16);
    else launch_pass_c<RS_WAVES_FAT, 2>(grid, s, ca, shape.passes16);
  } else
#endif
  launch_pass_c<RS_WAVES, 0>((Q + RS_WAVES - 1) / RS_WAVES, s, ca, shape.passes16);
  if (sb.ev) hipEventRecord(sb.ev[5], s);
}

}
```

### moped_amd/csrc/screen.h

```cpp
#pragma once
#include <hip/hip_fp16.h>
#include <hip/hip_runtime.h>
#include <stdint.h>

namespace mh {

struct ScreenDb {
  const _Float16* dbh = nullptr;
  const float* dneg = nullptr;
  float dmax = 0.f;
  float spread = __builtin_inff();
  bool usable = false;
  int32_t zero_idx = -1;
  float zero_d1 = __builtin_inff(), zero_d2 = __builtin_inff();
};

struct ScreenBufs {
  _Float16* qh = nullptr;
  uint8_t* qbad = nullptr;
  float2* part = nullptr;
  float* tau = nullptr;
  uint2* recs = nullptr;
  int32_t* ovf_cnt = nullptr;
  uint2* ovf = nullptr;
  int ovf_cap = 0, q_pad = 0;
  hipEvent_t* ev = nullptr;
  hipStream_t big = nullptr;
  hipEvent_t ev_in = nullptr, ev_out = nullptr;
  unsigned int* stats = nullptr;
  unsigned int* inc = nullptr;
  int n_cus = 0;
};

__host__ __device__ inline unsigned short screen_record_value(float top, float thr) {
  const _Float16 h = (_Float16)(top - thr);
  unsigned short b;
  __builtin_memcpy(&b, &h, 2);
  return b;
}
__host__ __device__ inline void screen_record_bounds(unsigned short value_bits, unsigned row0, float tau_q, float spread, int N,
                                                     float dmax, float& lo, float& hi) {
  _Float16 h;
  __builtin_memcpy(&h, &value_bits, 2);
  const float dv = (float)h;
  const float eps = fabsf(dv) * 0.001f + 1e-6f + 4e-7f * (fabsf(tau_q) + 0.5f * dmax * dmax);
  const bool fin = fabsf(dv) < 6.0e4f && fabsf(tau_q) < 1e30f;
  const bool whole = (int)(row0 | 31u) < N;
  hi = fin ? tau_q + dv + eps : __builtin_inff();
  lo = fin && whole && spread < 1e30f ? tau_q + dv - spread - eps : -__builtin_inff();
}

__host__ __device__ inline float screen_pack_value(float v, unsigned id, int bits) {
  const unsigned keep = ~((1u << bits) - 1u);
  unsigned u;
  __builtin_memcpy(&u, &v, 4);
  u = (u & keep) | (id & ~keep);
  __builtin_memcpy(&v, &u, 4);
  return v;
}
__host__ __device__ inline float screen_pack_pert(float qq, float dmax, int bits) {
  const float nq = sqrtf(fmaxf(qq, 0.f));
  const float W = 1.01f * (nq * dmax + 0.5f * dmax * dmax) + 4e-7f * (nq + dmax) + 1e-30f;
  return W * ldexpf(1.f, bits - 23);
}
__host__ __device__ inline void screen_sample_bounds(unsigned short value_bits, float tau_q, float pert, float dmax, float& lo,
                                                     float& hi) {
  _Float16 h;
  __builtin_memcpy(&h, &value_bits, 2);
  const float dv = (float)h;
  const float eps = fabsf(dv) * 0.001f + 1e-6f + 4e-7f * (fabsf(tau_q) + 0.5f * dmax * dmax);
  const bool fin = fabsf(dv) < 6.0e4f && fabsf(tau_q) < 1e30f;
  hi = fin ? tau_q + dv + eps + pert : __builtin_inff();
  lo = fin ? tau_q + dv - eps - pert : -__builtin_inff();
}

constexpr int SCREEN_OVF_CAP = 64;
size_t screen_rec_slots();

float screen_margin_host(float qq, float dmax);
void launch_screen_values(const _Float16* qh, int Q, const ScreenDb& sdb, int n_rows, float* out, hipStream_t s, int shape);
void launch_screen_sample_values(const float* qn, int Q, const ScreenDb& sdb, const int32_t* row0, float* out, hipStream_t s);
void launch_screen_prepare(const float* qn, const float* qnorm, int Q, int q_pad, _Float16* qh, uint8_t* qbad, hipStream_t s);
size_t screen_db_half_elems(int N);
size_t screen_dneg_elems(int N);
void launch_db_to_half(const float* db, const float* dnorm, int N, _Float16* dbh, float* dneg, unsigned int* stats,
                       hipStream_t s);
void launch_db_aggregates(const float* dnorm, int N, float* dneg, unsigned int* stats, hipStream_t s);
int screen_q_pad(int Q);
int screen_max_splits_a();
size_t screen_part_bytes(int q_pad);
void screen_launch_plan(int Q, int q_expected, int N, int out[8]);
int screen_park_places();
bool screen_wanted(int q_expected, int N, int mode = -1);
void launch_match_screen(const float* qn, const float* qnorm, int Q, const float* db, const float* dnorm, int N,
                         const RowMap& rmap, const ScreenDb& sdb, const ScreenBufs& sb, int32_t* idx1, float* d1,
                         float* d2, hipStream_t s, const int32_t* q_count, int q_expected);

}
```

Measured before the change: 17180.

## Prove ratio-test rejection from screen bounds and skip exact rescoring

The frame's ratio threshold is passed into the screen matcher's rescore pass. Using the coarse screening bounds (the upper bound on the best similarity and the lower bound on the second), the pass checks whether the ratio test must fail; if it must, the query is marked unmatched without the exact fp32 rescoring of its candidates. The ACCEPT variant runs with one wave per block and a one-query-per-wave grid instead of the default shape. It is on by default for whole-frame paths without a ratio table, and adds a device-side counter of pre-rejected queries. The proof depends on conservative error margins, and the changed launch shape could cost throughput for queries that are not rejected.

```diff
diff --git a/include/moped_hip.h b/include/moped_hip.h
--- a/include/moped_hip.h
+++ b/include/moped_hip.h
@@ -74,6 +74,9 @@
 void mh_screen_launch_plan(int Q, int q_expected, int N, int32_t out[8]);
 int mh_screen_park_places(void);
 int mh_match_incomplete(mh_ctx* ctx, uint32_t* count, int reset);
+int mh_screen_reject_proved(float qq, float dmax, float h1, float l2, float tau, float ratio);
+int mh_match_set_accept(mh_ctx* ctx, float ratio);
+int mh_match_prerejected(mh_ctx* ctx, uint32_t* count, int reset);
 int mh_screen_sample_values(mh_ctx* ctx, const float* q_host, int Q, const int32_t* row0_host, float* out_host);
 int mh_match_query_candidates(mh_ctx* ctx, int Q, uint32_t* out);
 
diff --git a/moped_amd/capi.py b/moped_amd/capi.py
--- a/moped_amd/capi.py
+++ b/moped_amd/capi.py
@@ -223,6 +223,7 @@
     "mh_object_hulls", "mh_hull_debug_form",
     "mh_frame_set_hulls", "mh_frame_fetch_hulls_slot", "mh_frame_fetch_hulls", "mh_frame_hull_block_stride",
     "mh_frame_fetch_batch_hulls_async",
+    "mh_screen_reject_proved", "mh_match_set_accept", "mh_match_prerejected",
 ]
 COMM_ID_BYTES = 128
 EX2_OBJECTS = 62
@@ -431,6 +432,10 @@
         L.mh_screen_launch_plan.argtypes = [i32, i32, i32, vp]
         L.mh_screen_launch_plan.restype = None
         L.mh_match_incomplete.argtypes = [vp, C.POINTER(C.c_uint32), i32]
+    if hasattr(L, "mh_screen_reject_proved"):
+        L.mh_screen_reject_proved.argtypes = [f32, f32, f32, f32, f32, f32]
+        L.mh_match_set_accept.argtypes = [vp, f32]
+        L.mh_match_prerejected.argtypes = [vp, C.POINTER(C.c_uint32), i32]
     if hasattr(L, "mh_screen_sample_values"):
         L.mh_screen_sample_values.argtypes = [vp, vp, i32, vp, vp]
         L.mh_match_query_candidates.argtypes = [vp, i32, vp]
@@ -997,6 +1002,14 @@
         self._ck(self.L.mh_match_incomplete(self.h, C.byref(n), int(reset)), "mh_match_incomplete")
         return int(n.value)
 
+    def match_set_accept(self, ratio: float):
+        self._ck(self.L.mh_match_set_accept(self.h, float(ratio)), "mh_match_set_accept")
+
+    def match_prerejected(self, reset=False) -> int:
+        n = C.c_uint32(0)
+        self._ck(self.L.mh_match_prerejected(self.h, C.byref(n), int(reset)), "mh_match_prerejected")
+        return int(n.value)
+
     def normalize(self, desc):
         d = np.ascontiguousarray(desc, np.float32).copy()
         self._ck(self.L.mh_normalize(self.h, _ptr(d), d.shape[0]), "mh_normalize")
diff --git a/moped_amd/csrc/api.hip b/moped_amd/csrc/api.hip
--- a/moped_amd/csrc/api.hip
+++ b/moped_amd/csrc/api.hip
@@ -72,8 +72,9 @@
     MH_HIP(ctx, o.ovf_cnt.ensure(qp, s));
     MH_HIP(ctx, o.ovf.ensure(qp * SCREEN_OVF_CAP, s));
     MH_HIP(ctx, o.stats.ensure(qp * 3, s));
-    MH_HIP(ctx, o.inc.ensure(qp + 1, s));
-    MH_HIP(ctx, hipMemsetAsync(o.inc, 0, (qp + 1) * sizeof(unsigned int), s));
+    const size_t inc_words = qp + 1 + (size_t)screen_prerej_words();
+    MH_HIP(ctx, o.inc.ensure(inc_words, s));
+    MH_HIP(ctx, hipMemsetAsync(o.inc, 0, inc_words * sizeof(unsigned int), s));
     MH_HIP(ctx, hipMemsetAsync(o.recs, 0, slots * sizeof(uint2), s));
     MH_HIP(ctx, hipMemsetAsync(o.ovf_cnt, 0, qp * sizeof(int32_t), s));
     MH_HIP(ctx, hipMemsetAsync(o.stats, 0, qp * 3 * sizeof(unsigned int), s));
@@ -93,7 +94,7 @@
 }
 
 int ctx_match(mh_ctx* ctx, const float* qn, const float* qnorm, int Q, int32_t* idx1, float* d1, float* d2,
-              const int32_t* q_count, int q_expected) {
+              const int32_t* q_count, int q_expected, float accept_ratio) {
   if (Q <= 0) return MH_OK;
   int rc = ensure_match_scratch(ctx, Q);
   if (rc) return rc;
@@ -111,6 +112,7 @@
     ctx->sbuf.n_cus = ctx->n_cus;
     ctx->sbuf.ev_in = ctx->lane_in;
     ctx->sbuf.ev_out = ctx->lane_out;
+    ctx->sbuf.accept_ratio = accept_ratio > 0.f ? accept_ratio : 0.f;
     launch_match_screen(qn, qnorm, Q, ctx->db_desc, ctx->db_norm, ctx->N, ctx->rmap, ctx->sdb, ctx->sbuf, idx1, d1,
                         d2, ctx->stream, q_count, q_expected);
     ++ctx->match_launches[2];
@@ -508,7 +510,9 @@
     launch_normalize(ctx->q_desc, ctx->q_norm, Q, ctx->stream);
   else
     launch_row_norms(ctx->q_desc, ctx->q_norm, Q, ctx->stream);
-  if ((rc = ctx_match(ctx, ctx->q_desc, ctx->q_norm, Q, ctx->nn_idx, ctx->nn_d1, ctx->nn_d2))) return rc;
+  if ((rc = ctx_match(ctx, ctx->q_desc, ctx->q_norm, Q, ctx->nn_idx, ctx->nn_d1, ctx->nn_d2, nullptr, 0,
+                      ctx->match_accept > 0.f ? ctx->match_accept : 0.f)))
+    return rc;
   int32_t* d_acc = (int32_t*)ctx->scratch.p;
   launch_accept(ctx->nn_idx, ctx->nn_d1, ctx->nn_d2, Q, ratio, d_acc, ctx->stream);
   MH_HIP(ctx, hipGetLastError());
@@ -567,6 +571,10 @@
 
 float mh_screen_margin(float qq, float dmax) { return screen_margin_host(qq, dmax); }
 
+int mh_screen_reject_proved(float qq, float dmax, float h1, float l2, float tau_q, float ratio) {
+  return screen_reject_proved_host(qq, dmax, h1, l2, tau_q, ratio) ? 1 : 0;
+}
+
 uint16_t mh_screen_record_value(float top, float thr) { return screen_record_value(top, thr); }
 
 void mh_screen_record_bounds(uint16_t value_bits, uint32_t row0, float tau, float spread, int N, float dmax, float* lo,
@@ -684,6 +692,28 @@
   return rc;
 }
 
+int mh_match_set_accept(mh_ctx* ctx, float ratio) {
+  if (!ctx || !(ratio == ratio) || ratio > 1e30f) return MH_ERR_ARG;
+  ctx->match_accept = ratio;
+  return MH_OK;
+}
+
+int mh_match_prerejected(mh_ctx* ctx, uint32_t* count, int reset) {
+  if (!ctx || !count) return MH_ERR_ARG;
+  MH_HIP(ctx, hipSetDevice(ctx->device));
+  if (int rc_stream = mh::use_stream(ctx)) return rc_stream;
+  MH_HIP(ctx, hipStreamSynchronize(ctx->stream));
+  *count = 0;
+  if (ctx->sbuf.inc) {
+    unsigned int* c = ctx->sbuf.inc + ctx->sbuf.q_pad + 1;
+    std::vector<unsigned int> h((size_t)screen_prerej_words());
+    MH_HIP(ctx, hipMemcpy(h.data(), c, h.size() * sizeof(unsigned int), hipMemcpyDeviceToHost));
+    for (size_t k = 0; k < h.size(); k += (size_t)screen_prerej_pitch()) *count += h[k];
+    if (reset) MH_HIP(ctx, hipMemset(c, 0, h.size() * sizeof(unsigned int)));
+  }
+  return MH_OK;
+}
+
 int mh_match_set_mode(mh_ctx* ctx, int mode) {
   if (!ctx || mode < -1 || mode > 3) return MH_ERR_ARG;
   ctx->match_mode = mode;
diff --git a/moped_amd/csrc/api_frame.hip b/moped_amd/csrc/api_frame.hip
--- a/moped_amd/csrc/api_frame.hip
+++ b/moped_amd/csrc/api_frame.hip
@@ -145,7 +145,9 @@
   ctx->feat_count_dev = n_dev;
   stamp(ctx, 0);
   launch_normalize(ctx->q_desc, ctx->q_norm, Q, ctx->stream, n_dev);
-  if (int rc = ctx_match(ctx, ctx->q_desc, ctx->q_norm, Q, ctx->nn_idx, ctx->nn_d1, ctx->nn_d2, n_dev, ctx->feat_expected)) return rc;
+  if (int rc = ctx_match(ctx, ctx->q_desc, ctx->q_norm, Q, ctx->nn_idx, ctx->nn_d1, ctx->nn_d2, n_dev, ctx->feat_expected,
+                         frame_accept_ratio(ctx, prm)))
+    return rc;
   stamp(ctx, 1);
   FrameCall c{ctx->q_uv, Q, cam, prm, seed};
   c.q_count = n_dev;
@@ -161,7 +163,8 @@
   stamp(ctx, 0);
   hipLaunchKernelGGL(image_batch_tail_kernel, dim3((B * Q * (DIM / 4) + 255) / 256), dim3(256), 0, s, ctx->q_desc, ctx->q_norm,
                      counts, Q, B);
-  if (int rc = ctx_match(ctx, ctx->q_desc, ctx->q_norm, B * Q, ctx->nn_idx, ctx->nn_d1, ctx->nn_d2)) return rc;
+  if (int rc = ctx_match(ctx, ctx->q_desc, ctx->q_norm, B * Q, ctx->nn_idx, ctx->nn_d1, ctx->nn_d2, nullptr, 0, frame_accept_ratio(ctx, prm)))
+    return rc;
   hipLaunchKernelGGL(image_batch_mask_kernel, dim3((B * Q + 255) / 256), dim3(256), 0, s, ctx->nn_idx, ctx->nn_d1, ctx->nn_d2,
                      counts, Q, B);
   stamp(ctx, 1);
@@ -210,7 +213,10 @@
   stamp(ctx, 0);
   launch_normalize(q_desc_dev, ctx->q_norm, Q, ctx->stream);
   if (opt.write_back && ctx->wb_ev) hipEventRecord(ctx->wb_ev, ctx->stream);
-  if (int rc_m = ctx_match(ctx, q_desc_dev, ctx->q_norm, Q, ctx->nn_idx, ctx->nn_d1, ctx->nn_d2)) return rc_m;
+  const bool whole = opt.stage_lo == 0 && opt.stage_hi == 5;
+  if (int rc_m = ctx_match(ctx, q_desc_dev, ctx->q_norm, Q, ctx->nn_idx, ctx->nn_d1, ctx->nn_d2, nullptr, 0,
+                           whole ? frame_accept_ratio(ctx, prm) : 0.f))
+    return rc_m;
   stamp(ctx, 1);
   ctx->step.done = -1;
   FrameCall c{q_uv_dev, Q, cam, prm, seed};
@@ -908,7 +914,8 @@
   ctx->feat_count_dev = nullptr;
   stamp(ctx, 0);
   launch_normalize(q_desc_dev, ctx->q_norm, B * Q, ctx->stream);
-  if ((rc = ctx_match(ctx, q_desc_dev, ctx->q_norm, B * Q, ctx->nn_idx, ctx->nn_d1, ctx->nn_d2))) return rc;
+  if ((rc = ctx_match(ctx, q_desc_dev, ctx->q_norm, B * Q, ctx->nn_idx, ctx->nn_d1, ctx->nn_d2, nullptr, 0, frame_accept_ratio(ctx, prm))))
+    return rc;
   stamp(ctx, 1);
   return rest_of_batch(ctx, FrameCall{q_uv_dev, Q, cam, prm, 0}, B, seeds, merge, true);
 }
diff --git a/moped_amd/csrc/context.h b/moped_amd/csrc/context.h
--- a/moped_amd/csrc/context.h
+++ b/moped_amd/csrc/context.h
@@ -123,6 +123,7 @@
     mh::DevBuf<unsigned int> stats, inc;
   } screen_own;
   int match_mode = -1;
+  float match_accept = 0.f;
   int pose_split = 1;
   std::shared_ptr<DbPool> pool;
   int db_models_reserved = 0;
@@ -324,7 +325,10 @@
 int depth_map_from_raw_own(mh_ctx* ctx, const char* who, const void* raw_host, const mh_raw_depth* raw, const float K[4],
                            int width, int height);
 int ctx_match(mh_ctx* ctx, const float* qn, const float* qnorm, int Q, int32_t* idx1, float* d1, float* d2,
-              const int32_t* q_count = nullptr, int q_expected = 0);
+              const int32_t* q_count = nullptr, int q_expected = 0, float accept_ratio = 0.f);
+inline float frame_accept_ratio(const mh_ctx* ctx, const mh_frame_params* prm) {
+  return ctx->match_accept >= 0.f && !ctx->rules.ratio_table && prm && prm->ratio > 0.f ? prm->ratio : 0.f;
+}
 int delivery_begin(mh_ctx* ctx, void* host_block, size_t bytes, unsigned char** dst_dev);
 int delivery_end(mh_ctx* ctx, void* host_block, size_t bytes, unsigned char* dst_dev, int B, int max_objects, uint32_t tag);
 int sift_into(mh_ctx* ctx, const uint8_t* gray_dev, int width, int height, int double_size, int cap,
diff --git a/moped_amd/csrc/match_screen.hip b/moped_amd/csrc/match_screen.hip
--- a/moped_amd/csrc/match_screen.hip
+++ b/moped_amd/csrc/match_screen.hip
@@ -32,10 +32,27 @@
 __host__ __device__ constexpr int sc_lds_bytes(int nw) { return SC_LDS_TILES + nw * sc_recbuf(nw) * SC_REC_BYTES; }
 static_assert(SC_TILE == 128 && DIM == 128, "tile image and chunk swizzle assume 128 x 128");
 
+__host__ __device__ inline float screen_value_err(float qq, float dmax) {
+  const float nq = sqrtf(fmaxf(qq, 0.f));
+  return 0.000978f * nq * dmax + 4e-7f * (nq + dmax) + 3e-5f * (nq * dmax + 0.5f * dmax * dmax);
+}
 __host__ __device__ inline float screen_margin(float qq, float dmax) {
-  const float nq = sqrtf(fmaxf(qq, 0.f));
-  const float E = 0.000978f * nq * dmax + 4e-7f * (nq + dmax) + 3e-5f * (nq * dmax + 0.5f * dmax * dmax);
+  const float E = screen_value_err(qq, dmax);
   return 2.f * E + 2e-6f * (qq + dmax * dmax);
+}
+
+__host__ __device__ inline bool screen_reject_proved(float qq, float dmax, float h1, float l2, float tau_q, float ratio) {
+  const float big = 1e30f;
+  if (!(ratio > 0.f) || !(ratio < big) || !(fabsf(qq) < big) || !(fabsf(dmax) < big) || !(fabsf(tau_q) < big)) return false;
+  if (!(fabsf(l2) < big) || !(h1 < big)) return false;
+  const float top = fmaxf(h1, tau_q);
+  const float delta = 2.f * screen_value_err(qq, dmax) + 2e-6f * (qq + dmax * dmax);
+  const float mag = fabsf(qq) + 2.f * fabsf(top) + 2.f * fabsf(l2) + delta;
+  const float slack = 1e-6f * mag;
+  const float lo_d1 = qq - 2.f * top - delta - slack;
+  const float hi_d2 = qq - 2.f * l2 + delta + slack;
+  if (!(hi_d2 > 0.f)) return false;
+  return lo_d1 >= ratio * hi_d2 * 1.000001f;
 }
 
 __global__ __launch_bounds__(256) void db_to_half_kernel(const float* __restrict__ db, const float* __restrict__ dnorm, int N,
@@ -1027,6 +1044,7 @@
 }
 
 constexpr int RS_WAVES = 4;
+constexpr int RS_WAVES_ACCEPT = 1;
 #ifdef MH_EXPERIMENTS
 constexpr int RS_WAVES_FAT = 16;
 constexpr int RS_FAT_K = 2;
@@ -1087,6 +1105,7 @@
   unsigned incw;
   float2 qv;
 };
+constexpr int RS_PREREJ_WORDS = 16, RS_PREREJ_PITCH = 64;
 constexpr size_t rs_lds_bytes(int waves) { return (size_t)waves * (DIM * 4 + RS_MAXC * 4 + SC_SA_SLOTS * 4 + 8); }
 
 struct RsArgs {
@@ -1118,6 +1137,8 @@
   unsigned int* inc_count;
   const _Float16* dbh;
   const float* dneg;
+  float accept_ratio;
+  unsigned int* prerej;
 };
 typedef const __attribute__((address_space(4))) RsArgs* RsArgsPtr;
 __device__ __forceinline__ RsArgsPtr rs_args() {
@@ -1158,14 +1179,15 @@
 }
 
 static_assert(RS_ITERS_C <= RS_ITERS, "a counted list's slots fit the registers the scan has");
-template <int COMPACT>
+template <int COMPACT, int ACCEPT = 0>
 __device__ __forceinline__ void rescore_query(
     int q, int lane, float* q_sw, int* cand_sw, int* samp_sw, int* ncand_sw, int* nsamp_sw, uint2 (&recv)[RS_ITERS], const RsScalars sc, int Qe,
     const float* __restrict__ db, const float* __restrict__ dnorm, int N,
     RowMap rmap, uint2* __restrict__ recs, int n_slots, int32_t* __restrict__ ovf_cnt, uint2* __restrict__ ovf,
     int ovf_cap, float dmax, float spread, int32_t* __restrict__ idx1, float* __restrict__ d1, float* __restrict__ d2,
     unsigned int* __restrict__ stats, int32_t zero_idx, float zero_d1, float zero_d2, SampleGeom g,
-    unsigned int* __restrict__ inc_count, const _Float16* __restrict__ dbh, const float* __restrict__ dneg) {
+    unsigned int* __restrict__ inc_count, const _Float16* __restrict__ dbh, const float* __restrict__ dneg,
+    float accept_ratio = 0.f, unsigned int* __restrict__ prerej = nullptr) {
   uint2* mine = recs + (size_t)q * SC_SLOT_PITCH;
   const int n_own = COMPACT ? min(sc.n_ovf, SC_SLOT_PITCH) : n_slots + g.sa_slots;
   auto slot_at = [&](int j) -> uint2& { return mine[COMPACT || j < n_slots ? j : SC_SLOTS_MAX + (j - n_slots)]; };
@@ -1212,6 +1234,7 @@
   int n_cand = 0;
   if (!brute) {
     float l1 = -__builtin_inff(), l2 = -__builtin_inff();
+    float h1 = -__builtin_inff();
     const float pert = screen_pack_pert(nq, dmax, g.pack_bits);
     auto bounds = [tau_q, spread, N, dmax, pert](uint2 rec, float& lo, float& hi) {
       if (rec.x & SC_REC_SAMPLE) screen_sample_bounds((unsigned short)(rec.y >> 16), tau_q, pert, dmax, lo, hi);
@@ -1242,6 +1265,7 @@
         bounds(rec, lo, hi);
         l2 = fmaxf(l2, fminf(l1, lo));
         l1 = fmaxf(l1, lo);
+        if (ACCEPT) h1 = fmaxf(h1, hi);
       }
     };
     if (COMPACT) {
@@ -1259,6 +1283,17 @@
       const float o1 = __shfl_xor(l1, d), o2 = __shfl_xor(l2, d);
       l2 = fmaxf(fmaxf(l2, o2), fminf(l1, o1));
       l1 = fmaxf(l1, o1);
+      if (ACCEPT) h1 = fmaxf(h1, __shfl_xor(h1, d));
+    }
+    if (ACCEPT && incw == 0u && accept_ratio > 0.f && screen_reject_proved(nq, dmax, h1, l2, tau_q, accept_ratio)) {
+      if (lane == 0) {
+        if (n_ovf) ovf_cnt[q] = 0;
+        idx1[q] = -1;
+        d1[q] = __builtin_inff();
+        d2[q] = __builtin_inff();
+        if (prerej) atomicAdd(prerej + (q % RS_PREREJ_WORDS) * RS_PREREJ_PITCH, 1u);
+      }
+      return;
     }
     const float keep_from = l2 - screen_margin(nq, dmax);
     auto keep = [&](int it) {
@@ -1395,7 +1430,7 @@
   }
 }
 
-template <int WAVES, int PF, int COMPACT>
+template <int WAVES, int PF, int COMPACT, int ACCEPT = 0>
 __global__ __launch_bounds__(64 * WAVES) __attribute__((amdgpu_waves_per_eu(WAVES == 12 ? 6 : 8, WAVES == 12 ? 6 : 8))) void rescore_kernel(const RsArgs args) {
   MH_TRACE_SCOPE(mh::TK_PASS_C);
   extern __shared__ __attribute__((aligned(16))) unsigned char rs_lds[];
@@ -1437,6 +1472,11 @@
     rmap.nb = A->rmap.nb;
     rmap.base = A->rmap.base;
     const SampleGeom g = {A->g.sa_slots, A->g.pack_bits, A->g.tile_first, A->g.tile_stride, A->g.tiles_base, A->g.tiles_rem, A->g.n_sel};
+    if (ACCEPT)
+      rescore_query<COMPACT, 1>(q, lane, q_sw, cand_sw, samp_sw, ncand_sw, nsamp_sw, recv, sc, Qe, A->db, A->dnorm, A->N, rmap, A->recs,
+                    A->n_slots, A->ovf_cnt, A->ovf, A->ovf_cap, A->dmax, A->spread, A->idx1, A->d1, A->d2, A->stats, A->zero_idx,
+                    A->zero_d1, A->zero_d2, g, A->inc_count, A->dbh, A->dneg, A->accept_ratio, A->prerej);
+    else
     rescore_query<COMPACT>(q, lane, q_sw, cand_sw, samp_sw, ncand_sw, nsamp_sw, recv, sc, Qe, A->db, A->dnorm, A->N, rmap, A->recs,
                   A->n_slots, A->ovf_cnt, A->ovf, A->ovf_cap, A->dmax, A->spread, A->idx1, A->d1, A->d2, A->stats, A->zero_idx,
                   A->zero_d1, A->zero_d2, g, A->inc_count, A->dbh, A->dneg);
@@ -1534,6 +1574,11 @@
 #endif
 
 float screen_margin_host(float qq, float dmax) { return screen_margin(qq, dmax); }
+bool screen_reject_proved_host(float qq, float dmax, float h1, float l2, float tau_q, float ratio) {
+  return screen_reject_proved(qq, dmax, h1, l2, tau_q, ratio);
+}
+int screen_prerej_words() { return RS_PREREJ_WORDS * RS_PREREJ_PITCH; }
+int screen_prerej_pitch() { return RS_PREREJ_PITCH; }
 
 size_t screen_db_half_elems(int N) { return ((size_t)N + SC_TILE - 1) / SC_TILE * SC_TILE * DIM; }
 size_t screen_dneg_elems(int N) { return ((size_t)N + SC_TILE - 1) / SC_TILE * SC_DD; }
@@ -1746,16 +1791,22 @@
   *geom_out = g;
 }
 
-template <int WAVES, int PF, int COMPACT>
+template <int WAVES, int PF, int COMPACT, int ACCEPT = 0>
 void launch_pass_c_layout(int grid, hipStream_t s, const RsArgs& args) {
   static DynLds attr;
-  attr.ensure(rescore_kernel<WAVES, PF, COMPACT>, rs_lds_bytes(WAVES));
-  hipLaunchKernelGGL((rescore_kernel<WAVES, PF, COMPACT>), dim3(grid), dim3(64 * WAVES), rs_lds_bytes(WAVES), s, args);
+  attr.ensure(rescore_kernel<WAVES, PF, COMPACT, ACCEPT>, rs_lds_bytes(WAVES));
+  hipLaunchKernelGGL((rescore_kernel<WAVES, PF, COMPACT, ACCEPT>), dim3(grid), dim3(64 * WAVES), rs_lds_bytes(WAVES), s, args);
 }
 template <int WAVES, int PF>
 void launch_pass_c(int grid, hipStream_t s, const RsArgs& args, bool compact) {
   if (compact) launch_pass_c_layout<WAVES, PF, 1>(grid, s, args);
   else launch_pass_c_layout<WAVES, PF, 0>(grid, s, args);
+}
+template <int WAVES>
+void launch_pass_c_accept(int Q, hipStream_t s, const RsArgs& args, bool compact) {
+  const int grid = (Q + WAVES - 1) / WAVES;
+  if (compact) launch_pass_c_layout<WAVES, 0, 1, 1>(grid, s, args);
+  else launch_pass_c_layout<WAVES, 0, 0, 1>(grid, s, args);
 }
 
 struct ShapeChoice {
@@ -1862,6 +1913,19 @@
   ca.dmax = sdb.dmax; ca.tau = sb.tau; ca.spread = sdb.spread; ca.idx1 = idx1; ca.d1 = d1; ca.d2 = d2; ca.stats = sb.stats;
   ca.zero_idx = sdb.zero_idx; ca.zero_d1 = sdb.zero_d1; ca.zero_d2 = sdb.zero_d2; ca.g = geom;
   ca.inc = geom.sa_slots > 0 ? sb.inc : nullptr; ca.inc_count = sb.inc ? sb.inc + sb.q_pad : nullptr; ca.dbh = sdb.dbh; ca.dneg = sdb.dneg;
+  ca.accept_ratio = sb.accept_ratio > 0.f ? sb.accept_ratio : 0.f;
+  ca.prerej = sb.inc ? sb.inc + sb.q_pad + 1 : nullptr;
+  if (ca.accept_ratio > 0.f) {
+#ifdef MH_EXPERIMENTS
+    static const int pa_waves = exp_int("MH_PASSC_WAVES", RS_WAVES_ACCEPT);
+    if (pa_waves == 4) launch_pass_c_accept<4>(Q, s, ca, shape.passes16);
+    else if (pa_waves == 2) launch_pass_c_accept<2>(Q, s, ca, shape.passes16);
+    else
+#endif
+    launch_pass_c_accept<RS_WAVES_ACCEPT>(Q, s, ca, shape.passes16);
+    if (sb.ev) hipEventRecord(sb.ev[5], s);
+    return;
+  }
 #ifdef MH_EXPERIMENTS
   static const int pc_waves = exp_int("MH_PASSC_WAVES", RS_WAVES), pc_k = exp_int("MH_PASSC_K", RS_FAT_K);
   static const int pc_pf = exp_int("MH_PASSC_PREFETCH", 0), pc_all = exp_int("MH_PASSC_FAT_ALL", 0);
diff --git a/moped_amd/csrc/screen.h b/moped_amd/csrc/screen.h
--- a/moped_amd/csrc/screen.h
+++ b/moped_amd/csrc/screen.h
@@ -29,6 +29,7 @@
   hipEvent_t ev_in = nullptr, ev_out = nullptr;
   unsigned int* stats = nullptr;
   unsigned int* inc = nullptr;
+  float accept_ratio = 0.f;
   int n_cus = 0;
 };
 
@@ -78,6 +79,9 @@
 size_t screen_rec_slots();
 
 float screen_margin_host(float qq, float dmax);
+bool screen_reject_proved_host(float qq, float dmax, float h1, float l2, float tau_q, float ratio);
+int screen_prerej_words();
+int screen_prerej_pitch();
 void launch_screen_values(const _Float16* qh, int Q, const ScreenDb& sdb, int n_rows, float* out, hipStream_t s, int shape);
 void launch_screen_sample_values(const float* qn, int Q, const ScreenDb& sdb, const int32_t* row0, float* out, hipStream_t s);
 void launch_screen_prepare(const float* qn, const float* qnorm, int Q, int q_pad, _Float16* qh, uint8_t* qbad, hipStream_t s);
```

After: 17670 (median of 6 runs). +2.9%, better.
